# wangxiaohit/GNNPN-SC

Hardware: AMD Instinct MI355X
Metric: service-composition problems/sec (ML+2PN inference) (higher is better)
Workload: dtype f32-split3xf16 (f32 operands and results; recurrent W_hh.h products: fp32 operands split exactly into 3 x f16, six f16-matrix-core products per term, f32 accumulate; everything else f32 arithmetic)

## Files before the change

### gnnpn-sc_amd/_lib.py

```python
import ctypes
import os
from ctypes import c_char_p, c_double, c_float, c_int, c_int32, c_int64, c_uint32, c_void_p

import torch

_HERE = os.path.dirname(os.path.abspath(__file__))
LIB_PATH = os.environ.get("GNNPN_LIB") or os.path.join(_HERE, "libgnnpn_hip.so")
ABI_VERSION = 9

ACT_NONE, ACT_RELU, ACT_SIGMOID = 0, 1, 2
E_UNSUP = -2
WOA_OK, WOA_ROWS_MISMATCH, WOA_INDEX_ERROR, WOA_NO_SLOTS = 0, 1, 2, 3

_P = c_void_p
_SIGNATURES = {
    "gnnpn_abi_version": (c_int, []),
    "gnnpn_last_error": (c_char_p, []),
    "gnnpn_linear_f32": (c_int, [_P, c_int64, _P, c_int64, _P, _P, _P, c_int, _P, c_int64, c_int64, c_int, c_int, _P]),
    "gnnpn_embed_concat_f32": (c_int, [_P, _P, c_int, c_int, c_int, _P, c_int64, _P]),
    "gnnpn_csr_aggregate_f32": (c_int, [_P, _P, _P, _P, c_int64, _P, _P, _P, _P, c_int, _P, c_int64, c_int32,
                                        c_int32, _P]),
    "gnnpn_csr_aggregate_blocks_f32": (c_int, [_P, _P, _P, _P, c_int64, _P, _P, _P, _P, c_int, _P, c_int64, c_int32,
                                               c_int32, c_int32, _P, _P]),
    "gnnpn_csr_block_row_order": (c_int, [_P, c_int32, c_int32, _P, _P]),
    "gnnpn_csr_tile_plan_geometry": (c_int, [c_int32, c_int32, _P]),
    "gnnpn_csr_tile_plan_rows": (c_int, [_P, _P, _P, c_int32, c_int32, _P, _P, _P, _P, _P, _P]),
    "gnnpn_csr_tile_plan_fill": (c_int, [_P, _P, c_int32, c_int32, _P, _P, _P, _P, c_int64, _P]),
    "gnnpn_csr_aggregate_tiled_f32": (c_int, [_P, _P, _P, _P, _P, c_int64, _P, _P, _P, _P, c_int, _P, c_int64, c_int32, c_int32,
                                              c_int32, _P]),
    "gnnpn_gcn_norm_f32": (c_int, [_P, _P, _P, _P, _P, c_int32, _P]),
    "gnnpn_segment_mean_f32": (c_int, [_P, _P, c_int64, _P, c_int64, c_int32, c_int32, _P]),
    "gnnpn_gin_layer_f32": (c_int, [_P, _P, _P, c_int64, c_int32, _P, _P, _P, _P, _P, c_int32, _P, _P, _P, _P, c_int32, _P, _P, c_int32,
                                    _P, c_int64, c_int64, _P]),
    "gnnpn_split_weights_bytes": (c_int64, [c_int32, c_int32]),
    "gnnpn_lstm_split_weights_bytes": (c_int64, []),
    "gnnpn_lstm_pack_split_weights_f32": (c_int, [_P, _P, _P]),
    "gnnpn_pack_split_weights_f16": (c_int, [_P, c_int64, c_int32, c_int32, _P, _P, _P]),
    "gnnpn_gin_layer_split": (c_int, [_P, _P, _P, c_int64, c_int32, _P, _P, _P, _P, _P, _P, c_int32, _P, _P, _P, _P, _P, c_int32,
                                      _P, _P, _P, c_int32, _P, c_int64, c_int64, _P]),
    "gnnpn_request_branch_f32": (c_int, [_P, c_int32, _P, c_int32, c_int32, _P, _P, _P, c_int32, c_int32, c_int32, _P, c_int32,
                                         _P, _P, _P, _P]),
    "gnnpn_select_candidates": (c_int, [_P, c_int64, _P, _P, _P, _P, _P, _P, _P, c_int32, c_int32, c_int32, _P]),
    "gnnpn_rank_rows": (c_int, [_P, c_int64, _P, c_int32, c_int32, _P]),
    "gnnpn_precision_at_k": (c_int, [_P, c_int64, _P, c_int64, c_int32, c_int32, _P, c_int32, _P, _P]),
    "gnnpn_lstm_encode_f32": (c_int, [c_int, _P, c_int32, c_int32, c_int32, c_int32, c_int32, _P, _P, c_int64, _P]),
    "gnnpn_lstm_encode_workspace_bytes": (c_int64, []),
    "gnnpn_set_option": (c_int, [c_char_p, c_int]),
    "gnnpn_decode_diag": (c_int, [_P, c_int32, c_int32]),
    "gnnpn_coop_reset_staffing": (c_int, []),
    "gnnpn_last_launch_units": (c_int64, []),
    "gnnpn_lds_footprint_kb": (c_int, [c_int]),
    "gnnpn_coop_staffing_count": (c_int, []),
    "gnnpn_bn_train_forward_f32": (c_int, [_P, c_int64, c_int32, _P, _P, c_float, c_float, c_int, _P, _P, _P, _P, _P, _P]),
    "gnnpn_bn_train_backward_f32": (c_int, [_P, _P, _P, _P, _P, c_int64, c_int32, c_int, _P, _P, _P, _P]),
    "gnnpn_bce_sigmoid_f32": (c_int, [_P, _P, c_int64, _P, _P, _P]),
    "gnnpn_dot_f32": (c_int, [_P, _P, c_int64, _P, _P]),
    "gnnpn_embed_grad_f32": (c_int, [_P, c_int64, _P, c_int64, c_int64, c_int32, c_int32, _P, _P]),
    "gnnpn_pointer_decode_f32": (c_int, [c_int, _P, _P, c_float, c_int, c_int32, c_int32, c_int32, c_int32, c_int32,
                                         _P, _P, c_int64, _P]),
    "gnnpn_pointer_decode_workspace_bytes": (c_int64, [c_int32, c_int32, c_int32]),
    "gnnpn_pointer_decode_replicas_f32": (c_int, [_P, _P, c_float, c_int, c_int32, c_int32, c_int32, ctypes.c_uint64, c_int32, c_int32,
                                                  c_int32, _P, _P, c_int64, _P]),
    "gnnpn_replica_seed": (ctypes.c_uint64, [ctypes.c_uint64, c_int32]),
    "gnnpn_best_of_select_f32": (c_int, [c_int32, c_int32, c_int32, _P, _P, _P, _P, _P, _P, _P, _P, _P, _P, _P, _P, _P, _P]),
    "gnnpn_pointer_decode_attn_f32": (c_int, [_P, _P, _P, c_float, c_int, c_int32, c_int32, c_int32, c_int32, _P]),
    "gnnpn_attention_logits_f32": (c_int, [_P, _P, c_int64, _P, c_float, c_int, _P, c_int32, c_int32, c_int32,
                                           c_int32, c_int32, _P]),
    "gnnpn_attention_logits_bahdanau_f32": (c_int, [_P, _P, c_int64, _P, _P, c_float, c_int, _P, c_int32, c_int32, c_int32, c_int32, c_int32, _P]),
    "gnnpn_qos_reward_f32": (c_int, [_P, _P, c_int32, c_int32, c_int, _P]),
    "gnnpn_split3_pieces_f32": (c_int, [_P, c_int64, c_int32, _P, _P, _P, _P]),
    "gnnpn_recurrent_product_f32": (c_int, [_P, _P, c_int32, _P, _P, _P]),
    "gnnpn_gemm_f32": (c_int, [_P, c_int64, c_int, _P, c_int64, c_int, _P, c_int64, c_int64, c_int, c_int, c_int, _P]),
    "gnnpn_colsum_chunks_f32": (c_int, [_P, c_int64, c_int64, c_int32, c_int64, _P, _P]),
    "gnnpn_lstm_train_forward_f32": (c_int, [_P, _P, _P, _P, _P, _P, c_int32, c_int32, c_int32, _P]),
    "gnnpn_decode_train_forward_f32": (c_int, [_P, c_int32, c_int32, c_int32, c_int32, c_float, c_int, _P]),
    "gnnpn_decode_train_backward_f32": (c_int, [_P, _P, _P, _P, _P, _P, _P, c_int32, c_int32, c_int32, c_int32, c_float, c_int, _P]),
    "gnnpn_lstm_train_backward_f32": (c_int, [_P, _P, _P, _P, _P, _P, _P, c_int32, c_int32, c_int32, _P]),
    "gnnpn_decode_attn_train_forward_f32": (c_int, [_P, c_int32, c_int32, c_int32, c_int32, c_float, c_int, _P]),
    "gnnpn_decode_attn_train_backward_f32": (c_int, [_P, _P, _P, _P, _P, _P, _P, c_int32, c_int32, c_int32, c_int32, c_float, c_int, _P]),
    "gnnpn_colsum_f32": (c_int, [_P, c_int64, c_int64, c_int32, _P, _P]),
    "gnnpn_scatter_dx_f32": (c_int, [_P, _P, _P, c_int32, c_int32, c_int32, c_int32, _P]),
    "gnnpn_sumsq_f32": (c_int, [_P, c_int64, _P, _P]),
    "gnnpn_adam_step_f32": (c_int, [_P, _P, _P, _P, c_int64, _P, c_float, c_float, c_float, c_float, c_float, c_int32, _P]),
    "gnnpn_eswoa_f64": (c_int, [c_int32, c_int32, _P, _P, _P, _P, _P, c_int32, c_int32, _P, c_int32, _P, _P, _P, _P, _P]),
    "gnnpn_eswoa_wide_workspace_bytes": (c_int64, [c_int32, c_int32, c_int32]),
    "gnnpn_eswoa_wide_f64": (c_int, [c_int32, c_int32, _P, _P, _P, _P, _P, c_int32, c_int32, _P, _P, c_int64, _P, _P, _P, _P, _P]),
    "gnnpn_eswoa_ragged_workspace_bytes": (c_int64, [c_int32, c_int32, c_int32, c_int32]),
    "gnnpn_eswoa_ragged_f64": (c_int, [c_int32, _P, c_int32, c_int32, c_int32, _P, _P, _P, _P, _P, c_int32, c_int32, _P, c_int32, _P,
                                       c_int64, _P, _P, _P, _P, _P, _P]),
    "gnnpn_woa_candidates_workspace_bytes": (c_int64, [c_int32, c_int32, c_int32]),
    "gnnpn_woa_candidates_count": (c_int, [c_int32, c_int32, _P, c_int32, _P, _P, _P, c_int32, _P, _P, _P, c_int32, c_int32, c_double,
                                           _P, c_int32, c_int32, _P, c_int64, _P, _P, _P, _P, _P, _P]),
    "gnnpn_woa_candidates_fill": (c_int, [c_int32, c_int32, _P, _P, _P, c_int32, _P, c_int64, _P, _P, c_int32, c_int32, _P, _P, _P, _P,
                                          _P]),
    "gnnpn_debug_round5_f64": (c_int, [_P, _P, c_int64, _P]),
    "gnnpn_debug_cell_activations": (c_int, [_P, _P, _P, c_int64, _P]),
    "gnnpn_debug_lds_interferer": (c_int, [c_int32, c_int32, c_int32, _P]),
    "gnnpn_gate_wait": (c_int, [_P, c_uint32, c_int32, _P]),
    "gnnpn_debug_mfma_f16": (c_int, [_P, _P, _P, _P, _P]),
}
EXPORTS = tuple(_SIGNATURES)

class DecodeNet(ctypes.Structure):
    _fields_ = [(n, _P) for n in ("embedded", "enc_out", "h0", "c0", "start", "wih_packed", "whh_packed", "bih",
                                  "bhh", "latent_win", "emb_w", "emb_b", "xw_fold", "xb_fold", "start_fold", "idx", "win_logits", "pick_prob", "actions",
                                  "queries")] + \
               [("latent_from", c_int32), ("sample", c_int32), ("sample_seed", ctypes.c_uint64), ("whh_split", _P)]


class Attention(ctypes.Structure):
    _fields_ = [("attention", c_int32), ("n_glimpses", c_int32)] + \
               [(n, _P) for n in ("pointer_wq", "pointer_bq", "pointer_ref", "pointer_v", "glimpse_wq", "glimpse_bq",
                                  "glimpse_ref", "glimpse_v")]


class LaunchOpts(ctypes.Structure):
    _fields_ = [("impl", c_int32), ("lds_kb", c_int32), ("write_through", c_int32), ("paired_start", c_int32),
                ("sticky_status", _P)]


class TilePlanGeom(ctypes.Structure):
    _fields_ = [(n, c_int32) for n in ("n_blocks", "src_tiles", "src_tile_rows", "dst_tiles", "dst_tile_rows", "units", "wavefronts",
                                       "passes")] + \
               [(n, c_int64) for n in ("header_bytes", "order_bytes", "tstart_bytes", "selfw_bytes", "meta_bytes")]


class GinLayer(ctypes.Structure):
    _fields_ = [(n, _P) for n in ("w0_packed", "b0", "bn1_scale", "bn1_shift", "w3_packed", "b3", "bn2_scale", "bn2_shift",
                                  "eps")]


class DecodeTrain(ctypes.Structure):
    _fields_ = [(n, _P) for n in ("embedded", "enc_out", "h0", "c0", "start", "wih", "whh", "bih", "bhh", "latent_win", "idx",
                                  "x_all", "gates_pre", "c_all", "h_all", "z0", "probs", "logp")]


class DecodeAttnTrain(ctypes.Structure):
    _fields_ = ([("base", DecodeTrain), ("bahdanau", c_int32), ("n_glimpses", c_int32)]
                + [(n, _P) for n in ("p_wq_t", "p_wq", "p_bq", "p_v", "p_ref", "g_wq_t", "g_wq", "g_bq", "g_v", "g_ref", "q_all", "a_all",
                                     "d_p_ref", "d_g_ref", "d_p_qp", "d_g_qp", "d_p_v", "d_g_v")])


class EncodeNet(ctypes.Structure):
    _fields_ = [(n, _P) for n in ("pregates", "inputs", "w_in", "b_in", "whh_packed", "bhh", "enc_out", "h_n", "c_n", "whh_split")]


_lib = None


class GnnpnError(RuntimeError):
    pass


SOURCE_GROUPS = {
    "recurrent": ("lstm_coop.hip", "decode_lean.hip", "decode_coop.hip", "coop_common.h", "common.h", "recurrent.h", "lstm_shared.h",
                  "decode_shared.h", "lstm.hip", "decode.hip"),
    "aggregate": ("graph_tiled.hip", "graph.hip", "graph_lds.h", "common.h"),
}


def source_hash(group=None):
    import hashlib
    root = os.path.dirname(_HERE)
    csrc = os.path.join(_HERE, "csrc")
    if group is None:
        files = sorted(os.path.join(csrc, f) for f in os.listdir(csrc) if f.endswith((".hip", ".h", ".cpp")))
    else:
        files = sorted(os.path.join(csrc, f) for f in SOURCE_GROUPS[group])
    files.append(os.path.join(root, "include", "gnnpn_hip.h"))
    h = hashlib.sha256()
    for f in files:
        h.update(os.path.basename(f).encode())
        with open(f, "rb") as fh:
            h.update(fh.read())
    return h.hexdigest()[:16]


def load():
    global _lib
    if _lib is not None:
        return _lib
    if not os.path.exists(LIB_PATH):
        raise GnnpnError(
            f"{LIB_PATH} is missing: build it with `python gnnpn-sc_amd/build.py` (hipcc, gfx950). "
            "There is no CPU fallback for the ML+2PN hot path.")
    lib = ctypes.CDLL(LIB_PATH)
    for name, (res, args) in _SIGNATURES.items():
        fn = getattr(lib, name)
        fn.restype, fn.argtypes = res, args
    if lib.gnnpn_abi_version() != ABI_VERSION:
        raise GnnpnError(f"ABI mismatch: library {lib.gnnpn_abi_version()} vs binding {ABI_VERSION}")
    _lib = lib
    return lib


def check(rc, what):
    if rc != 0:
        msg = load().gnnpn_last_error().decode("utf-8", "replace")
        raise GnnpnError(f"{what} failed ({rc}): {msg}")


def stream_ptr():
    return ctypes.c_void_p(torch.cuda.current_stream().cuda_stream)


def dev_ptr(t, dtype, name, allow_none=False):
    if t is None:
        if allow_none:
            return None
        raise GnnpnError(f"{name}: tensor required")
    if not isinstance(t, torch.Tensor) or not t.is_cuda:
        raise GnnpnError(f"{name}: expected a CUDA tensor (the hot path has no CPU implementation), got "
# ... 14 lines not shown
```

### gnnpn-sc_amd/csrc/coop_common.h

```cpp
#pragma once
#include "common.h"
#include "lstm_shared.h"

typedef float f32x4 __attribute__((ext_vector_type(4)));
typedef unsigned long long u64;

__device__ __forceinline__ void granule_store(u64* p, unsigned tag, float v) {
    __hip_atomic_store(p, ((u64)tag << 32) | __float_as_uint(v), __ATOMIC_RELAXED,
                       __HIP_MEMORY_SCOPE_AGENT);
}

typedef unsigned u32x4 __attribute__((ext_vector_type(4)));
#define GNNPN_LD2(dst, voff, sbase, off) "global_load_dwordx4 " dst ", " voff ", " sbase " offset:" off " sc1\n\t"
__device__ __forceinline__ const u64* uniform_ptr(const u64* p) {
    const unsigned long long v = (unsigned long long)p;
    const unsigned lo = __builtin_amdgcn_readfirstlane((unsigned)v), hi = __builtin_amdgcn_readfirstlane((unsigned)(v >> 32));
    return reinterpret_cast<const u64*>(((unsigned long long)hi << 32) | lo);
}
__device__ __forceinline__ void granule_reload2_x8_masked(u32x4 (&v)[8], const u64* base, unsigned voff, unsigned long long lanes) {
    const u64* q = base + 512;
    unsigned long long saved;
    asm volatile("s_and_saveexec_b64 %8, %12\n\t"
                 GNNPN_LD2("%0", "%9", "%10", "0") GNNPN_LD2("%1", "%9", "%10", "1024") GNNPN_LD2("%2", "%9", "%10", "2048")
                 GNNPN_LD2("%3", "%9", "%10", "3072") GNNPN_LD2("%4", "%9", "%11", "0") GNNPN_LD2("%5", "%9", "%11", "1024")
                 GNNPN_LD2("%6", "%9", "%11", "2048") GNNPN_LD2("%7", "%9", "%11", "3072")
                 "s_waitcnt vmcnt(0)\n\t"
                 "s_mov_b64 exec, %8"
                 : "+v"(v[0]), "+v"(v[1]), "+v"(v[2]), "+v"(v[3]), "+v"(v[4]), "+v"(v[5]), "+v"(v[6]), "+v"(v[7]), "=&s"(saved)
                 : "v"(voff), "s"(base), "s"(q), "s"(lanes)
                 : "memory", "scc");
}
__device__ __forceinline__ void granule_load2_x8_x4(u32x4 (&v)[8], u32x4 (&w)[4], const u64* base, const u64* pbase, unsigned voff) {
    const u64* q = base + 512;
    asm volatile(GNNPN_LD2("%0", "%12", "%13", "0") GNNPN_LD2("%1", "%12", "%13", "1024") GNNPN_LD2("%2", "%12", "%13", "2048")
                 GNNPN_LD2("%3", "%12", "%13", "3072") GNNPN_LD2("%4", "%12", "%14", "0") GNNPN_LD2("%5", "%12", "%14", "1024")
                 GNNPN_LD2("%6", "%12", "%14", "2048") GNNPN_LD2("%7", "%12", "%14", "3072")
                 GNNPN_LD2("%8", "%12", "%15", "0") GNNPN_LD2("%9", "%12", "%15", "1024") GNNPN_LD2("%10", "%12", "%15", "2048")
                 GNNPN_LD2("%11", "%12", "%15", "3072")
                 "s_waitcnt vmcnt(0)"
                 : "=&v"(v[0]), "=&v"(v[1]), "=&v"(v[2]), "=&v"(v[3]), "=&v"(v[4]), "=&v"(v[5]), "=&v"(v[6]), "=&v"(v[7]),
                   "=&v"(w[0]), "=&v"(w[1]), "=&v"(w[2]), "=&v"(w[3])
                 : "v"(voff), "s"(base), "s"(q), "s"(pbase)
                 : "memory");
}

__device__ __forceinline__ void granule_load2_x8_x4_lat(u32x4 (&v)[8], u32x4 (&w)[4], u64& lat, const u64* base, const u64* pbase,
                                                        const u64* lbase, unsigned voff) {
    const u64* q = base + 512;
    asm volatile(GNNPN_LD2("%0", "%13", "%15", "0") GNNPN_LD2("%1", "%13", "%15", "1024") GNNPN_LD2("%2", "%13", "%15", "2048")
                 GNNPN_LD2("%3", "%13", "%15", "3072") GNNPN_LD2("%4", "%13", "%16", "0") GNNPN_LD2("%5", "%13", "%16", "1024")
                 GNNPN_LD2("%6", "%13", "%16", "2048") GNNPN_LD2("%7", "%13", "%16", "3072")
                 GNNPN_LD2("%8", "%13", "%17", "0") GNNPN_LD2("%9", "%13", "%17", "1024") GNNPN_LD2("%10", "%13", "%17", "2048")
                 GNNPN_LD2("%11", "%13", "%17", "3072")
                 "global_load_dwordx2 %12, %14, %18 sc1\n\t"
                 "s_waitcnt vmcnt(0)"
                 : "=&v"(v[0]), "=&v"(v[1]), "=&v"(v[2]), "=&v"(v[3]), "=&v"(v[4]), "=&v"(v[5]), "=&v"(v[6]), "=&v"(v[7]),
                   "=&v"(w[0]), "=&v"(w[1]), "=&v"(w[2]), "=&v"(w[3]), "=&v"(lat)
                 : "v"(voff), "v"(voff >> 1), "s"(base), "s"(q), "s"(pbase), "s"(lbase)
                 : "memory");
}

constexpr int COOP_STAFFING_WORD = 8 * 256 + 8;
__device__ __forceinline__ void coop_raise(unsigned* err, unsigned* sticky, unsigned code, unsigned* seats = nullptr) {
    atomicOr(err, code);
    if (sticky) atomicOr(sticky, code);
    if (seats && atomicCAS(err + 4, 1u, 2u) == 1u) atomicSub(seats + COOP_STAFFING_WORD, 1u);
}

constexpr int COOP_STATUS_BYTES = 16384;
constexpr unsigned COOP_LDS_UNITS = 640;
constexpr int COOP_XCD_STRIDE = 32;
constexpr int COOP_XCDCNT_OFFSET = 12288;
constexpr int COOP_ARRIVE_OFFSET = 13312;
constexpr int COOP_PLACED_OFFSET = 14336;
constexpr int COOP_CLAIM_OFFSET = 2048;
constexpr int COOP_TAKEN_OFFSET = 10240;
constexpr int COOP_OVERREAD_BYTES = 4096;
constexpr int COOP_OVERSUB = 3;
constexpr unsigned COOP_SURPLUS_WAIT_TICKS = 1600;
constexpr unsigned COOP_RESERVE_WAIT_TICKS = 200000;

__device__ __forceinline__ unsigned xcc_id() {
    return __builtin_amdgcn_s_getreg(20 | (0 << 6) | (3 << 11)) & 0xfu;
}

__device__ __forceinline__ void granule_store_l2_bits(u64* p, u64 g) {
    asm volatile("global_store_dwordx2 %0, %1, off" ::"v"(p), "v"(g) : "memory");
}
__device__ __forceinline__ void granule_store_l2(u64* p, unsigned tag, float v) {
    granule_store_l2_bits(p, ((u64)tag << 32) | __float_as_uint(v));
}
__device__ __forceinline__ void granule_publish(u64* p, unsigned tag, float v, bool same_xcd) {
    if (same_xcd) granule_store_l2(p, tag, v);
    else granule_store(p, tag, v);
}

namespace {
__global__ __launch_bounds__(256) void coop_zero_kernel(unsigned long long* __restrict__ p, size_t n8, unsigned* __restrict__ sticky,
                                                        int word, unsigned expected, int skip_zeroing) {
    if (sticky && blockIdx.x == 0 && threadIdx.x == 0) atomicAdd(sticky + word, expected);
    if (skip_zeroing) return;
    for (size_t i = blockIdx.x * (size_t)blockDim.x + threadIdx.x; i < n8; i += (size_t)gridDim.x * blockDim.x)
        __hip_atomic_store(p + i, 0ull, __ATOMIC_RELAXED, __HIP_MEMORY_SCOPE_AGENT);
}
}
inline hipError_t coop_zero_workspace(void* workspace, size_t bytes, hipStream_t s, unsigned* sticky, int word, unsigned expected,
                                      bool skip_zeroing = false) {
    const size_t n8 = bytes / 8;
    unsigned blocks = skip_zeroing ? 1u : (unsigned)((n8 + 255) / 256);
    if (blocks > 2048) blocks = 2048;
    hipLaunchKernelGGL(coop_zero_kernel, dim3(blocks), dim3(256), 0, s, static_cast<unsigned long long*>(workspace), n8, sticky, word,
                       expected, skip_zeroing ? 1 : 0);
    return hipGetLastError();
}

constexpr int COOP_G = 8, COOP_ROWS = 16, COOP_H = 256;

struct CoopLaunch {
    int n_tiles, gpx, groups, groups_per_net;
    unsigned* status;
    char* buffers;
    unsigned* seats;
};

template <typename Need>
inline int coop_begin(const char* who, int n_nets, int32_t rows, Need need, int expected_word, const CoopOpts& opts,
                      void* workspace, int64_t workspace_bytes, hipStream_t s, CoopLaunch& L) {
    int dev = 0, n_cu = 0;
    if (hipGetDevice(&dev) != hipSuccess ||
        hipDeviceGetAttribute(&n_cu, hipDeviceAttributeMultiprocessorCount, dev) != hipSuccess)
        GNNPN_FAIL(GNNPN_E_LAUNCH, "%s: cannot query the device", who);
    L.n_tiles = (rows + COOP_ROWS - 1) / COOP_ROWS;
    L.gpx = n_cu / (8 * COOP_G);
    if (L.gpx > 8) L.gpx = 8;
    while (L.gpx > 1 && (L.gpx - 1) * 8 >= n_nets * L.n_tiles) --L.gpx;
    if (L.gpx < 1 || n_cu < 256)
        GNNPN_FAIL(GNNPN_E_UNSUP, "%s: device has %d CUs, the cooperative form is built for 8 XCDs x 32 CUs", who, n_cu);
    L.groups = L.gpx * 8;
    if (L.groups < n_nets) GNNPN_FAIL(GNNPN_E_UNSUP, "%s: %d groups for %d nets", who, L.groups, n_nets);
    L.groups_per_net = L.groups / n_nets;
    const int64_t bytes = need(L.groups);
    if (!workspace || workspace_bytes < bytes || !gnnpn_aligned(workspace, 256))
        GNNPN_FAIL(GNNPN_E_ARG, "%s: workspace of %lld B (256-B aligned) required", who, (long long)bytes);
    L.seats = gnnpn_cu_seat_table();
    if (!L.seats) GNNPN_FAIL(GNNPN_E_LAUNCH, "%s: cannot allocate the seat table", who);
    const unsigned units = (unsigned)(COOP_G * n_nets * L.n_tiles);
    if (coop_zero_workspace(workspace, (size_t)bytes, s, opts.sticky, expected_word, units, (gnnpn_option_lstm_ablate() & 0x2000) != 0) !=
        hipSuccess)
        GNNPN_FAIL(GNNPN_E_LAUNCH, "%s: workspace memset failed", who);
    g_gnnpn_last_units = opts.sticky ? (int64_t)units : 0;
    L.status = static_cast<unsigned*>(workspace);
    L.buffers = static_cast<char*>(workspace) + COOP_STATUS_BYTES;
    return GNNPN_OK;
}

struct DecodeWorkspace {
    int64_t h_bytes, p_bytes, l_bytes;
    int64_t total() const { return COOP_STATUS_BYTES + h_bytes + p_bytes + l_bytes + COOP_OVERREAD_BYTES; }
};
inline DecodeWorkspace decode_workspace(int64_t groups, int64_t rows, int32_t T, int32_t K, int64_t xp_granules) {
    const int64_t tiles = (rows + COOP_ROWS - 1) / COOP_ROWS;
    return {groups * 2 * COOP_ROWS * COOP_H * 8, groups * 2 * xp_granules * 8, tiles * T * COOP_ROWS * (int64_t)K * 8};
}
__device__ __forceinline__ void coop_note_finished(unsigned* sticky, int word, unsigned tiles_done) {
    if (sticky && tiles_done) atomicAdd(sticky + word, tiles_done);
}

__device__ __forceinline__ void coop_note_staffed(unsigned* status, unsigned* count_xcc, unsigned target, unsigned* seats) {
    if (atomicAdd(count_xcc, 1u) + 1u == target && atomicAdd(status + 5, 1u) + 1u == 8u && atomicExch(status + 4, 2u) == 1u)
        atomicSub(seats + COOP_STAFFING_WORD, 1u);
}
template <int G>
__device__ __forceinline__ bool coop_place(unsigned* status, int gpx, int* slot, int& group, int& member, unsigned* seats,
                                           bool paired_start = false, unsigned* sticky = nullptr) {
    if (threadIdx.x < 64) {
        const int lane = threadIdx.x;
        const unsigned xcc = xcc_id();
        unsigned* count = status + COOP_XCDCNT_OFFSET / 4;
        unsigned* arrive = status + COOP_ARRIVE_OFFSET / 4;
        unsigned* taken = status + COOP_TAKEN_OFFSET / 4 + xcc * 64;
        const unsigned target = (unsigned)(gpx * G);
        auto staffed = [&]() {
            unsigned v = 0;
            if (lane == 0) v = __hip_atomic_load(status + 5, __ATOMIC_RELAXED, __HIP_MEMORY_SCOPE_AGENT);
            return __shfl(v, 0, 64) >= 8u;
        };
        int g = -1, m = 0;
#ifndef GNNPN_COOP_NO_ENTRY_ACQUIRE
        __builtin_amdgcn_fence(__ATOMIC_ACQUIRE, "agent");
#endif
        const unsigned hw = __builtin_amdgcn_s_getreg(4 | (0 << 6) | (31 << 11));
        const unsigned key = (xcc << 8) | ((hw >> 8) & 0xffu);
        unsigned* staffing = seats + COOP_STAFFING_WORD;
        const unsigned* word = lane < 8 ? count + COOP_XCD_STRIDE * lane : lane == 9 ? status + 4 : seats + key;
        unsigned got = 0;
        if (lane < 12 && lane != 8 && lane != 10) got = __hip_atomic_load(word, __ATOMIC_RELAXED, __HIP_MEMORY_SCOPE_AGENT);
        if (lane == 8) got = atomicAdd(arrive + COOP_XCD_STRIDE * xcc, 1u);
        const bool staffed_at_entry = __all(lane >= 8 || got >= target);
        unsigned arrival = __shfl(got, 8, 64);
        const bool marked = __shfl(got, 9, 64) != 0u;
        const unsigned seat_seen = __shfl(got, 11, 64);
        if (lane == 0) {
            if (arrival == 0u && !marked && atomicCAS(status + 4, 0u, 1u) == 0u) atomicAdd(staffing, 1u);
            if (arrival >= gridDim.x / 8 || (staffed_at_entry && arrival < target)) coop_raise(status, sticky, 8u);
        }
        if (!staffed_at_entry) {
            if (lane == 0) {
                atomicAdd(status + COOP_CLAIM_OFFSET / 4 + key, 1u);
                const unsigned la = __builtin_amdgcn_s_getreg(6 | (0 << 6) | (31 << 11));
                const unsigned lds_base = la & 0xfffu, lds_size = (la >> 12) & 0xfffu;
                const bool badly_placed = lds_base != 0u && lds_base < lds_size && lds_base + 2u * lds_size > COOP_LDS_UNITS;
                bool another_staffing = false;
                if (badly_placed && !paired_start) {
                    if (atomicCAS(status + 4, 0u, 1u) == 0u) atomicAdd(staffing, 1u);
                    another_staffing = __hip_atomic_load(staffing, __ATOMIC_RELAXED, __HIP_MEMORY_SCOPE_AGENT) > 1u;
                }
                const bool fragments = (paired_start || another_staffing) && badly_placed;
                const bool reserve_arrival = arrival + target >= gridDim.x / 8;
                if (fragments && !reserve_arrival) {
                    atomicAdd(status + 3, 1u);
                    if (sticky) atomicAdd(sticky + GNNPN_STATUS_DECLINED_SEATS, 1u);
                    g = -2;
                } else if (!fragments) {
                    unsigned s = seat_seen;
                    if (s == 0u) {
                        if (atomicCAS(seats + key, 0u, 0xffffffffu) == 0u) {
                            s = atomicAdd(seats + 8 * 256 + xcc, 1u) + 1u;
                            __hip_atomic_store(seats + key, s, __ATOMIC_RELAXED, __HIP_MEMORY_SCOPE_AGENT);
                        } else {
                            s = 0xffffffffu;
                        }
                    }
                    for (unsigned spin = 0; s == 0xffffffffu && spin < 100000u; ++spin)
                        s = __hip_atomic_load(seats + key, __ATOMIC_RELAXED, __HIP_MEMORY_SCOPE_AGENT);
                    const unsigned seat = s - 1u;
                    if (seat < target && atomicCAS(taken + seat, 0u, 1u) == 0u) {
                        g = (int)xcc * gpx + (int)(seat / G);
                        m = (int)(seat % G);
                        coop_note_staffed(status, count + COOP_XCD_STRIDE * xcc, target, seats);
                    }
                }
            }
            g = __shfl(g, 0, 64);
            m = __shfl(m, 0, 64);
            arrival = __shfl(arrival, 0, 64);
            if (g == -2) {
                g = -1;
            } else if (g < 0) {
                const unsigned per_xcd = gridDim.x / 8;
                const bool reserve = arrival + target >= per_xcd;
                const unsigned long long patience = reserve ? COOP_RESERVE_WAIT_TICKS : COOP_SURPLUS_WAIT_TICKS;
                const unsigned long long t0 = __builtin_amdgcn_s_memrealtime();
                bool done = staffed();
                while (!done && __builtin_amdgcn_s_memrealtime() - t0 < patience) {
                    __builtin_amdgcn_s_sleep(8);
                    done = staffed();
                }
                if (!done && reserve) {
                    if (lane == 0) {
                        for (unsigned seat = 0; seat < target && g < 0; ++seat) {
                            if (atomicCAS(taken + seat, 0u, 1u) == 0u) {
                                g = (int)xcc * gpx + (int)(seat / G);
                                m = (int)(seat % G);
                                coop_note_staffed(status, count + COOP_XCD_STRIDE * xcc, target, seats);
                                atomicAdd(status + 2, 1u);
                                if (sticky) atomicAdd(sticky + GNNPN_STATUS_OFF_CANONICAL_SEATS, 1u);
                            }
                        }
                    }
                    g = __shfl(g, 0, 64);
                    m = __shfl(m, 0, 64);
                }
            }
        }
        if (lane == 0) {
            slot[0] = g;
            slot[1] = m;
        }
    }
    __syncthreads();
    group = slot[0];
    member = slot[1];
    return group >= 0;
}

__device__ __forceinline__ float swap8(float v) {
    return __int_as_float(__builtin_amdgcn_update_dpp(0, __float_as_int(v), 0x128 , 0xF, 0xF, false));
}

__device__ __forceinline__ u64 phase_stamp() {
    u64 t;
    __builtin_amdgcn_sched_barrier(0);
    asm volatile("s_memtime %0\n\ts_waitcnt lgkmcnt(0)" : "=s"(t)::"memory");
    __builtin_amdgcn_sched_barrier(0);
    return t;
}

constexpr int LDT = 260;
__device__ __forceinline__ int ht_index(int row, int unit) { return row * LDT + (unit & 3) * 64 + (unit >> 2); }

struct NoHook {
// ... 220 lines not shown
```

### gnnpn-sc_amd/csrc/decode.hip

```cpp
#include <atomic>

#include "common.h"
#include <string.h>
#include "recurrent.h"
#include "decode_shared.h"
#include "lstm_shared.h"

template <int H, int BT, bool REP = false>
__global__ __launch_bounds__((H < 64 ? 64 : H)) void pointer_decode_kernel(
    const float* __restrict__ embedded, const float* __restrict__ enc_out, const float* __restrict__ h0,
    const float* __restrict__ c0, const float* __restrict__ start, const float* __restrict__ wih,
    const float* __restrict__ whh, const float* __restrict__ bih, const float* __restrict__ bhh,
    const float* __restrict__ latent_win, const float* __restrict__ inputs, float tanh_c, int use_tanh,
    int32_t* __restrict__ idx_out, float* __restrict__ win_logits, float* __restrict__ pick_prob,
    float* __restrict__ actions, float* __restrict__ queries, int32_t B, int32_t T, int32_t n_per, int sample,
    unsigned long long sample_seed, int rep_R, int rep_first) {
    constexpr int NT = H < 64 ? 64 : H;
    constexpr int NW = NT / 64;
    __shared__ __attribute__((aligned(16))) float xs[BT][H];
    __shared__ __attribute__((aligned(16))) float hs[2][BT][H];
    __shared__ float lg[BT][64];
    __shared__ int sel[BT];

    const int j = threadIdx.x;
    const bool owner = j < H;
    const int lane = j & 63, wave = j >> 6;
    const int b0 = blockIdx.x * BT;
    const int L = T * n_per;
    const float4* __restrict__ Wi = reinterpret_cast<const float4*>(wih);
    const float4* __restrict__ Wh = reinterpret_cast<const float4*>(whh);
    auto prob_of = [rep_R](int b) { return REP ? b / rep_R : b; };

    float bi[4], bh[4], c[BT], h[BT];
#pragma unroll
    for (int g = 0; g < 4; ++g) {
        bi[g] = owner ? bih[g * H + j] : 0.0f;
        bh[g] = owner ? bhh[g * H + j] : 0.0f;
    }
#pragma unroll
    for (int p = 0; p < BT; ++p) {
        const bool ok = owner && (b0 + p < B);
        c[p] = ok ? c0[(int64_t)prob_of(b0 + p) * H + j] : 0.0f;
        h[p] = ok ? h0[(int64_t)prob_of(b0 + p) * H + j] : 0.0f;
        if (owner) {
            hs[0][p][j] = h[p];
            xs[p][j] = start[j];
        }
    }
    __syncthreads();

    int cur = 0;
    for (int k = 0; k < T; ++k) {
        if (owner) {
            float ai[BT][4], ah[BT][4];
#pragma unroll
            for (int p = 0; p < BT; ++p)
#pragma unroll
                for (int g = 0; g < 4; ++g) ai[p][g] = ah[p][g] = 0.0f;
            gemv_chain<H, BT>(Wi, xs, j, ai);
            gemv_chain<H, BT>(Wh, hs[cur], j, ah);
#pragma unroll
            for (int p = 0; p < BT; ++p) {
                float gate[4];
#pragma unroll
                for (int g = 0; g < 4; ++g)
                    gate[g] = __fadd_rn(__fadd_rn(ah[p][g], bh[g]), __fadd_rn(ai[p][g], bi[g]));
                lstm_cell_update(gate[0], gate[1], gate[2], gate[3], c[p], h[p]);
                hs[cur ^ 1][p][j] = h[p];
                if (queries && b0 + p < B) queries[((int64_t)(b0 + p) * T + k) * H + j] = h[p];
            }
        }
        __syncthreads();
        cur ^= 1;

        for (int q = wave; q < BT * n_per; q += NW) {
            const int p = q / n_per, r = q - p * n_per;
            float part = 0.0f;
            if (b0 + p < B) part = lane_dot4<H>(enc_out + ((int64_t)prob_of(b0 + p) * L + (int64_t)k * n_per + r) * H, hs[cur][p]);
            const float dot = wave_sum(part);
            if (lane == 0) lg[p][r] = dot;
        }
        __syncthreads();

        if (j < BT && b0 + j < B) {
            const int p = j;
            const int64_t wbase = ((int64_t)(b0 + p) * T + k) * n_per;
            const int64_t lbase = ((int64_t)prob_of(b0 + p) * T + k) * n_per;
            const unsigned long long seed =
                REP ? replica_seed(sample_seed, (unsigned long long)(rep_first + (b0 + p) % rep_R)) : sample_seed;
            float prob;
            const int best_r = window_pick(lg[p], n_per, tanh_c, use_tanh, win_logits, wbase, latent_win, lbase,
                                           sample, seed, (unsigned long long)prob_of(b0 + p) * T + k, prob);
            pick_prob[(int64_t)(b0 + p) * T + k] = prob;
            idx_out[(int64_t)(b0 + p) * T + k] = k * n_per + best_r;
            sel[p] = k * n_per + best_r;
        }
        __syncthreads();

#pragma unroll
        for (int p = 0; p < BT; ++p) {
            if (b0 + p < B) {
                const int64_t row = (int64_t)prob_of(b0 + p) * L + sel[p];
                if (owner) xs[p][j] = embedded[row * H + j];
                if (j < 8) actions[((int64_t)(b0 + p) * T + k) * 8 + j] = inputs[row * 8 + j];
            }
        }
        __syncthreads();
    }
}

template <int H, bool REP = false>
static void launch_decode(const DecodeArgs& args, const DecodeNet& d, const float* latent, hipStream_t s,
                          ReplicaMap rep = ReplicaMap{0, 0}) {
    constexpr int NT = H < 64 ? 64 : H;
    const int32_t B = args.B;
    int bt = 1;
    while (bt < 4 && B / (bt * 2) >= 256) bt *= 2;
    dim3 grid((B + bt - 1) / bt), block(NT);
#define GNNPN_LAUNCH_DEC(BT_)                                                                                                    \
    hipLaunchKernelGGL((pointer_decode_kernel<H, BT_, REP>), grid, block, 0, s, d.embedded, d.enc_out, d.h0, d.c0, d.start, d.wih, \
                       d.whh, d.bih, d.bhh, latent, args.inputs, args.tanh_c, args.use_tanh, d.idx, d.win_logits, d.pick_prob,   \
                       d.actions, d.queries, B, args.T, args.K, d.sample, (unsigned long long)d.sample_seed, rep.R, rep.first)
    switch (bt) {
        case 1: GNNPN_LAUNCH_DEC(1); break;
        case 2: GNNPN_LAUNCH_DEC(2); break;
        default: GNNPN_LAUNCH_DEC(4); break;
    }
#undef GNNPN_LAUNCH_DEC
}

extern "C" int gnnpn_pointer_decode_f32(int n_nets, const gnnpn_decode_net_t* nets, const float* inputs,
                                        float tanh_c, int use_tanh, int32_t B, int32_t T, int32_t n_per, int32_t H,
                                        int32_t precision, const gnnpn_launch_opts_t* opts_in, void* workspace,
                                        int64_t workspace_bytes, void* stream) {
    g_gnnpn_last_units = 0;
    GNNPN_REQUIRE(B >= 0 && T > 0, "pointer_decode: bad shape");
    if (B == 0) return GNNPN_OK;
    GNNPN_REQUIRE(nets && inputs, "pointer_decode: null input");
    const CoopOpts opts = coop_opts(opts_in);
    GNNPN_REQUIRE(opts.impl >= 0 && opts.impl <= 4 && opts.impl != 3, "pointer_decode: opts.impl must be 0 (auto), 1 (streaming), 2 (cooperative, 8-CU groups) or 4 (8-CU groups, 256-register build) — the 16-CU-group form (3) was removed in ABI version 7");
    GNNPN_REQUIRE(opts.lds_kb >= 0 && opts.lds_kb <= 160, "pointer_decode: opts.lds_kb must be 0..160");
    GNNPN_REQUIRE(precision == GNNPN_PREC_F32 || precision == GNNPN_PREC_SPLIT, "pointer_decode: precision must be GNNPN_PREC_F32 or GNNPN_PREC_SPLIT, got %d", precision);
    GNNPN_REQUIRE(n_nets >= 1 && n_nets <= GNNPN_MAX_DECODE_NETS, "pointer_decode: n_nets must be 1..%d",
                  GNNPN_MAX_DECODE_NETS);
    GNNPN_REQUIRE(n_per >= 1 && n_per <= 64, "pointer_decode: n_per must be in [1,64], got %d", n_per);
    if (H != 256 && H != 32) GNNPN_FAIL(GNNPN_E_UNSUP, "pointer_decode: hidden size %d not built (256, 32)", H);
    DecodeArgs args{};
    for (int n = 0; n < n_nets; ++n) {
        const gnnpn_decode_net_t& d = nets[n];
        if (const int rc = decode_net_check(d, "pointer_decode", n)) return rc;
        GNNPN_REQUIRE(d.embedded || (d.emb_w && d.emb_b) || d.xw_fold,
                      "pointer_decode: net %d needs embedded, (emb_w, emb_b) or the folded input side", n);
        GNNPN_REQUIRE(d.latent_from < n && d.latent_from >= -1, "pointer_decode: latent_from of net %d must name an "
                      "earlier net of the call", n);
        GNNPN_REQUIRE(!(d.latent_win && d.latent_from >= 0), "pointer_decode: net %d has two latent sources", n);
        GNNPN_REQUIRE(!d.whh_split || gnnpn_aligned(d.whh_split, 16), "pointer_decode: whh_split must be 16-byte aligned");
        static_assert(sizeof(DecodeNet) == sizeof(gnnpn_decode_net_t), "layout");
        memcpy(&args.net[n], &d, sizeof(DecodeNet));
    }
    args.inputs = inputs;
    args.tanh_c = tanh_c;
    args.use_tanh = use_tanh;
    args.B = B;
    args.T = T;
    args.K = n_per;
    hipStream_t s = (hipStream_t)stream;
    bool any_sample = false;
    for (int n = 0; n < n_nets; ++n) any_sample |= nets[n].sample != 0;
    if (any_sample && (precision != GNNPN_PREC_F32 || opts.impl > 2))
        GNNPN_FAIL(GNNPN_E_UNSUP, "pointer_decode: sampling is built in the streaming and the 8-CU-group fp32 forms (impl 0-2, "
                   "GNNPN_PREC_F32)");
    const int impl = opts.impl;
    if (impl != 1 && gnnpn_decode_coop_supported(H, n_per) && (workspace != nullptr || impl >= 2)) {
        const int rc = gnnpn_launch_decode_coop(args, n_nets, precision, impl == 4, opts, workspace, workspace_bytes, s);
        const bool fall_through = rc == GNNPN_E_UNSUP && impl == 0 && precision == GNNPN_PREC_F32;
        if (rc != GNNPN_OK && !fall_through) return rc;
        if (fall_through) {
            static std::atomic<bool> said{false};
            if (!said.exchange(true))
                fprintf(stderr, "[gnnpn] pointer_decode: %s — taking the per-workgroup streaming form (about 10 x slower per step)\n", gnnpn_last_error());
        }
        if (rc == GNNPN_OK) {
            GNNPN_CHECK_LAUNCH("pointer_decode_f32(coop)");
            return GNNPN_OK;
        }
    }
    if (precision == GNNPN_PREC_SPLIT)
        GNNPN_FAIL(GNNPN_E_UNSUP, "pointer_decode: the split-operand precision needs the cooperative form (H = 256)");
    for (int n = 0; n < n_nets; ++n) {
        const DecodeNet& d = args.net[n];
        if (!d.embedded) GNNPN_FAIL(GNNPN_E_UNSUP, "pointer_decode: the streaming form needs the embedded tensor");
        const float* latent = d.latent_from >= 0 ? args.net[d.latent_from].win_logits : d.latent_win;
        GNNPN_FOR_H(H, launch_decode<HH>(args, d, latent, s));
    }
    GNNPN_CHECK_LAUNCH("pointer_decode_f32");
    return GNNPN_OK;
}

extern "C" uint64_t gnnpn_replica_seed(uint64_t seed, int32_t replica) {
    return replica_seed(seed, (unsigned long long)(long long)replica);
}

extern "C" int gnnpn_pointer_decode_replicas_f32(const gnnpn_decode_net_t* net, const float* inputs, float tanh_c, int use_tanh,
                                                 int32_t B, int32_t R, int32_t first, uint64_t seed, int32_t T, int32_t n_per,
                                                 int32_t H, const gnnpn_launch_opts_t* opts_in, void* workspace,
                                                 int64_t workspace_bytes, void* stream) {
    g_gnnpn_last_units = 0;
    GNNPN_REQUIRE(R >= 1, "pointer_decode_replicas: R must be >= 1, got %d", R);
    GNNPN_REQUIRE(first >= 0, "pointer_decode_replicas: first replica must be >= 0, got %d", first);
    GNNPN_REQUIRE(B >= 0 && T > 0 && n_per >= 1 && n_per <= 64, "pointer_decode_replicas: bad shape (B %d, T %d, n_per %d)", B, T, n_per);
    const int64_t rows = (int64_t)B * R;
    GNNPN_REQUIRE(rows <= (1 << 30), "pointer_decode_replicas: B*R = %lld rows exceed 2^30", (long long)rows);
    if (H != 256 && H != 32) GNNPN_FAIL(GNNPN_E_UNSUP, "pointer_decode_replicas: hidden size %d not built (256, 32)", H);
    if (B == 0) return GNNPN_OK;
    GNNPN_REQUIRE(net && inputs, "pointer_decode_replicas: null input");
    const CoopOpts opts = coop_opts(opts_in);
    GNNPN_REQUIRE(opts.impl >= 0 && opts.impl <= 2, "pointer_decode_replicas: opts.impl must be 0 (auto), 1 (streaming) or 2 (cooperative)");
    GNNPN_REQUIRE(opts.lds_kb >= 0 && opts.lds_kb <= 160, "pointer_decode_replicas: opts.lds_kb must be 0..160");
    const gnnpn_decode_net_t& d = *net;
    if (const int rc = decode_net_check(d, "pointer_decode_replicas", 0)) return rc;
    GNNPN_REQUIRE(d.embedded || d.xw_fold, "pointer_decode_replicas: the net needs embedded or the folded input side");
    GNNPN_REQUIRE(!d.queries, "pointer_decode_replicas: queries are not written (must be NULL)");
    GNNPN_REQUIRE(d.latent_from == -1, "pointer_decode_replicas: latent_from must be -1 (Low's window logits come from latent_win)");
    DecodeArgs args{};
    memcpy(&args.net[0], &d, sizeof(DecodeNet));
    args.net[0].sample = 1;
    args.net[0].sample_seed = seed;
    args.net[0].whh_split = nullptr;
    args.inputs = inputs;
    args.tanh_c = tanh_c;
    args.use_tanh = use_tanh;
    args.B = (int32_t)rows;
    args.T = T;
    args.K = n_per;
    hipStream_t s = (hipStream_t)stream;
    const bool coop = opts.impl != 1 && gnnpn_decode_coop_supported(H, n_per) && d.xw_fold && (workspace != nullptr || opts.impl == 2);
    if (coop) {
        const int64_t need = gnnpn_decode_coop_workspace_need(rows, T, n_per);
        GNNPN_REQUIRE(workspace && workspace_bytes >= need && gnnpn_aligned(workspace, 256),
                      "pointer_decode_replicas: B*R = %lld rows need a workspace of %lld B (256-B aligned), got %lld B",
                      (long long)rows, (long long)need, (long long)workspace_bytes);
        const int rc = gnnpn_launch_decode_coop(args, 1, GNNPN_PREC_F32, false, opts, workspace, workspace_bytes, s,
                                                ReplicaMap{R, first});
        if (rc != GNNPN_OK) return rc;
        GNNPN_CHECK_LAUNCH("pointer_decode_replicas_f32(coop)");
        return GNNPN_OK;
    }
    if (opts.impl == 2) GNNPN_FAIL(GNNPN_E_UNSUP, "pointer_decode_replicas: the cooperative form needs H = 256, n_per <= 16 and the folded input side");
    if (!d.embedded) GNNPN_FAIL(GNNPN_E_UNSUP, "pointer_decode_replicas: the streaming form needs the embedded tensor");
    GNNPN_FOR_H(H, (launch_decode<HH, true>(args, args.net[0], args.net[0].latent_win, s, ReplicaMap{R, first})));
    GNNPN_CHECK_LAUNCH("pointer_decode_replicas_f32");
    return GNNPN_OK;
}

__global__ __launch_bounds__(256) void attention_logits_kernel(const float* __restrict__ enc_out,
                                                               const float* __restrict__ queries, int64_t ld_q,
                                                               float tanh_c, int use_tanh, float* __restrict__ logits,
                                                               int64_t n_rows, int32_t L, int32_t H) {
    const int lane = threadIdx.x & 63;
    const int64_t row = (int64_t)blockIdx.x * 4 + (threadIdx.x >> 6);
    if (row >= n_rows) return;
    const int64_t b = row / L;
    const float* e = enc_out + row * H;
    const float* q = queries + b * ld_q;
    float part = 0.0f;
    for (int i = lane * 4; i < H; i += 256) {
        const float4 ev = *reinterpret_cast<const float4*>(e + i);
        const float4 qv = *reinterpret_cast<const float4*>(q + i);
        part = fmaf(ev.x, qv.x, part);
        part = fmaf(ev.y, qv.y, part);
        part = fmaf(ev.z, qv.z, part);
        part = fmaf(ev.w, qv.w, part);
    }
    float v = wave_sum(part);
    if (use_tanh) v = __fmul_rn(tanh_c, tanhf(v));
    if (lane == 0) logits[row] = v;
}

__global__ __launch_bounds__(256) void attention_logits_bahdanau_kernel(const float* __restrict__ ref, const float* __restrict__ qp,
                                                                        int64_t ld_q, const float* __restrict__ v, float tanh_c,
                                                                        int use_tanh, float* __restrict__ logits, int64_t n_rows,
                                                                        int32_t L, int32_t H) {
    const int lane = threadIdx.x & 63;
    const int64_t row = (int64_t)blockIdx.x * 4 + (threadIdx.x >> 6);
    if (row >= n_rows) return;
    const float* r = ref + row * H;
    const float* q = qp + (row / L) * ld_q;
    float part = 0.0f;
    for (int i = lane; i < H; i += 64) part = fmaf(v[i], tanhf(q[i] + r[i]), part);
    float u = wave_sum(part);
    if (use_tanh) u = __fmul_rn(tanh_c, tanhf(u));
    if (lane == 0) logits[row] = u;
}

__global__ void mask_logits_kernel(const int32_t* __restrict__ masked_idx, float* __restrict__ logits, int32_t B,
                                   int32_t L, int32_t n_masked, int32_t ld_idx) {
    const int i = blockIdx.x * blockDim.x + threadIdx.x;
    if (i >= B * n_masked) return;
    const int b = i / n_masked, m = i - b * n_masked;
    const int pos = masked_idx[(int64_t)b * ld_idx + m];
    if (pos >= 0 && pos < L) logits[(int64_t)b * L + pos] = -INFINITY;
}

extern "C" int gnnpn_attention_logits_f32(const float* enc_out, const float* queries, int64_t ld_q,
                                          const int32_t* masked_idx, float tanh_c, int use_tanh, float* logits,
                                          int32_t B, int32_t L, int32_t H, int32_t n_masked, int32_t ld_idx,
                                          void* stream) {
    GNNPN_REQUIRE(B >= 0 && L > 0 && H > 0 && H % 4 == 0 && ld_q >= H && ld_q % 4 == 0, "attention_logits: bad shape");
    if (B == 0) return GNNPN_OK;
    GNNPN_REQUIRE(enc_out && queries && logits, "attention_logits: null operand");
    GNNPN_REQUIRE(n_masked == 0 || (masked_idx && ld_idx >= n_masked), "attention_logits: bad mask list");
    GNNPN_REQUIRE(gnnpn_aligned(enc_out, 16) && gnnpn_aligned(queries, 16), "attention_logits: 16-byte alignment");
    if (B == 0) return GNNPN_OK;
    hipStream_t s = (hipStream_t)stream;
    const int64_t n_rows = (int64_t)B * L;
    hipLaunchKernelGGL(attention_logits_kernel, dim3((unsigned)((n_rows + 3) / 4)), dim3(256), 0, s, enc_out, queries,
                       ld_q, tanh_c, use_tanh, logits, n_rows, L, H);
    if (n_masked > 0)
        hipLaunchKernelGGL(mask_logits_kernel, dim3((B * n_masked + 255) / 256), dim3(256), 0, s, masked_idx, logits,
                           B, L, n_masked, ld_idx);
    GNNPN_CHECK_LAUNCH("attention_logits_f32");
    return GNNPN_OK;
}

extern "C" int gnnpn_attention_logits_bahdanau_f32(const float* ref, const float* qp, int64_t ld_q, const float* v,
                                                   const int32_t* masked_idx, float tanh_c, int use_tanh, float* logits, int32_t B,
                                                   int32_t L, int32_t H, int32_t n_masked, int32_t ld_idx, void* stream) {
    GNNPN_REQUIRE(ref && qp && v && logits && B >= 0 && L > 0 && H > 0 && ld_q >= H, "attention_logits_bahdanau: bad argument");
    GNNPN_REQUIRE(n_masked == 0 || (masked_idx && ld_idx >= n_masked), "attention_logits_bahdanau: bad mask");
    if (B == 0) return GNNPN_OK;
    hipStream_t s = (hipStream_t)stream;
    const int64_t n_rows = (int64_t)B * L;
    hipLaunchKernelGGL(attention_logits_bahdanau_kernel, dim3((unsigned)((n_rows + 3) / 4)), dim3(256), 0, s, ref, qp, ld_q, v,
                       tanh_c, use_tanh, logits, n_rows, L, H);
    if (n_masked > 0)
        hipLaunchKernelGGL(mask_logits_kernel, dim3((B * n_masked + 255) / 256), dim3(256), 0, s, masked_idx, logits, B, L,
                           n_masked, ld_idx);
    GNNPN_CHECK_LAUNCH("attention_logits_bahdanau_f32");
    return GNNPN_OK;
}

__global__ __launch_bounds__(256) void qos_reward_kernel(const float* __restrict__ actions, float* __restrict__ R, int32_t B,
                                                        int32_t T, int level) {
    const int lane = threadIdx.x & 63;
    const int b = blockIdx.x * 4 + (threadIdx.x >> 6);
    if (b >= B) return;
    const float* a = actions + (int64_t)b * T * 8;
    const float lo0 = a[4], hi0 = a[5], lo1 = a[6], hi1 = a[7];
    float prod2 = 1.0f, prod3 = 1.0f, mn = INFINITY;
    double sum0 = 0.0;
    int n_real = 0;
    auto fetch = [&](int t) { return *reinterpret_cast<const float4*>(a + (int64_t)min(t, T - 1) * 8); };
    auto consume = [&](float4 q, int t0) {
        if (t0 + lane >= T) q = make_float4(0.0f, INFINITY, 1.0f, 1.0f);
        n_real += q.x > 0.0f;
        mn = fminf(mn, q.y);
        const double xd = (double)q.x;
        const int lo = __double2loint(xd), hi = __double2hiint(xd);
        const int zi = __float_as_int(q.z), wi = __float_as_int(q.w);
        const int cnt = min(64, T - t0);
#define GNNPN_REWARD_STEP(i)                                                                                      \
    prod2 = __fmul_rn(prod2, __int_as_float(__builtin_amdgcn_readlane(zi, i)));                                   \
    prod3 = __fmul_rn(prod3, __int_as_float(__builtin_amdgcn_readlane(wi, i)));                                   \
    sum0 += __hiloint2double(__builtin_amdgcn_readlane(hi, i), __builtin_amdgcn_readlane(lo, i));
        if (cnt == 64) {
#pragma unroll
            for (int i = 0; i < 64; ++i) { GNNPN_REWARD_STEP(i) }
        } else {
            for (int i = 0; i < cnt; ++i) { GNNPN_REWARD_STEP(i) }
        }
#undef GNNPN_REWARD_STEP
    };
    float4 qa = fetch(lane), qb;
    for (int t0 = 0; t0 < T; t0 += 128) {
        qb = fetch(t0 + 64 + lane);
        consume(qa, t0);
        if (t0 + 64 >= T) break;
        qa = fetch(t0 + 128 + lane);
        consume(qb, t0 + 64);
    }
#pragma unroll
    for (int off = 32; off > 0; off >>= 1) {
        n_real += __shfl_xor(n_real, off, 64);
        mn = fminf(mn, __shfl_xor(mn, off, 64));
    }
    if (lane != 0) return;
    int violate = 0;
    if (prod2 < lo0 || prod2 > hi0) ++violate;
    if (prod3 < lo1 || prod3 > hi1) ++violate;
    if (level == 0) {
        R[b] = (float)violate;
        return;
    }
    float obj = (float)sum0 / (float)n_real;
    obj = __fadd_rn(obj, 1.0f);
    obj = __fsub_rn(obj, mn);
    obj = obj / 2.0f;
    const double v = (double)violate + (double)obj;
    R[b] = (float)(rint(v * 1e5) / 1e5);
}

extern "C" int gnnpn_qos_reward_f32(const float* actions, float* R, int32_t B, int32_t T, int level,
                                    void* stream) {
    GNNPN_REQUIRE(B >= 0 && T > 0 && (level == 0 || level == 1), "qos_reward: bad argument");
    if (B == 0) return GNNPN_OK;
    GNNPN_REQUIRE(actions && R, "qos_reward: null operand");
    hipLaunchKernelGGL(qos_reward_kernel, dim3((B + 3) / 4), dim3(256), 0, (hipStream_t)stream, actions, R, B, T,
                       level);
    GNNPN_CHECK_LAUNCH("qos_reward_f32");
    return GNNPN_OK;
}

__global__ __launch_bounds__(256) void best_of_select_kernel(int32_t B, int32_t N, int32_t T, const float* __restrict__ R0,
                                                             const int32_t* __restrict__ idx0, const float* __restrict__ act0,
                                                             const float* __restrict__ prob0, const float* __restrict__ Rs,
                                                             const int32_t* __restrict__ idxs, const float* __restrict__ acts,
                                                             const float* __restrict__ probs, float* __restrict__ R_out,
                                                             int32_t* __restrict__ idx_out, float* __restrict__ act_out,
                                                             float* __restrict__ prob_out, int32_t* __restrict__ winner) {
    const int lane = threadIdx.x & 63;
    const int b = blockIdx.x * 4 + (threadIdx.x >> 6);
    if (b >= B) return;
    const int S = N - 1;
    unsigned long long best = ~0ull;
    for (int j = lane; j < N; j += 64) {
        float r = j == 0 ? R0[b] : Rs[(int64_t)b * S + (j - 1)];
        if (r == 0.0f) r = 0.0f;
        const unsigned hi = r != r ? 0xFFFFFFFFu : float_order_key(r);
        const unsigned long long key = ((unsigned long long)hi << 32) | (unsigned)j;
        best = key < best ? key : best;
    }
#pragma unroll
    for (int off = 32; off > 0; off >>= 1) {
        const unsigned lo = __shfl_xor((unsigned)(best & 0xffffffffu), off, 64);
        const unsigned hi = __shfl_xor((unsigned)(best >> 32), off, 64);
        const unsigned long long o = ((unsigned long long)hi << 32) | lo;
        best = o < best ? o : best;
    }
    const int w = (int)(best & 0xffffffffu);
    const int64_t src = w == 0 ? (int64_t)b : (int64_t)b * S + (w - 1);
    const int32_t* si = (w == 0 ? idx0 : idxs) + src * T;
    const float* sp = (w == 0 ? prob0 : probs) + src * T;
    const float* sa = (w == 0 ? act0 : acts) + src * T * 8;
    for (int t = lane; t < T; t += 64) {
        idx_out[(int64_t)b * T + t] = si[t];
        prob_out[(int64_t)b * T + t] = sp[t];
    }
    for (int i = lane; i < T * 8; i += 64) act_out[(int64_t)b * T * 8 + i] = sa[i];
    if (lane == 0) {
        winner[b] = w;
        R_out[b] = w == 0 ? R0[b] : Rs[src];
    }
}

extern "C" int gnnpn_best_of_select_f32(int32_t B, int32_t N, int32_t T, const float* R0, const int32_t* idx0, const float* actions0,
                                        const float* probs0, const float* Rs, const int32_t* idxs, const float* actionss,
                                        const float* probss, float* R_out, int32_t* idx_out, float* actions_out, float* probs_out,
                                        int32_t* winner, void* stream) {
    GNNPN_REQUIRE(B >= 0 && N >= 1 && T > 0 && (int64_t)T * 8 < (1ll << 31), "best_of_select: bad argument (B %d, N %d, T %d)", B, N, T);
    if (B == 0) return GNNPN_OK;
    GNNPN_REQUIRE(R0 && idx0 && actions0 && probs0, "best_of_select: null input (replica 0)");
    GNNPN_REQUIRE(N == 1 || (Rs && idxs && actionss && probss), "best_of_select: null input (replicas 1..N-1)");
    GNNPN_REQUIRE(R_out && idx_out && actions_out && probs_out && winner, "best_of_select: null output");
    hipLaunchKernelGGL(best_of_select_kernel, dim3((B + 3) / 4), dim3(256), 0, (hipStream_t)stream, B, N, T, R0, idx0, actions0,
                       probs0, Rs, idxs, actionss, probss, R_out, idx_out, actions_out, probs_out, winner);
    GNNPN_CHECK_LAUNCH("best_of_select_f32");
    return GNNPN_OK;
}
```

### gnnpn-sc_amd/csrc/decode_lean.hip

```cpp
#include "common.h"
#include "recurrent.h"
#include "decode_shared.h"
#include "coop_common.h"
#include "lstm_shared.h"

namespace {
constexpr int H = COOP_H;
constexpr int G = COOP_G;
constexpr int ROWS = COOP_ROWS;
constexpr int UNITS = H / G;
constexpr int KW = 16;
constexpr unsigned SPIN_LIMIT = 400000;
constexpr int XP_GRANULES = ROWS * KW * G;

typedef unsigned u32x2 __attribute__((ext_vector_type(2)));
constexpr int AUX_SC1 = 16;


__device__ __forceinline__ __amdgpu_buffer_rsrc_t make_rsrc(const void* p, unsigned bytes) {
    return __builtin_amdgcn_make_buffer_rsrc(const_cast<void*>(p), 0, (int)bytes, 0x00020000);
}
__device__ __forceinline__ float dpp_ror(float v, int n) {
    switch (n) {
        case 1: return __int_as_float(__builtin_amdgcn_update_dpp(0, __float_as_int(v), 0x121, 0xF, 0xF, true));
// ... 277 lines not shown
                    float dot = 0.0f, lv = 0.0f;
                    if (live) {
                        dot = __fadd_rn(__fadd_rn(__fadd_rn(__uint_as_float(vp[0].x), __uint_as_float(vp[0].z)), __uint_as_float(vp[1].x)), __uint_as_float(vp[1].z));
                        dot = __fadd_rn(__fadd_rn(__fadd_rn(__fadd_rn(dot, __uint_as_float(vp[2].x)), __uint_as_float(vp[2].z)), __uint_as_float(vp[3].x)), __uint_as_float(vp[3].z));
                        if (latent_in_launch) lv = __uint_as_float(vl.x);
                        else if (net.latent_win) lv = __uint_as_float(__builtin_amdgcn_raw_buffer_load_b32(r_lw, vo_wl, so_t, 0));
                    }
                    float v = a.use_tanh ? __fmul_rn(a.tanh_c, tanhf(dot)) : dot;
                    if (live && first) {
                        __builtin_amdgcn_raw_buffer_store_b32(__float_as_uint(v), r_wl, vo_wl, so_t, 0);
                        if (publishes_latent)
                            __builtin_amdgcn_raw_buffer_store_b64(u32x2{__float_as_uint(v), 1u}, r_lat, vo_lat, so_l0, AUX_SC1);
                    }
                    v = (has_lat && live) ? __fadd_rn(v, lv) : v;
                    float m = live ? v : -INFINITY;
                    m = fmaxf(m, dpp_ror(m, 8));
                    m = fmaxf(m, dpp_ror(m, 4));
                    m = fmaxf(m, dpp_ror(m, 2));
                    m = fmaxf(m, dpp_ror(m, 1));
                    const unsigned hit = (unsigned)(__ballot(live && v == m) >> (16 * rq)) & 0xffffu;
                    const int pick_r = hit ? __ffs(hit) - 1 : 0;
                    if (r == 0) {
                        sel[row] = pick_r;
                        if (first) __builtin_amdgcn_raw_buffer_store_b32((unsigned)((k - 1) * K + pick_r), r_idx, vo_idx, (unsigned)(k - 1) * 4u, 0);
                    }
                }
                __syncthreads();
                if (abort_flag) break;
                axf0 = win[c][sel[c]][kq];
                axf1 = win[c][sel[c]][4 + kq];
                if (first && wave == 0) {
                    __builtin_amdgcn_raw_buffer_store_b32(__float_as_uint(axf0), r_act, vo_act, (unsigned)(k - 1) * 32u, 0);
                    __builtin_amdgcn_raw_buffer_store_b32(__float_as_uint(axf1), r_act, vo_act, (unsigned)(k - 1) * 32u + 16u, 0);
                }
                if (k == T) break;
                if constexpr (DIAG) st[5] = phase_stamp();
            }

            if constexpr (!EV_EARLY) request_ev();
            u32x4 wv0, wv1;
            wv0 = __builtin_amdgcn_raw_buffer_load_b128(r_in, vo_win, so_k * 32u, 0);
            wv1 = __builtin_amdgcn_raw_buffer_load_b128(r_in, vo_win, so_k * 32u + 16u, 0);
            float gx[2][4];
            if (k > 0) {
                f32x4 ax0 = {0.f, 0.f, 0.f, 0.f}, ax1 = ax0;
                ax0 = __builtin_amdgcn_mfma_f32_16x16x4f32(axf0, wXf[0][0], ax0, 0, 0, 0);
                ax1 = __builtin_amdgcn_mfma_f32_16x16x4f32(axf0, wXf[1][0], ax1, 0, 0, 0);
                ax0 = __builtin_amdgcn_mfma_f32_16x16x4f32(axf1, wXf[0][1], ax0, 0, 0, 0);
                ax1 = __builtin_amdgcn_mfma_f32_16x16x4f32(axf1, wXf[1][1], ax1, 0, 0, 0);
#pragma unroll
                for (int q = 0; q < 4; ++q) {
                    gx[0][q] = __fadd_rn(ax0[q], bi[0]);
                    gx[1][q] = __fadd_rn(ax1[q], bi[1]);
                }
            } else {
#pragma unroll
                for (int q = 0; q < 4; ++q) {
                    gx[0][q] = sg[0];
                    gx[1][q] = sg[1];
                }
            }
            {
                f32x2 g0[2], g1[2];
#pragma unroll
                for (int q = 0; q < 2; ++q) {
                    g0[q] = (f32x2{ah[0][2 * q], ah[0][2 * q + 1]} + pk_set(bh[0])) + f32x2{gx[0][2 * q], gx[0][2 * q + 1]};
                    g1[q] = (f32x2{ah[1][2 * q], ah[1][2 * q + 1]} + pk_set(bh[1])) + f32x2{gx[1][2 * q], gx[1][2 * q + 1]};
                }
                cell_update_split(g0, g1, c < 8, cst, hl);
            }
            {
                const unsigned so_pub = (step & 1) * (ROWS * H * 8);
                if constexpr (SPLIT) {
                    store_granule(r_h, vo_hpub, so_pub, split_granule(step + 1, hl.x), same_xcd);
                    store_granule(r_h, vo_hpub, so_pub + H * 8, split_granule(step + 1, hl.y), same_xcd);
                } else {
                    store_granule(r_h, vo_hpub, so_pub, ((u64)(step + 1) << 32) | __float_as_uint(hl.x), same_xcd);
                    store_granule(r_h, vo_hpub, so_pub + H * 8, ((u64)(step + 1) << 32) | __float_as_uint(hl.y), same_xcd);
                }
                hsl[own0][wave * 8 + (c & 7)] = hl.x;
                hsl[own0 + 1][wave * 8 + (c & 7)] = hl.y;
                if (net.queries) {
                    __builtin_amdgcn_raw_buffer_store_b32(__float_as_uint(hl.x), r_q, vo_q, (unsigned)k * (H * 4), 0);
                    __builtin_amdgcn_raw_buffer_store_b32(__float_as_uint(hl.y), r_q, vo_q, (unsigned)(k + T) * (H * 4), 0);
                }
            }
            if constexpr (DIAG) {
                asm volatile("" ::"v"(hl.y));
                st[6] = phase_stamp();
            }
            __syncthreads();
            {
                float p = 0.0f;
                if (pdot) {
#pragma unroll
                    for (int j = 0; j < EVN; ++j) {
                        const float4 hv = *reinterpret_cast<const float4*>(&hsl[prow][phalf * (4 * EVN) + 4 * j]);
                        p = fmaf(__uint_as_float(ev[j].x), hv.x, p);
                        p = fmaf(__uint_as_float(ev[j].y), hv.y, p);
                        p = fmaf(__uint_as_float(ev[j].z), hv.z, p);
                        p = fmaf(__uint_as_float(ev[j].w), hv.w, p);
                    }
                }
                if constexpr (EVH == 2)
                    p = __fadd_rn(p, __int_as_float(__builtin_amdgcn_update_dpp(0, __float_as_int(p), 0xB1 , 0xF, 0xF, false)));
                if (pdot && phalf == 0)
                    store_granule(r_p, vo_ppub, (step & 1) * (XP_GRANULES * 8), ((u64)(step + 1) << 32) | __float_as_uint(p), same_xcd);
            }
            if (wr_live) {
                *reinterpret_cast<u32x4*>(&win[wr_row][wr_cand][0]) = wv0;
                *reinterpret_cast<u32x4*>(&win[wr_row][wr_cand][4]) = wv1;
            }
            if constexpr (DIAG) {
                st[7] = phase_stamp();
                if (blockIdx.x == 0 && tid == 0 && k > 0) {
                    u64* prof = reinterpret_cast<u64*>(err) + 4;
                    prof[0] += st[1] - st[0];
                    prof[1] += st[2] - st[1];
                    prof[2] += st[3] - st[2];
                    prof[3] += st[4] - st[3];
                    prof[4] += st[5] - st[4];
                    prof[5] += st[6] - st[5];
                    prof[6] += st[7] - st[6];
                    prof[7] += 1;
                }
            }
            ++step;
        }
        if (abort_flag) break;
        ++tiles_done;
    }
    if (tid == 0) {
        if (abort_flag) coop_raise(err, sticky, 2u, seats);
        coop_note_finished(sticky, GNNPN_STATUS_DEC_FINISHED, tiles_done);
    }
}

struct PickProbArgs {
    const float* win[2];
    const float* lat[2];
    const int32_t* idx[2];
    float* out[2];
};
__global__ __launch_bounds__(256) void pick_prob_kernel(PickProbArgs a, int64_t rows, int T, int K) {
    const int net = blockIdx.y;
    const float* __restrict__ win = a.win[net];
    const float* __restrict__ lat = a.lat[net];
    const int32_t* __restrict__ idx = a.idx[net];
    float* __restrict__ out = a.out[net];
    const int64_t row = blockIdx.x * 256ll + threadIdx.x;
    if (row >= rows) return;
    const unsigned t_base = (unsigned)__builtin_amdgcn_readfirstlane((int)((blockIdx.x * 256ll) % T));
    const int t = (int)((t_base + threadIdx.x) % (unsigned)T);
    float v[16];
#pragma unroll
    for (int j = 0; j < 16; ++j) {
        v[j] = 0.0f;
        if (j < K) {
            v[j] = win[row * K + j];
            if (lat) v[j] = __fadd_rn(v[j], lat[row * K + j]);
        }
    }
    const int pick_r = min(max(idx[row] - t * K, 0), 15);
    float best = v[0];
#pragma unroll
    for (int j = 1; j < 16; ++j) best = j == pick_r ? v[j] : best;
#pragma unroll
    for (int j = 0; j < 16; ++j) v[j] = j < K ? expf(__fsub_rn(v[j], best)) : 0.0f;
#pragma unroll
    for (int n = 8; n >= 1; n >>= 1)
#pragma unroll
        for (int j = 0; j < n; ++j) v[j] = __fadd_rn(v[j], v[j + n]);
    out[row] = 1.0f / v[0];
}

static DecodeWorkspace lean_workspace(int64_t groups, int64_t rows, int32_t T, int32_t K) {
    return decode_workspace(groups, rows, T, K, XP_GRANULES);
}

int64_t gnnpn_decode_lean_workspace_bytes(int32_t B, int32_t T, int32_t n_per) { return lean_workspace(64, B, T, n_per).total(); }

int gnnpn_launch_decode_lean(const DecodeArgs& args, int n_nets, int precision, bool shared_cu, const CoopOpts& opts,
                             void* workspace, int64_t workspace_bytes, hipStream_t s) {
    if (args.K > KW) GNNPN_FAIL(GNNPN_E_UNSUP, "pointer_decode: the cooperative form is built for n_per <= %d", KW);
    if ((int64_t)ROWS * args.T * args.K * H * 4 >= (1ll << 32) || (int64_t)args.T * ROWS * args.K * 8 >= (1ll << 32))
        GNNPN_FAIL(GNNPN_E_UNSUP, "pointer_decode: a tile of 16 problems must stay below 4 GB of encoder output");
    const bool split = precision == GNNPN_PREC_SPLIT;
    const bool wide = args.K > 8;
    const bool stamps = (gnnpn_option_lstm_ablate() & 0x800) != 0;
    if (stamps && wide) GNNPN_FAIL(GNNPN_E_UNSUP, "pointer_decode: the stamped build exists for n_per <= 8");
    CoopLaunch c;
    const auto need = [&](int groups) { return lean_workspace(groups, args.B, args.T, args.K).total(); };
    if (const int rc = coop_begin("pointer_decode", n_nets, args.B, need, GNNPN_STATUS_DEC_EXPECTED, opts, workspace, workspace_bytes, s, c))
        return rc;
    const DecodeWorkspace w = lean_workspace(c.groups, args.B, args.T, args.K);
    u64* p_h = reinterpret_cast<u64*>(c.buffers);
    u64* p_p = reinterpret_cast<u64*>(c.buffers + w.h_bytes);
    u64* p_l = reinterpret_cast<u64*>(c.buffers + w.h_bytes + w.p_bytes);
    static unsigned* p_diag = gnnpn_decode_diag_buffer();
    const int wt = (opts.write_through ? 1 : 0) | (opts.paired_start ? 2 : 0);
#define GNNPN_LEAN(SPLIT_, OCC_, EVH_, ...)                                                                                           \
    hipLaunchKernelGGL((pointer_decode_lean_kernel<SPLIT_, OCC_, EVH_, ##__VA_ARGS__>), dim3(COOP_OVERSUB * c.groups * G), dim3(256),       \
                       gnnpn_lds_padding((const void*)pointer_decode_lean_kernel<SPLIT_, OCC_, EVH_, ##__VA_ARGS__>, opts.lds_kb), s, args, \
                       p_h, p_p, p_l, c.status, opts.sticky, n_nets, c.groups_per_net, c.gpx, wt, c.seats, p_diag)
    if (stamps) {
        if (split) GNNPN_LEAN(true, 1, 2, true);
        else GNNPN_LEAN(false, 1, 2, true);
    } else if (split && shared_cu && wide) GNNPN_LEAN(true, 2, 1);
    else if (split && shared_cu) GNNPN_LEAN(true, 2, 2);
    else if (split && wide) GNNPN_LEAN(true, 1, 1);
    else if (split) GNNPN_LEAN(true, 1, 2);
    else if (shared_cu && wide) GNNPN_LEAN(false, 2, 1);
    else if (shared_cu) GNNPN_LEAN(false, 2, 2);
    else if (wide) GNNPN_LEAN(false, 1, 1);
    else GNNPN_LEAN(false, 1, 2);
#undef GNNPN_LEAN
    if (hipGetLastError() != hipSuccess) GNNPN_FAIL(GNNPN_E_LAUNCH, "pointer_decode: launch of the cooperative kernel failed");
    const int64_t rows = (int64_t)args.B * args.T;
    for (int n0 = 0; n0 < n_nets; n0 += 2) {
        PickProbArgs pa = {};
        const int cnt = n_nets - n0 < 2 ? n_nets - n0 : 2;
        for (int n = 0; n < cnt; ++n) {
            const DecodeNet& d = args.net[n0 + n];
            pa.win[n] = d.win_logits;
            pa.lat[n] = d.latent_from >= 0 ? args.net[d.latent_from].win_logits : d.latent_win;
            pa.idx[n] = d.idx;
            pa.out[n] = d.pick_prob;
        }
        hipLaunchKernelGGL(pick_prob_kernel, dim3((unsigned)((rows + 255) / 256), (unsigned)cnt), dim3(256), 0, s, pa, rows, args.T, args.K);
    }
    return GNNPN_OK;
}
```

### gnnpn-sc_amd/csrc/decode_shared.h

```cpp
#pragma once
#include "common.h"
#include "lstm_shared.h"

struct DecodeNet {
    const float* embedded;
    const float* enc_out;
    const float* h0;
    const float* c0;
    const float* start;
    const float* wih;
    const float* whh;
    const float* bih;
    const float* bhh;
    const float* latent_win;
    const float* emb_w;
    const float* emb_b;
    const float* xw_fold;
    const float* xb_fold;
    const float* start_fold;
    int32_t* idx;
    float* win_logits;
    float* pick_prob;
    float* actions;
    float* queries;
    int32_t latent_from;
    int32_t sample;
    uint64_t sample_seed;
    const void* whh_split;
};
static_assert(sizeof(DecodeNet) == sizeof(gnnpn_decode_net_t), "DecodeNet must mirror gnnpn_decode_net_t");

inline int decode_net_check(const gnnpn_decode_net_t& d, const char* who, int n) {
    GNNPN_REQUIRE(d.enc_out && d.h0 && d.c0 && d.start && d.wih_packed && d.whh_packed && d.bih && d.bhh,
                  "%s: null input of net %d (enc_out, h0, c0, start and the decoder weights are required)", who, n);
    GNNPN_REQUIRE(d.idx && d.win_logits && d.pick_prob && d.actions, "%s: null output of net %d", who, n);
    GNNPN_REQUIRE((d.xw_fold != nullptr) == (d.xb_fold != nullptr) && (d.xw_fold != nullptr) == (d.start_fold != nullptr),
                  "%s: net %d: xw_fold, xb_fold and start_fold go together", who, n);
    GNNPN_REQUIRE(d.sample == 0 || d.sample == 1, "%s: net %d: sample must be 0 (greedy) or 1 (multinomial)", who, n);
    GNNPN_REQUIRE(gnnpn_aligned(d.wih_packed, 16) && gnnpn_aligned(d.whh_packed, 16) && gnnpn_aligned(d.enc_out, 16) &&
                      (!d.embedded || gnnpn_aligned(d.embedded, 16)),
                  "%s: weights / enc_out / embedded must be 16-byte aligned", who);
    return GNNPN_OK;
}

template <int H>
__device__ __forceinline__ float lane_dot4(const float* __restrict__ row, const float* q) {
    float part = 0.0f;
    for (int e = (threadIdx.x & 63) * 4; e < H; e += 256) {
        const float4 rv = *reinterpret_cast<const float4*>(row + e);
        const float4 qv = *reinterpret_cast<const float4*>(q + e);
        part = fmaf(rv.x, qv.x, part);
        part = fmaf(rv.y, qv.y, part);
        part = fmaf(rv.z, qv.z, part);
        part = fmaf(rv.w, qv.w, part);
    }
    return part;
}

__device__ __forceinline__ int window_pick(float* lg, int K, float tanh_c, int use_tanh, float* __restrict__ win_logits, int64_t wbase,
                                           const float* __restrict__ latent_win, int64_t lbase, int sample, unsigned long long seed,
                                           unsigned long long ctr, float& prob) {
    float best = 0.0f;
    int best_r = -1;
    for (int r = 0; r < K; ++r) {
        float v = lg[r];
        if (use_tanh) v = __fmul_rn(tanh_c, tanhf(v));
        win_logits[wbase + r] = v;
        if (latent_win) v = __fadd_rn(v, latent_win[lbase + r]);
        lg[r] = v;
        if (best_r < 0 || v > best) {
            best = v;
            best_r = r;
        }
    }
    float denom = 0.0f;
    for (int r = 0; r < K; ++r) denom = __fadd_rn(denom, expf(__fsub_rn(lg[r], best)));
    prob = 1.0f / denom;
    if (sample) {
        const float u = stream_uniform24(seed, ctr);
        float cdf = 0.0f;
        int pick = -1, last_pos = 0;
        for (int r = 0; r < K; ++r) {
            const float pr = expf(__fsub_rn(lg[r], best)) / denom;
            cdf = __fadd_rn(cdf, pr);
            if (pr > 0.0f) last_pos = r;
            if (pick < 0 && u < cdf) pick = r;
        }
        if (pick < 0) pick = last_pos;
        best_r = pick;
        prob = expf(__fsub_rn(lg[pick], best)) / denom;
    }
    return best_r;
}

#define GNNPN_MAX_DECODE_NETS 2

struct DecodeArgs {
    DecodeNet net[GNNPN_MAX_DECODE_NETS];
    const float* inputs;
    float tanh_c;
    int use_tanh;
    int32_t B, T, K;
};

struct ReplicaMap {
    int32_t R;
    int32_t first;
};

bool gnnpn_decode_coop_supported(int32_t H, int32_t n_per);
int64_t gnnpn_decode_coop_workspace_need(int64_t rows, int32_t T, int32_t n_per);
int gnnpn_launch_decode_coop(const DecodeArgs& args, int n_nets, int precision, bool shared_cu, const CoopOpts& opts,
                             void* workspace, int64_t workspace_bytes, hipStream_t s, ReplicaMap rep = ReplicaMap{0, 0});
int gnnpn_launch_decode_lean(const DecodeArgs& args, int n_nets, int precision, bool shared_cu, const CoopOpts& opts,
                             void* workspace, int64_t workspace_bytes, hipStream_t s);
int64_t gnnpn_decode_lean_workspace_bytes(int32_t B, int32_t T, int32_t n_per);
unsigned* gnnpn_decode_diag_buffer();
```

### gnnpn-sc_amd/csrc/lstm.hip

```cpp
#include "common.h"
#include "recurrent.h"
#include "lstm_shared.h"

template <int H, int BT>
__global__ __launch_bounds__(H) void lstm_encode_kernel(LstmNets nets, int32_t B, int32_t L) {
    __shared__ __attribute__((aligned(16))) float hs[2][BT][H];
    const int net = blockIdx.y;
    const int b0 = blockIdx.x * BT;
    const int j = threadIdx.x;
    const float* __restrict__ pre = nets.pregates[net];
    const float4* __restrict__ Wp = reinterpret_cast<const float4*>(nets.whh[net]);
    float* __restrict__ enc = nets.enc_out[net];

    float bh[4];
#pragma unroll
    for (int g = 0; g < 4; ++g) bh[g] = nets.bhh[net][g * H + j];
    float c[BT], h[BT];
#pragma unroll
    for (int p = 0; p < BT; ++p) {
        c[p] = 0.0f;
        h[p] = 0.0f;
        hs[0][p][j] = 0.0f;
    }
    __syncthreads();

    int cur = 0;
    for (int t = 0; t < L; ++t) {
        float pg[BT][4];
#pragma unroll
        for (int p = 0; p < BT; ++p)
#pragma unroll
            for (int g = 0; g < 4; ++g)
                pg[p][g] = (b0 + p < B) ? pre[((int64_t)(b0 + p) * L + t) * (4 * H) + g * H + j] : 0.0f;
        float acc[BT][4];
#pragma unroll
        for (int p = 0; p < BT; ++p)
#pragma unroll
            for (int g = 0; g < 4; ++g) acc[p][g] = 0.0f;
        gemv_chain<H, BT>(Wp, hs[cur], j, acc);
#pragma unroll
        for (int p = 0; p < BT; ++p) {
            lstm_cell_update(__fadd_rn(__fadd_rn(acc[p][0], bh[0]), pg[p][0]),
                             __fadd_rn(__fadd_rn(acc[p][1], bh[1]), pg[p][1]),
                             __fadd_rn(__fadd_rn(acc[p][2], bh[2]), pg[p][2]),
                             __fadd_rn(__fadd_rn(acc[p][3], bh[3]), pg[p][3]), c[p], h[p]);
            hs[cur ^ 1][p][j] = h[p];
            if (b0 + p < B) enc[((int64_t)(b0 + p) * L + t) * H + j] = h[p];
        }
        __syncthreads();
        cur ^= 1;
    }
#pragma unroll
    for (int p = 0; p < BT; ++p) {
        if (b0 + p < B) {
            nets.h_n[net][(int64_t)(b0 + p) * H + j] = h[p];
            nets.c_n[net][(int64_t)(b0 + p) * H + j] = c[p];
        }
    }
}

template <int H>
static int launch_encode(const LstmNets& nets, int n_nets, int32_t B, int32_t L, hipStream_t s) {
    int bt = 1;
    while (bt < 8 && (int64_t)B * n_nets / (bt * 2) >= 256) bt *= 2;
    dim3 grid((B + bt - 1) / bt, n_nets), block(H);
    switch (bt) {
        case 1: hipLaunchKernelGGL((lstm_encode_kernel<H, 1>), grid, block, 0, s, nets, B, L); break;
        case 2: hipLaunchKernelGGL((lstm_encode_kernel<H, 2>), grid, block, 0, s, nets, B, L); break;
        case 4: hipLaunchKernelGGL((lstm_encode_kernel<H, 4>), grid, block, 0, s, nets, B, L); break;
        default: hipLaunchKernelGGL((lstm_encode_kernel<H, 8>), grid, block, 0, s, nets, B, L); break;
    }
    return 0;
}

extern "C" int gnnpn_lstm_encode_f32(int n_nets, const gnnpn_encode_net_t* in, int32_t B, int32_t L, int32_t H,
                                     int32_t F, int32_t precision, const gnnpn_launch_opts_t* opts_in, void* workspace,
                                     int64_t workspace_bytes, void* stream) {
    GNNPN_REQUIRE(n_nets >= 1 && n_nets <= GNNPN_MAX_NETS, "lstm_encode: n_nets must be 1..%d", GNNPN_MAX_NETS);
    GNNPN_REQUIRE(in, "lstm_encode: null net array");
    GNNPN_REQUIRE(B >= 0 && L > 0, "lstm_encode: bad shape");
    g_gnnpn_last_units = 0;
    if (B == 0) return GNNPN_OK;
    GNNPN_REQUIRE(precision >= GNNPN_PREC_F32 && precision <= GNNPN_PREC_SPLIT, "lstm_encode: unknown precision %d", precision);
    if (H != 256 && H != 32) GNNPN_FAIL(GNNPN_E_UNSUP, "lstm_encode: hidden size %d not built (256, 32)", H);
    LstmNets nets{};
    bool any_fold = false;
    for (int n = 0; n < n_nets; ++n) {
        const gnnpn_encode_net_t& e = in[n];
        GNNPN_REQUIRE(e.whh_packed && e.bhh && e.enc_out && e.h_n && e.c_n, "lstm_encode: null operand for net %d", n);
        GNNPN_REQUIRE(e.pregates || (e.inputs && e.w_in && e.b_in),
                      "lstm_encode: net %d needs pregates or (inputs, w_in, b_in)", n);
        GNNPN_REQUIRE(gnnpn_aligned(e.whh_packed, 16), "lstm_encode: packed weights must be 16-byte aligned");
        any_fold |= (e.pregates == nullptr);
        nets.pregates[n] = e.pregates;
        nets.inputs[n] = e.inputs;
        nets.w_in[n] = e.w_in;
        nets.b_in[n] = e.b_in;
        nets.whh[n] = e.whh_packed;
        GNNPN_REQUIRE(!e.whh_split || gnnpn_aligned(e.whh_split, 16), "lstm_encode: whh_split must be 16-byte aligned");
        nets.whh_split[n] = e.whh_split;
        nets.bhh[n] = e.bhh;
        nets.enc_out[n] = e.enc_out;
        nets.h_n[n] = e.h_n;
        nets.c_n[n] = e.c_n;
    }
    if (any_fold) GNNPN_REQUIRE(F == 8, "lstm_encode: in-kernel input projection is built for F = 8, got %d", F);
    if (B == 0) return GNNPN_OK;
    hipStream_t s = (hipStream_t)stream;
    const CoopOpts opts = coop_opts(opts_in);
    GNNPN_REQUIRE(opts.impl >= 0 && opts.impl <= 2, "lstm_encode: opts.impl must be 0 (auto), 1 (streaming) or 2 (cooperative, 8-member groups) — the 16-member form (3) was removed in ABI version 7");
    GNNPN_REQUIRE(opts.lds_kb >= 0 && opts.lds_kb <= 160, "lstm_encode: opts.lds_kb must be 0..160");
    const int impl = opts.impl;
    const bool coop = H == 256 && impl != 1 && (workspace != nullptr || impl >= 2);
    if (!coop && any_fold)
        GNNPN_FAIL(GNNPN_E_UNSUP, "lstm_encode: the streaming form needs precomputed pregates");
    if (precision != GNNPN_PREC_F32 && !coop)
        GNNPN_FAIL(GNNPN_E_UNSUP, "lstm_encode: fp16-operand precisions need the cooperative form (H = 256, workspace)");
    if (coop) {
        const int rc = gnnpn_launch_encode_coop(nets, n_nets, B, L, precision, opts, workspace, workspace_bytes, s);
        if (rc != GNNPN_OK) return rc;
    } else if (H == 256) {
        launch_encode<256>(nets, n_nets, B, L, s);
    } else {
        launch_encode<32>(nets, n_nets, B, L, s);
    }
    GNNPN_CHECK_LAUNCH("lstm_encode_f32");
    return GNNPN_OK;
}
```

### gnnpn-sc_amd/csrc/lstm_shared.h

```cpp
#pragma once
#include "common.h"

#define GNNPN_MAX_NETS 4

struct LstmNets {
    const float* pregates[GNNPN_MAX_NETS];
    const float* inputs[GNNPN_MAX_NETS];
    const float* w_in[GNNPN_MAX_NETS];
    const float* b_in[GNNPN_MAX_NETS];
    const float* whh[GNNPN_MAX_NETS];
    const void* whh_split[GNNPN_MAX_NETS];
    const float* bhh[GNNPN_MAX_NETS];
    float* enc_out[GNNPN_MAX_NETS];
    float* h_n[GNNPN_MAX_NETS];
    float* c_n[GNNPN_MAX_NETS];
};


struct CoopOpts {
    int impl = 0, lds_kb = 0;
    bool write_through = false, paired_start = false;
    unsigned* sticky = nullptr;
};
inline CoopOpts coop_opts(const gnnpn_launch_opts_t* o) {
    CoopOpts c;
    if (o) {
        c.impl = o->impl;
        c.lds_kb = o->lds_kb;
        c.write_through = o->write_through != 0;
        c.paired_start = o->paired_start != 0;
        c.sticky = o->sticky_status;
    }
    return c;
}

int gnnpn_launch_encode_coop(const LstmNets& nets, int n_nets, int32_t B, int32_t L, int precision, const CoopOpts& opts,
                             void* workspace, int64_t workspace_bytes, hipStream_t s);
constexpr int COOP_SEAT_TABLE_WORDS = 8 * 256 + 8 + 8;
unsigned* gnnpn_cu_seat_table();
extern thread_local int64_t g_gnnpn_last_units;
int gnnpn_option_lstm_ablate();
```

### gnnpn-sc_amd/csrc/torch_ops.cpp

```cpp
#include <ATen/ATen.h>
#include <c10/core/DeviceGuard.h>
#include <c10/hip/HIPStream.h>
#include <torch/library.h>

#include <string>
#include <vector>

#include "gnnpn_hip.h"

namespace {

using at::Tensor;
using OptTensor = std::optional<Tensor>;

#define GNNPN_ON_DEVICE_OF(t)                          \
    TORCH_CHECK((t).is_cuda(), "gnnpn: expected a CUDA tensor (the hot path has no CPU implementation)"); \
    const c10::DeviceGuard device_guard_((t).device()); \
    void* const stream_ = (void*)c10::hip::getCurrentHIPStream((t).device().index()).stream()
#define cur_stream() stream_

void check_rc(int rc, const char* what) { TORCH_CHECK(rc == GNNPN_OK, what, " failed (", rc, "): ", gnnpn_last_error()); }

template <typename T>
const T* cptr(const Tensor& t, at::ScalarType dt, const char* name) {
// ... 69 lines not shown
                                            (int)act, out_f32(y), C, (int32_t)n, (int32_t)C, (int32_t)block_rows, i32(row_order, "row_order"),
                                            cur_stream()), "gnnpn_csr_aggregate_blocks_f32");
    return y;
}
Tensor csr_aggregate_tiled(const Tensor& header, const Tensor& order, const Tensor& selfw, const Tensor& batches, const Tensor& x,
                           const OptTensor& self_coef, const OptTensor& bias, const OptTensor& scale, const OptTensor& shift, int64_t act,
                           int64_t n_rows, int64_t block_rows) {
    GNNPN_ON_DEVICE_OF(x);
    rows2d(x, "csr_aggregate_tiled.x");
    const int64_t C = x.size(1);
    Tensor y = new_f32(x, {n_rows, C});
    check_rc(gnnpn_csr_aggregate_tiled_f32(i32(header, "header"), i32(order, "order"), f32(selfw, "selfw"),
                                           cptr<uint8_t>(batches, at::kByte, "batches"), f32(x, "x"), C, f32(self_coef, "self_coef"),
                                           f32(bias, "bias"), f32(scale, "scale"), f32(shift, "shift"), (int)act, out_f32(y), C,
                                           (int32_t)n_rows, (int32_t)C, (int32_t)block_rows, cur_stream()), "gnnpn_csr_aggregate_tiled_f32");
    return y;
}

Tensor gcn_norm(const Tensor& rowptr, const Tensor& col, const Tensor& w_raw) {
    GNNPN_ON_DEVICE_OF(w_raw);
    const int64_t n = rowptr.numel() - 1;
    Tensor dis = new_f32(w_raw, {n}), norm = at::empty_like(w_raw);
    check_rc(gnnpn_gcn_norm_f32(i32(rowptr, "rowptr"), i32(col, "col"), f32(w_raw, "w_raw"), out_f32(dis), out_f32(norm), (int32_t)n,
                                cur_stream()), "gnnpn_gcn_norm_f32");
    return norm;
}

Tensor segment_mean(const Tensor& segptr, const Tensor& x) {
    GNNPN_ON_DEVICE_OF(x);
    rows2d(x, "segment_mean.x");
    const int64_t n_seg = segptr.numel() - 1, C = x.size(1);
    Tensor out = new_f32(x, {n_seg, C});
    check_rc(gnnpn_segment_mean_f32(i32(segptr, "segptr"), f32(x, "x"), C, out_f32(out), C, (int32_t)n_seg, (int32_t)C, cur_stream()),
             "gnnpn_segment_mean_f32");
    return out;
}

Tensor request_branch(const Tensor& x, const Tensor& table, const Tensor& rowptr, const Tensor& col, const Tensor& seg_ptr, int64_t max_nodes,
                      at::TensorList layer_tensors, const Tensor& lin_w_packed, const Tensor& lin_b, int64_t hidden) {
    GNNPN_ON_DEVICE_OF(x);
    rows2d(x, "request_branch.x");
    TORCH_CHECK(layer_tensors.size() % 9 == 0, "request_branch: nine tensors per layer");
    const size_t n_layers = layer_tensors.size() / 9;
    std::vector<gnnpn_gin_layer_t> layers(n_layers);
    for (size_t i = 0; i < n_layers; ++i) {
        const float* p[9];
        for (int j = 0; j < 9; ++j) p[j] = f32(layer_tensors[i * 9 + j], "request_branch.layer_tensors");
        layers[i] = gnnpn_gin_layer_t{p[0], p[1], p[2], p[3], p[4], p[5], p[6], p[7], p[8]};
    }
    const int64_t B = seg_ptr.numel() - 1;
    Tensor out = new_f32(x, {B, hidden});
    check_rc(gnnpn_request_branch_f32(f32(x, "x"), (int32_t)(x.size(1) - 1), f32(table, "table"), (int32_t)table.size(0),
                                      (int32_t)table.size(1), i32(rowptr, "rowptr"), i32(col, "col"), i32(seg_ptr, "seg_ptr"), (int32_t)B,
                                      (int32_t)max_nodes, (int32_t)n_layers, layers.data(), (int32_t)hidden, f32(lin_w_packed, "lin_w_packed"),
                                      f32(lin_b, "lin_b"), out_f32(out), cur_stream()), "gnnpn_request_branch_f32");
    return out;
}

Tensor gin_layer(const Tensor& rowptr, const Tensor& col, const Tensor& x, const Tensor& eps, const Tensor& w1, const OptTensor& b1,
                 const OptTensor& a1, const OptTensor& s1, const Tensor& w2, const OptTensor& b2, const OptTensor& a2, const OptTensor& s2,
                 const OptTensor& w3, const OptTensor& b3) {
    GNNPN_ON_DEVICE_OF(x);
    rows2d(x, "gin_layer.x");
    const int64_t n = x.size(0), c_in = x.size(1);
    const bool lin3 = w3.has_value() && w3->defined();
    TORCH_CHECK(w1.dim() == 3 && w2.dim() == 3 && (!lin3 || w3->dim() == 3) && w1.size(1) * 2 == (c_in + 31) / 32 * 32,
                "gin_layer: weights must be packed with ops.pack_mfma_b32 (and w1 for this many input channels)");
    const int64_t h1 = w1.size(0) * 32, h2 = w2.size(0) * 32, h3 = lin3 ? w3->size(0) * 32 : 0;
    Tensor out = new_f32(x, {n, lin3 ? h3 : h2});
    check_rc(gnnpn_gin_layer_f32(i32(rowptr, "rowptr"), i32(col, "col"), f32(x, "x"), c_in, (int32_t)c_in, f32(eps, "eps"), f32(w1, "w1"),
                                 f32(b1, "b1"), f32(a1, "a1"), f32(s1, "s1"), (int32_t)h1, f32(w2, "w2"), f32(b2, "b2"), f32(a2, "a2"),
                                 f32(s2, "s2"), (int32_t)h2, f32(w3, "w3"), f32(b3, "b3"), (int32_t)h3, out_f32(out), out.size(1), n,
                                 cur_stream()), "gnnpn_gin_layer_f32");
    return out;
}

Tensor gin_layer_split(const Tensor& rowptr, const Tensor& col, const Tensor& x, const Tensor& eps, const Tensor& w1, const Tensor& i1,
                       const OptTensor& b1, const OptTensor& a1, const OptTensor& s1, const Tensor& w2, const Tensor& i2, const OptTensor& b2,
                       const OptTensor& a2, const OptTensor& s2, const OptTensor& w3, const OptTensor& i3, const OptTensor& b3) {
    GNNPN_ON_DEVICE_OF(x);
    rows2d(x, "gin_layer_split.x");
    const int64_t n = x.size(0), c_in = x.size(1), k1 = (c_in + 31) / 32 * 32;
    const bool lin3 = w3.has_value() && w3->defined();
    const int64_t h1 = i1.numel(), h2 = i2.numel(), h3 = lin3 ? (i3.has_value() ? i3->numel() : 0) : 0;
    TORCH_CHECK(w1.numel() == gnnpn_split_weights_bytes((int32_t)h1, (int32_t)k1) && w2.numel() == gnnpn_split_weights_bytes((int32_t)h2, (int32_t)h1) &&
                    (!lin3 || w3->numel() == gnnpn_split_weights_bytes((int32_t)h3, (int32_t)h2)),
                "gin_layer_split: packed weights do not chain (c_in -> h1 -> h2 [-> h3]); pack with ops.pack_split_weights");
    Tensor out = new_f32(x, {n, lin3 ? h3 : h2});
    check_rc(gnnpn_gin_layer_split(i32(rowptr, "rowptr"), i32(col, "col"), f32(x, "x"), c_in, (int32_t)c_in, f32(eps, "eps"),
                                   cptr<uint8_t>(w1, at::kByte, "w1"), f32(i1, "i1"), f32(b1, "b1"), f32(a1, "a1"), f32(s1, "s1"), (int32_t)h1,
                                   cptr<uint8_t>(w2, at::kByte, "w2"), f32(i2, "i2"), f32(b2, "b2"), f32(a2, "a2"), f32(s2, "s2"), (int32_t)h2,
                                   cptr<uint8_t>(w3, at::kByte, "w3"), f32(i3, "i3"), f32(b3, "b3"), (int32_t)h3, out_f32(out), out.size(1), n,
                                   cur_stream()), "gnnpn_gin_layer_split");
    return out;
}

std::tuple<Tensor, Tensor> segment_topk_feasible(const Tensor& scores, const Tensor& cat_ptr, const Tensor& qos, const Tensor& local_bounds,
                                                 const Tensor& present, const Tensor& global_bounds, int64_t n_per) {
    GNNPN_ON_DEVICE_OF(scores);
    rows2d(scores, "select.scores");
    const int64_t B = scores.size(0), S = scores.size(1), T = cat_ptr.numel() - 1;
    TORCH_CHECK(qos.sizes() == at::IntArrayRef({S, 4}) && local_bounds.sizes() == at::IntArrayRef({B, T, 4}) &&
                    present.sizes() == at::IntArrayRef({B, T}) && global_bounds.sizes() == at::IntArrayRef({B, 4}),
                "select_candidates: inconsistent shapes");
    Tensor rows = new_f32(scores, {B, T * n_per, 8}), ids = new_i32(scores, {B, T * n_per});
    check_rc(gnnpn_select_candidates(f32(scores, "scores"), S, i32(cat_ptr, "cat_ptr"), cptr<double>(qos, at::kDouble, "qos"),
                                     cptr<double>(local_bounds, at::kDouble, "local_bounds"), cptr<uint8_t>(present, at::kByte, "present"),
                                     cptr<double>(global_bounds, at::kDouble, "global_bounds"), out_f32(rows),
                                     static_cast<int32_t*>(ids.data_ptr()), (int32_t)B, (int32_t)T, (int32_t)n_per, cur_stream()),
             "gnnpn_select_candidates");
    return {rows, ids};
}

Tensor rank_rows(const Tensor& scores) {
    GNNPN_ON_DEVICE_OF(scores);
    rows2d(scores, "rank_rows.scores");
    const int64_t B = scores.size(0), S = scores.size(1);
    Tensor ranking = new_i32(scores, {B, S});
    check_rc(gnnpn_rank_rows(f32(scores, "scores"), S, static_cast<int32_t*>(ranking.data_ptr()), (int32_t)B, (int32_t)S, cur_stream()),
             "gnnpn_rank_rows");
    return ranking;
}

Tensor precision_at_k(const Tensor& ranking, const Tensor& labels, at::IntArrayRef ks) {
    GNNPN_ON_DEVICE_OF(labels);
    const int64_t B = labels.size(0), S = labels.size(1);
    std::vector<int32_t> k32(ks.begin(), ks.end());
    Tensor kt = at::tensor(k32, at::TensorOptions().dtype(at::kInt)).to(labels.device());
    Tensor out = new_f32(labels, {B, (int64_t)ks.size()});
    check_rc(gnnpn_precision_at_k(i32(ranking, "ranking"), ranking.size(1), f32(labels, "labels"), S, (int32_t)B, (int32_t)S, i32(kt, "ks"),
                                  (int32_t)ks.size(), out_f32(out), cur_stream()), "gnnpn_precision_at_k");
    return out;
}

Tensor attention_logits(const Tensor& enc_out, const Tensor& queries, int64_t step, const Tensor& idx, double tanh_c, bool use_tanh) {
    GNNPN_ON_DEVICE_OF(enc_out);
    const int64_t B = enc_out.size(0), L = enc_out.size(1), H = enc_out.size(2), T = queries.size(1);
    f32(enc_out, "enc_out"), f32(queries, "queries");
    Tensor out = new_f32(enc_out, {B, L});
    check_rc(gnnpn_attention_logits_f32(f32(enc_out, "enc_out"), static_cast<const float*>(queries.data_ptr()) + step * H, T * H,
                                        i32(idx, "idx"), (float)tanh_c, use_tanh ? 1 : 0, out_f32(out), (int32_t)B, (int32_t)L, (int32_t)H,
                                        (int32_t)step, (int32_t)T, cur_stream()), "gnnpn_attention_logits_f32");
    return out;
}

Tensor qos_reward(const Tensor& actions, int64_t level) {
    GNNPN_ON_DEVICE_OF(actions);
    const int64_t B = actions.size(0), T = actions.size(1);
    Tensor R = new_f32(actions, {B});
    check_rc(gnnpn_qos_reward_f32(f32(actions, "actions"), out_f32(R), (int32_t)B, (int32_t)T, (int)level, cur_stream()), "gnnpn_qos_reward_f32");
    return R;
}

int precision_code(const std::string& p, const char* what) {
    if (p == "f32") return GNNPN_PREC_F32;
    if (p == "f16") return GNNPN_PREC_F16;
    if (p == "split") return GNNPN_PREC_SPLIT;
    TORCH_CHECK(false, what, ": unknown precision '", p, "'");
}
bool coop_supported(int64_t H, int64_t n_per, int64_t impl) { return H == 256 && n_per <= 16 && impl != 1; }
gnnpn_launch_opts_t launch_opts(int64_t impl, int64_t lds_kb, bool write_through, bool paired_start, const OptTensor& status) {
    gnnpn_launch_opts_t o{};
    o.impl = (int32_t)impl, o.lds_kb = (int32_t)lds_kb, o.write_through = write_through ? 1 : 0, o.paired_start = paired_start ? 1 : 0;
    TORCH_CHECK(!(status.has_value() && status->defined()) || status->numel() >= GNNPN_STATUS_WORDS,
                "status: a block of ", GNNPN_STATUS_WORDS, " int32 words (ops.Workspaces.status)");
    o.sticky_status = (status.has_value() && status->defined())
                          ? const_cast<uint32_t*>(reinterpret_cast<const uint32_t*>(cptr<int32_t>(*status, at::kInt, "status")))
                          : nullptr;
    return o;
}

std::vector<Tensor> lstm_encode(const c10::List<OptTensor>& net_tensors, int64_t n_nets, std::string precision, int64_t impl, int64_t lds_kb,
                                bool write_through, const OptTensor& workspace, const OptTensor& status, bool paired_start) {
    constexpr size_t EK = 7;
    TORCH_CHECK(n_nets >= 1 && net_tensors.size() == EK * (size_t)n_nets, "lstm_encode: seven tensors per net (custom_ops.ENCODE_KEYS)");
    std::vector<OptTensor> t(net_tensors.size());
    for (size_t i = 0; i < t.size(); ++i) t[i] = net_tensors.get(i);
    auto has = [&](size_t i) { return t[i].has_value() && t[i]->defined(); };
    TORCH_CHECK(has(5), "lstm_encode: nets[0].bhh required");
    GNNPN_ON_DEVICE_OF(*t[5]);
    const int64_t H = t[5]->numel() / 4;
    const Tensor& first = has(0) ? *t[0] : *t[1];
    TORCH_CHECK(first.dim() == 3, "lstm_encode: pregates / inputs must be [B, L, .]");
    const int64_t B = first.size(0), L = first.size(1);
    const bool coop = coop_supported(H, 1, impl);
    const int prec = precision_code(precision, "lstm_encode");
    TORCH_CHECK(prec == GNNPN_PREC_F32 || coop, "lstm_encode: precision='", precision, "' needs the cooperative form (H = 256)");
    std::vector<gnnpn_encode_net_t> nets(n_nets);
    std::vector<Tensor> enc, hn, cn, keep;
    for (int64_t i = 0; i < n_nets; ++i)
        if (has(EK * i + 6) && has(EK * i + 4)) lstm_split(*t[EK * i + 6], *t[EK * i + 4], "nets.whh_split");
    for (int64_t i = 0; i < n_nets; ++i) {
        const size_t o = EK * i;
        Tensor pre = has(o) ? *t[o] : Tensor();
        if (!pre.defined() && !coop) {
            TORCH_CHECK(has(o + 1) && has(o + 2) && has(o + 3), "lstm_encode: nets[", i, "] needs pregates or inputs + w_in + b_in");
            const Tensor& x = *t[o + 1];
            pre = linear(x.reshape({B * L, x.size(2)}), *t[o + 2], t[o + 3], std::nullopt, std::nullopt, 0).view({B, L, 4 * H});
            keep.push_back(pre);
        }
        enc.push_back(new_f32(first, {B, L, H})), hn.push_back(new_f32(first, {B, H})), cn.push_back(new_f32(first, {B, H}));
        gnnpn_encode_net_t& a = nets[i];
        a = gnnpn_encode_net_t{};
        a.pregates = pre.defined() ? f32(pre, "nets.pregates") : nullptr;
        if (!pre.defined()) {
            TORCH_CHECK(has(o + 1) && has(o + 2) && has(o + 3), "lstm_encode: nets[", i, "] needs pregates or inputs + w_in + b_in");
            a.inputs = f32(*t[o + 1], "nets.inputs"), a.w_in = f32(*t[o + 2], "nets.w_in"), a.b_in = f32(*t[o + 3], "nets.b_in");
        }
        TORCH_CHECK(has(o + 4) && has(o + 5), "lstm_encode: nets[", i, "].whh / bhh required");
        a.whh_packed = f32(*t[o + 4], "nets.whh"), a.bhh = f32(*t[o + 5], "nets.bhh");
        a.whh_split = has(o + 6) ? lstm_split(*t[o + 6], *t[o + 4], "nets.whh_split") : nullptr;
        a.enc_out = out_f32(enc.back()), a.h_n = out_f32(hn.back()), a.c_n = out_f32(cn.back());
    }
    const bool ws = coop && workspace.has_value() && workspace->defined();
    TORCH_CHECK(!coop || ws, "lstm_encode: the cooperative form (H = 256) needs a workspace (ops.Workspaces.encode())");
    const gnnpn_launch_opts_t opts = launch_opts(impl, lds_kb, write_through, paired_start, coop ? status : OptTensor());
    check_rc(gnnpn_lstm_encode_f32((int)n_nets, nets.data(), (int32_t)B, (int32_t)L, (int32_t)H, 8, prec, &opts,
                                   ws ? const_cast<uint8_t*>(cptr<uint8_t>(*workspace, at::kByte, "workspace")) : nullptr,
                                   ws ? workspace->numel() : 0, cur_stream()), "gnnpn_lstm_encode_f32");
    std::vector<Tensor> out;
    out.insert(out.end(), enc.begin(), enc.end()), out.insert(out.end(), hn.begin(), hn.end()), out.insert(out.end(), cn.begin(), cn.end());
    return out;
}

std::vector<Tensor> pointer_decode(const c10::List<OptTensor>& net_tensors, at::IntArrayRef latent_from, const Tensor& inputs, int64_t n_cat,
                                   int64_t n_per, double tanh_c, bool use_tanh, bool want_queries, std::string precision, int64_t impl,
                                   int64_t lds_kb, bool write_through, const OptTensor& workspace, const OptTensor& status,
                                   at::IntArrayRef sample_seeds, bool paired_start) {
    GNNPN_ON_DEVICE_OF(inputs);
    constexpr size_t NK = 16;
    const size_t n_nets = latent_from.size();
    TORCH_CHECK(n_nets >= 1 && n_nets <= 2 && net_tensors.size() == NK * n_nets, "pointer_decode: sixteen tensors per net (custom_ops.DECODE_KEYS), 1 or 2 nets");
    std::vector<OptTensor> t(net_tensors.size());
    for (size_t i = 0; i < t.size(); ++i) t[i] = net_tensors.get(i);
    auto has = [&](size_t i) { return t[i].has_value() && t[i]->defined(); };
    TORCH_CHECK(has(0) && t[0]->dim() == 3, "pointer_decode: nets[0].enc_out [B, L, H] required");
    const int64_t B = t[0]->size(0), L = t[0]->size(1), H = t[0]->size(2);
    const int prec = precision_code(precision, "pointer_decode");
    TORCH_CHECK(L == n_cat * n_per, "pointer_decode: seq_len ", L, " != ", n_cat, "*", n_per);
    const bool coop = coop_supported(H, n_per, impl);
    for (size_t i = 0; i < n_nets; ++i)
        if (has(NK * i + 15) && has(NK * i + 5)) lstm_split(*t[NK * i + 15], *t[NK * i + 5], "whh_split");
    std::vector<gnnpn_decode_net_t> nets(n_nets);
    std::vector<Tensor> out, keep;
    for (size_t i = 0; i < n_nets; ++i) {
        const size_t o = NK * i;
        gnnpn_decode_net_t& a = nets[i];
        a = gnnpn_decode_net_t{};
        for (size_t j = 0; j < 8; ++j) TORCH_CHECK(has(o + j), "pointer_decode: nets[", i, "] operand ", j, " required");
        a.enc_out = f32(*t[o + 0], "enc_out"), a.h0 = f32(*t[o + 1], "h0"), a.c0 = f32(*t[o + 2], "c0"), a.start = f32(*t[o + 3], "start");
        a.wih_packed = f32(*t[o + 4], "wih"), a.whh_packed = f32(*t[o + 5], "whh"), a.bih = f32(*t[o + 6], "bih"), a.bhh = f32(*t[o + 7], "bhh");
        if (has(o + 11) && coop) {
            TORCH_CHECK(has(o + 12) && has(o + 13), "pointer_decode: xw_fold needs xb_fold and start_fold");
            a.xw_fold = f32(*t[o + 11], "xw_fold"), a.xb_fold = f32(*t[o + 12], "xb_fold"), a.start_fold = f32(*t[o + 13], "start_fold");
        }
        Tensor emb = has(o + 8) ? *t[o + 8] : Tensor();
        if (!emb.defined() && !coop) {
            TORCH_CHECK(has(o + 9) && has(o + 10), "pointer_decode: nets[", i, "] needs embedded or emb_w + emb_b");
            emb = linear(inputs.reshape({B * L, inputs.size(2)}), *t[o + 9], t[o + 10], std::nullopt, std::nullopt, 0).view({B, L, H});
            keep.push_back(emb);
        }
        a.embedded = emb.defined() ? f32(emb, "embedded") : nullptr;
        if (!emb.defined()) {
            TORCH_CHECK(has(o + 9) && has(o + 10), "pointer_decode: nets[", i, "] needs embedded or emb_w + emb_b");
            a.emb_w = f32(*t[o + 9], "emb_w"), a.emb_b = f32(*t[o + 10], "emb_b");
        }
        a.latent_win = has(o + 14) ? f32(*t[o + 14], "latent_win") : nullptr;
        a.whh_split = has(o + 15) ? lstm_split(*t[o + 15], *t[o + 5], "whh_split") : nullptr;
        a.latent_from = (int32_t)latent_from[i];
        const int64_t seed = i < sample_seeds.size() ? sample_seeds[i] : -1;
        a.sample = seed >= 0 ? 1 : 0;
        a.sample_seed = seed >= 0 ? (uint64_t)seed : 0;
        Tensor idx = new_i32(inputs, {B, n_cat}), win = new_f32(inputs, {B, n_cat, n_per}), prob = new_f32(inputs, {B, n_cat});
        Tensor actions = new_f32(inputs, {B, n_cat, 8}), q = want_queries ? new_f32(inputs, {B, n_cat, H}) : new_f32(inputs, {0});
        a.idx = static_cast<int32_t*>(idx.data_ptr()), a.win_logits = out_f32(win), a.pick_prob = out_f32(prob), a.actions = out_f32(actions);
        a.queries = want_queries ? out_f32(q) : nullptr;
        out.push_back(idx), out.push_back(win), out.push_back(prob), out.push_back(actions), out.push_back(q);
    }
    const bool ws = coop && workspace.has_value() && workspace->defined();
    TORCH_CHECK(!coop || ws, "pointer_decode: the cooperative form needs a workspace (ops.Workspaces.decode(B, T, n_per))");
    const gnnpn_launch_opts_t opts = launch_opts(impl, lds_kb, write_through, paired_start, coop ? status : OptTensor());
    check_rc(gnnpn_pointer_decode_f32((int)n_nets, nets.data(), f32(inputs, "inputs"), (float)tanh_c, use_tanh ? 1 : 0, (int32_t)B, (int32_t)n_cat,
                                      (int32_t)n_per, (int32_t)H, prec == GNNPN_PREC_SPLIT ? GNNPN_PREC_SPLIT : GNNPN_PREC_F32, &opts,
                                      ws ? const_cast<uint8_t*>(cptr<uint8_t>(*workspace, at::kByte, "workspace")) : nullptr,
                                      ws ? workspace->numel() : 0, cur_stream()), "gnnpn_pointer_decode_f32");
    return out;
}

}

TORCH_LIBRARY(gnnpn, m) {
    m.def("linear(Tensor a, Tensor weight, Tensor? bias=None, Tensor? scale=None, Tensor? shift=None, int act=0) -> Tensor");
    m.def("embed_concat(Tensor x, Tensor table) -> Tensor");
    m.def("csr_aggregate(Tensor rowptr, Tensor col, Tensor? w, Tensor x, Tensor? self_coef=None, Tensor? bias=None, Tensor? scale=None, "
          "Tensor? shift=None, int act=0) -> Tensor");
    m.def("csr_aggregate_blocks(Tensor rowptr, Tensor col, Tensor? w, Tensor x, Tensor? self_coef, Tensor? bias, Tensor? scale, "
          "Tensor? shift, int act, int block_rows, Tensor? row_order=None) -> Tensor");
    m.def("csr_aggregate_tiled(Tensor header, Tensor order, Tensor selfw, Tensor batches, Tensor x, Tensor? self_coef, Tensor? bias, "
          "Tensor? scale, Tensor? shift, int act, int n_rows, int block_rows) -> Tensor");
    m.def("gcn_norm(Tensor rowptr, Tensor col, Tensor w_raw) -> Tensor");
    m.def("segment_mean(Tensor segptr, Tensor x) -> Tensor");
    m.def("request_branch(Tensor x, Tensor table, Tensor rowptr, Tensor col, Tensor seg_ptr, int max_nodes, Tensor[] layer_tensors, "
          "Tensor lin_w_packed, Tensor lin_b, int hidden) -> Tensor");
    m.def("gin_layer(Tensor rowptr, Tensor col, Tensor x, Tensor eps, Tensor w1, Tensor? b1, Tensor? a1, Tensor? s1, Tensor w2, Tensor? b2, "
          "Tensor? a2, Tensor? s2, Tensor? w3=None, Tensor? b3=None) -> Tensor");
    m.def("gin_layer_split(Tensor rowptr, Tensor col, Tensor x, Tensor eps, Tensor w1, Tensor i1, Tensor? b1, Tensor? a1, Tensor? s1, "
          "Tensor w2, Tensor i2, Tensor? b2, Tensor? a2, Tensor? s2, Tensor? w3=None, Tensor? i3=None, Tensor? b3=None) -> Tensor");
    m.def("segment_topk_feasible(Tensor scores, Tensor cat_ptr, Tensor qos, Tensor local_bounds, Tensor present, Tensor global_bounds, "
          "int n_per) -> (Tensor, Tensor)");
    m.def("rank_rows(Tensor scores) -> Tensor");
    m.def("precision_at_k(Tensor ranking, Tensor labels, int[] ks) -> Tensor");
    m.def("attention_logits(Tensor enc_out, Tensor queries, int step, Tensor idx, float tanh_c, bool use_tanh) -> Tensor");
    m.def("qos_reward(Tensor actions, int level) -> Tensor");
    m.def("lstm_encode(Tensor?[] net_tensors, int n_nets, str precision='f32', int impl=0, int lds_kb=0, bool write_through=False, "
          "Tensor? workspace=None, Tensor? status=None, bool paired_start=False) -> Tensor[]");
    m.def("pointer_decode(Tensor?[] net_tensors, int[] latent_from, Tensor inputs, int n_cat, int n_per, float tanh_c=10.0, "
          "bool use_tanh=True, bool want_queries=False, str precision='f32', int impl=0, int lds_kb=0, bool write_through=False, "
          "Tensor? workspace=None, Tensor? status=None, int[] sample_seeds=[], bool paired_start=False) -> Tensor[]");
}

TORCH_LIBRARY_IMPL(gnnpn, CUDA, m) {
    m.impl("linear", linear);
    m.impl("embed_concat", embed_concat);
    m.impl("csr_aggregate", csr_aggregate);
    m.impl("csr_aggregate_blocks", csr_aggregate_blocks);
    m.impl("csr_aggregate_tiled", csr_aggregate_tiled);
    m.impl("gcn_norm", gcn_norm);
    m.impl("segment_mean", segment_mean);
    m.impl("request_branch", request_branch);
    m.impl("gin_layer", gin_layer);
    m.impl("gin_layer_split", gin_layer_split);
    m.impl("segment_topk_feasible", segment_topk_feasible);
    m.impl("rank_rows", rank_rows);
    m.impl("precision_at_k", precision_at_k);
    m.impl("attention_logits", attention_logits);
    m.impl("qos_reward", qos_reward);
    m.impl("lstm_encode", lstm_encode);
    m.impl("pointer_decode", pointer_decode);
}
```

### gnnpn-sc_amd/custom_ops.py

```python
import os

import torch

from . import _lib, ops

DECODE_KEYS = ("enc_out", "h0", "c0", "start", "wih", "whh", "bih", "bhh", "embedded", "emb_w", "emb_b",
               "xw_fold", "xb_fold", "start_fold", "latent_win", "whh_split")
DECODE_OUTS = ("idx", "win_logits", "pick_prob", "actions", "queries")
ENCODE_KEYS = ("pregates", "inputs", "w_in", "b_in", "whh", "bhh", "whh_split")
REQUEST_LAYER_KEYS = ("w0p", "b0", "a1", "s1", "w3p", "b3", "a2", "s2", "eps")

TORCH_LIB_PATH = os.environ.get("GNNPN_TORCH_LIB") or os.path.join(os.path.dirname(os.path.abspath(__file__)), "libgnnpn_torch.so")


def _load():
    _lib.load()
    if not os.path.exists(TORCH_LIB_PATH):
        raise _lib.GnnpnError(f"{TORCH_LIB_PATH} is missing: build it with `python gnnpn-sc_amd/build.py` (the gnnpn:: operators are "
                              "registered from C++; there is no Python or CPU fallback)")
    torch.ops.load_library(TORCH_LIB_PATH)


_load()



def _gnnpn_errors(fn):
    import functools

    @functools.wraps(fn)
    def call(*a, **k):
        try:
            return fn(*a, **k)
        except _lib.GnnpnError:
            raise
        except RuntimeError as e:
            raise _lib.GnnpnError(str(e).split("\nException raised from")[0]) from None
    return call


def _coop_ws(device, H, n_per, impl, ws):
    return ops.workspaces(device, ws) if ops.coop_supported(H, n_per, impl) else None


@_gnnpn_errors
def lstm_encode(nets, precision="f32", impl=0, lds_kb=0, write_through=False, ws=None, paired_start=False):
    flat = [d.get(k) for d in nets for k in ENCODE_KEYS]
    first = nets[0]["pregates"] if nets[0].get("pregates") is not None else nets[0]["inputs"]
    wsp = _coop_ws(first.device, nets[0]["bhh"].numel() // 4, 1, impl, ws)
    out = torch.ops.gnnpn.lstm_encode(flat, len(nets), precision, impl, lds_kb, bool(write_through),
                                      None if wsp is None else wsp.encode(), None if wsp is None else wsp.status, bool(paired_start))
    if wsp is not None:
        wsp.note_launch(0, _lib.load().gnnpn_last_launch_units())
    n = len(nets)
    return out[:n], out[n:2 * n], out[2 * n:]


@_gnnpn_errors
def pointer_decode(nets, inputs, n_cat, n_per, tanh_c=10.0, use_tanh=True, want_queries=False, precision="f32", impl=0,
                   lds_kb=0, write_through=False, ws=None, paired_start=False):
    flat = [d.get(k) for d in nets for k in DECODE_KEYS]
    lf = [int(d.get("latent_from", -1)) for d in nets]
    seeds = [int(d["sample_seed"]) & 0x7FFFFFFFFFFFFFFF if d.get("sample") else -1 for d in nets]
    B, L, H = nets[0]["enc_out"].shape
    wsp = _coop_ws(inputs.device, H, n_per, impl, ws)
    out = torch.ops.gnnpn.pointer_decode(flat, lf, inputs, n_cat, n_per, float(tanh_c), bool(use_tanh), bool(want_queries),
                                         precision, impl, lds_kb, bool(write_through),
                                         None if wsp is None else wsp.decode(B, n_cat, n_per), None if wsp is None else wsp.status,
                                         seeds, bool(paired_start))
    if wsp is not None:
        wsp.note_launch(1, _lib.load().gnnpn_last_launch_units())
    m = len(DECODE_OUTS)
    res = []
    for i in range(len(nets)):
        d = dict(zip(DECODE_OUTS, out[i * m:(i + 1) * m]))
        if d["queries"].numel() == 0 and not want_queries:
            d["queries"] = None
        res.append(d)
    return res


@_gnnpn_errors
def request_branch(x, table, rowptr, col, seg_ptr, max_nodes, layers, lin_w_packed, lin_b, hidden):
    flat = [lp[k] for lp in layers for k in REQUEST_LAYER_KEYS]
    return torch.ops.gnnpn.request_branch(x, table, rowptr, col, seg_ptr, int(max_nodes), flat, lin_w_packed, lin_b, int(hidden))


@_gnnpn_errors
def csr_aggregate(rowptr, col, w, x, self_coef=None, bias=None, scale=None, shift=None, act=0, block_rows=0):
    form, aux = ops.csr_aggregate_form(rowptr, col, w, x, block_rows)
    if form == "tiled":
        return torch.ops.gnnpn.csr_aggregate_tiled(aux.header, aux.order, aux.selfw, aux.batches, x, self_coef, bias, scale, shift, act,
                                                   aux.n_rows, aux.block_rows)
    if form == "blocks":
        return torch.ops.gnnpn.csr_aggregate_blocks(rowptr, col, w, x, self_coef, bias, scale, shift, act, int(block_rows), aux)
    return torch.ops.gnnpn.csr_aggregate(rowptr, col, w, x, self_coef, bias, scale, shift, act)
```

### gnnpn-sc_amd/modelPN.py

```python
import math

import os

import torch
from torch import nn

from . import custom_ops, ops

FOLD_INPUT_PROJECTION = True

qosandcons = 8
qosNum = 4
consNum = 2


class LatentWindows:

    def __init__(self, win, idx, enc_out, queries, tanh_c, use_tanh, bahdanau=None):
        self.win, self.idx = win, idx
        self._enc_out, self._queries = enc_out, queries
        self._tanh_c, self._use_tanh = tanh_c, use_tanh
        self._bahdanau, self._ref = bahdanau, None

    def __len__(self):
        return self.win.shape[1]

    def __getitem__(self, k):
        if isinstance(k, slice):
            return [self[i] for i in range(*k.indices(len(self)))]
        if k < 0:
            k += len(self)
        if self._bahdanau is not None:
            from . import ops
            a = {n: v.detach().float().contiguous() for n, v in self._bahdanau.items()}
            B, L, H = self._enc_out.shape
            if self._ref is None:
                self._ref = ops.linear(self._enc_out.reshape(B * L, H), a["wref"].reshape(H, H).contiguous(), a["bref"]).view(B, L, H)
            qp = ops.linear(self._queries[:, k, :].contiguous(), a["wq"], a["bq"])
            return ops.attention_logits_bahdanau(self._ref, qp, a["v"], k, self.idx, self._tanh_c, self._use_tanh)
        return torch.ops.gnnpn.attention_logits(self._enc_out, self._queries, k, self.idx, self._tanh_c, self._use_tanh)

    def __iter__(self):
        return (self[k] for k in range(len(self)))

    def copy(self):
        return self


def _window_tensor(latent, n_cat, n_per):
    if latent is None:
        return None
    if isinstance(latent, LatentWindows):
        return latent.win
    if len(latent) != n_cat:
        raise ValueError(f"latent has {len(latent)} steps, expected {n_cat}")
    return torch.stack([latent[k][:, k * n_per:(k + 1) * n_per] for k in range(n_cat)], 1).contiguous()


class Attention(nn.Module):

    def __init__(self, hidden_size, use_tanh=False, C=10, name="Bahdanau", use_cuda=True):
        super().__init__()
        if name not in ops.ATTENTION_NAMES:
            raise NotImplementedError(name)
        self.use_tanh, self.C, self.name = use_tanh, C, name
        if name == "Bahdanau":
            self.W_query = nn.Linear(hidden_size, hidden_size)
            self.W_ref = nn.Conv1d(hidden_size, hidden_size, 1, 1)
            self.V = nn.Parameter(torch.FloatTensor(hidden_size))
            self.V.data.uniform_(-(1. / math.sqrt(hidden_size)), 1. / math.sqrt(hidden_size))

    def side(self):
        if self.name != "Bahdanau":
            return None
        return {"wq": self.W_query.weight, "bq": self.W_query.bias, "wref": self.W_ref.weight, "bref": self.W_ref.bias,
                "v": self.V}


class PointerNet(nn.Module):

    def __init__(self, embedding_size, hidden_size, seq_len, n_glimpses, tanh_exploration, use_tanh, attention,
                 sNumber, sCategory, use_cuda=True, level="low", mask=False):
        super().__init__()
        if n_glimpses < 0:
            raise ValueError("n_glimpses >= 0")
        self.embedding_size, self.hidden_size, self.n_glimpses = embedding_size, hidden_size, n_glimpses
        self.attention = attention
        self.general = attention != "Dot" or n_glimpses != 0
        self.seq_len, self.use_cuda, self.level = seq_len, use_cuda, level
        self.serNumber, self.serCategory = sNumber, sCategory
        self.C, self.use_tanh, self.mask = float(tanh_exploration), bool(use_tanh), mask
        if embedding_size != 0:
            self.embedding1 = nn.Embedding(sCategory, embedding_size)
        self.embedding2 = nn.Linear(embedding_size + qosandcons, hidden_size)
        self.encoder = nn.LSTM(hidden_size, hidden_size, batch_first=True)
        self.decoder = nn.LSTM(hidden_size, hidden_size, batch_first=True)
        self.pointer = Attention(hidden_size, use_tanh=use_tanh, C=tanh_exploration, name=attention, use_cuda=use_cuda)
        self.glimpse = Attention(hidden_size, use_tanh=False, name=attention, use_cuda=use_cuda)
        self.decoder_start_input = nn.Parameter(torch.FloatTensor(hidden_size))
        self.decoder_start_input.data.uniform_(-(1. / math.sqrt(hidden_size)), 1. / math.sqrt(hidden_size))
        self._packed = None
        self.fold_on_device = False
        self.sample_seed = int(torch.initial_seed()) & 0x7FFFFFFF
        self.sample_calls = 0

    def next_sample_seed(self):
        self.sample_calls += 1
        return (self.sample_seed * 1000003 + self.sample_calls) & 0x7FFFFFFFFFFFFFFF

    def _load_from_state_dict(self, *a, **k):
        self._packed = None
        return super()._load_from_state_dict(*a, **k)

    def _apply(self, fn, *a, **k):
        self._packed = None
        return super()._apply(fn, *a, **k)

    def packed(self):
        if self._packed is None:
            f = lambda t: t.detach().float().contiguous()
            self._packed = {
                "emb_w": f(self.embedding2.weight), "emb_b": f(self.embedding2.bias),
                "enc_wih": f(self.encoder.weight_ih_l0), "enc_bih": f(self.encoder.bias_ih_l0),
                "enc_whh": ops.pack_lstm_weight(f(self.encoder.weight_hh_l0)), "enc_bhh": f(self.encoder.bias_hh_l0),
                "dec_wih": ops.pack_lstm_weight(f(self.decoder.weight_ih_l0)), "dec_bih": f(self.decoder.bias_ih_l0),
                "dec_whh": ops.pack_lstm_weight(f(self.decoder.weight_hh_l0)), "dec_bhh": f(self.decoder.bias_hh_l0),
                "start": f(self.decoder_start_input),
            }
            if self.hidden_size == 256 and self.embedding2.weight.is_cuda and not torch.cuda.is_current_stream_capturing():
                self._packed["enc_whh_split"] = ops.pack_lstm_split_weights(self._packed["enc_whh"])
                self._packed["dec_whh_split"] = ops.pack_lstm_split_weights(self._packed["dec_whh"])
            if self.embedding_size != 0:
                self._packed["whh_absmax"] = None
                return self._packed
            where = (lambda t: t.detach().double()) if self.fold_on_device else (lambda t: t.detach().double().cpu())
            dev = self.embedding2.weight.device
            back = lambda t: t.float().contiguous().to(dev)
            w_ih, w_e, b_e = where(self.encoder.weight_ih_l0), where(self.embedding2.weight), where(self.embedding2.bias)
            self._packed["enc_wfold"] = back(w_ih @ w_e)
            self._packed["enc_bfold"] = back(w_ih @ b_e + where(self.encoder.bias_ih_l0))
            d_ih, d_b = where(self.decoder.weight_ih_l0), where(self.decoder.bias_ih_l0)
            self._packed["dec_wfold"] = back(d_ih @ w_e)
            self._packed["dec_bfold"] = back(d_ih @ b_e + d_b)
            self._packed["dec_sfold"] = back(d_ih @ where(self.decoder_start_input) + d_b)
            self._packed["whh_absmax"] = None
        return self._packed

    def check_precision(self, precision):
        if precision == "f16":
            w = self.packed()
            if w["whh_absmax"] is None:
                w["whh_absmax"] = float(max(self.encoder.weight_hh_l0.detach().abs().max(),
                                            self.decoder.weight_hh_l0.detach().abs().max()))
            m = w["whh_absmax"]
            if not m < 6.0e4:
                raise ops.GnnpnError(f"precision={precision!r}: max |W_hh| = {m:g} does not fit fp16 operands; use 'f32' or 'split'")

    def encode_args(self, inputs, fold=None):
        B, L, F = inputs.shape
        assert L == self.seq_len
        w = self.packed()
        fold = FOLD_INPUT_PROJECTION if fold is None else fold
# ... 25 lines not shown
        if sample_seed is not None:
            d.update(sample=True, sample_seed=int(sample_seed))
        return d

    @torch.no_grad()
    def run(self, inputs, latent=None, want_queries=False, fold=None, sample_seed=None, encoder_precision="f32"):
        inputs = inputs.contiguous()
        enc_args, embedded = self.encode_args(inputs, fold)
        enc, h_n, c_n = custom_ops.lstm_encode([enc_args], precision=encoder_precision)
        impl = 0
        if self.embedding_size != 0:
            rows9, inputs = inputs, inputs[:, :, 1:].contiguous()
            fold = False
            if sample_seed is not None:
                impl = 1
        if self.general:
            out = ops.pointer_decode_attn(
                self.decode_args(embedded, enc[0], h_n[0], c_n[0], _window_tensor(latent, self.serCategory, self.serNumber),
                                 fold=False, sample_seed=sample_seed),
                inputs, self.serCategory, self.serNumber, self.attention, self.n_glimpses, self.pointer.side(),
                self.glimpse.side(), self.C, self.use_tanh, want_queries)
            out["enc_out"] = enc[0]
            return self._with_category(out, rows9) if self.embedding_size != 0 else out
        out = custom_ops.pointer_decode(
            [self.decode_args(embedded, enc[0], h_n[0], c_n[0],
                              _window_tensor(latent, self.serCategory, self.serNumber), fold=fold, sample_seed=sample_seed)],
            inputs, self.serCategory, self.serNumber, self.C, self.use_tanh, want_queries, impl=impl)[0]
        out["enc_out"] = enc[0]
        return self._with_category(out, rows9) if self.embedding_size != 0 else out

    @staticmethod
    def _with_category(out, rows9):
        cat = torch.gather(rows9[:, :, 0], 1, out["idx"].long()).unsqueeze(-1)
        out["actions"] = torch.cat([cat, out["actions"]], dim=2)
        return out

    def forward(self, inputs, latent, sample="sample"):
        out = self.run(inputs, latent, want_queries=True,
                       sample_seed=None if sample == "greedy" else self.next_sample_seed())
        lat = LatentWindows(out["win_logits"], out["idx"], out["enc_out"], out["queries"], self.C, self.use_tanh, self.pointer.side())
        idxs = [out["idx"][:, k].long() for k in range(self.serCategory)]
        return _ProbList(out, latent, self.serCategory, self.serNumber), idxs, lat


class _ProbList:

    def __init__(self, out, latent, n_cat, n_per):
        win = out["win_logits"]
        lw = _window_tensor(latent, n_cat, n_per)
        self._p = torch.softmax(win if lw is None else win + lw, dim=2)
        self._n_per, self._L = n_per, n_cat * n_per

    def __len__(self):
        return self._p.shape[1]

    def __getitem__(self, k):
        B = self._p.shape[0]
        full = torch.zeros((B, self._L), dtype=self._p.dtype, device=self._p.device)
        full[:, k * self._n_per:(k + 1) * self._n_per] = self._p[:, k]
        return full

    def __iter__(self):
        return (self[k] for k in range(len(self)))


def calc(services, constraints, sCategory):
    rows = torch.stack([torch.as_tensor(s)[:qosNum].float().cpu() for s in services]).unsqueeze(0)
    act = torch.zeros((1, rows.shape[1], 8), dtype=torch.float32)
    act[0, :, :qosNum] = rows[0]
    for i in range(consNum):
        act[0, 0, qosNum + 2 * i], act[0, 0, qosNum + 2 * i + 1] = constraints[i][0][-2], constraints[i][0][-1]
    dev = torch.device("cuda")
    violate = int(torch.ops.gnnpn.qos_reward(act.to(dev), 0).item())
    total = float(torch.ops.gnnpn.qos_reward(act.to(dev), 1).item())
    return violate, total - violate, []


def reward(sample_solution, optSolutions, sCategory, USE_CUDA=False, level="Low", embedding_size=20,
           verbose=False):
    actions = torch.stack(list(sample_solution), dim=1)
    if actions.shape[-1] == 1 + qosandcons:
        actions = actions[..., 1:]
    actions = actions.contiguous()
    R = torch.ops.gnnpn.qos_reward(actions, 0 if level == "Low" else 1)
    if verbose:
        lst = R.tolist()
        print(f"{level}, {sum(1 for v in lst if v >= 1)}, {sum(lst) / max(len(lst), 1)}: ", lst)
    return R


class CombinatorialRL(nn.Module):

    def __init__(self, embedding_size, hidden_size, seq_len, n_glimpses, tanh_exploration, use_tanh, reward,
                 attention, sNumber, sCategory, use_cuda=True, level="Low", mask=False):
        super().__init__()
        self.reward = reward
        self.use_cuda, self.level, self.embedding_size = use_cuda, level, embedding_size
        self.sNumber, self.serCategory = sNumber, sCategory
        self.actor = PointerNet(embedding_size, hidden_size, seq_len, n_glimpses, tanh_exploration, use_tanh,
                                attention, sNumber, sCategory, use_cuda, level=level, mask=mask)

    @torch.no_grad()
    def forward(self, inputs, labs, latent=None, sample="sample", training="RL"):
        out = self.actor.run(inputs, latent, want_queries=True,
                             sample_seed=None if sample == "greedy" else self.actor.next_sample_seed())
        T = self.serCategory
        action_idxs = [out["idx"][:, k].long() for k in range(T)]
        actions = [out["actions"][:, k, :] for k in range(T)]
        action_probs = [out["pick_prob"][:, k] for k in range(T)]
        latent_p = LatentWindows(out["win_logits"], out["idx"], out["enc_out"], out["queries"], self.actor.C,
                                 self.actor.use_tanh, self.actor.pointer.side())
        if training == "RL":
            R = self.reward(actions, labs, self.serCategory, USE_CUDA=self.use_cuda, level=self.level,
                            embedding_size=self.embedding_size)
            return R, action_probs, actions, action_idxs, latent_p
        return (_ProbList(out, latent, T, self.sNumber), action_probs, actions, action_idxs, latent_p)


@torch.no_grad()
def default_precision(low, high, fold=None, sampling=False, decode_impl=0):
    la, ha = low.actor, high.actor
    fits = all(a.hidden_size == 256 and a.serNumber <= 16 and a.embedding_size == 0 and not a.general for a in (la, ha))
    folded = FOLD_INPUT_PROJECTION if fold is None else bool(fold)
    return "split" if fits and folded and not sampling and decode_impl != 1 else "f32"


def two_level_greedy(low, high, inputs, fold=None, precision=None, decode_impl=0, lds_kb=0, write_through=False, ws=None,
                     sample_high_seed=None, paired_start=False):
    inputs = inputs.contiguous()
    la, ha = low.actor, high.actor
    if precision is None:
        precision = default_precision(low, high, fold, sample_high_seed is not None, decode_impl)
    if la.general or ha.general or la.embedding_size != 0 or ha.embedding_size != 0:
        dl = la.run(inputs, None, fold=fold, encoder_precision=precision)
        dh = ha.run(inputs, LatentWindows(dl["win_logits"], dl["idx"], None, None, la.C, la.use_tanh), fold=fold,
                    sample_seed=sample_high_seed, encoder_precision=precision)
        R = torch.ops.gnnpn.qos_reward(dh["actions"][..., -qosandcons:].contiguous(), 0 if high.level == "Low" else 1)
        return {"idx_low": dl["idx"], "idx_high": dh["idx"], "R": R, "actions": dh["actions"],
                "action_probs": dh["pick_prob"], "win_low": dl["win_logits"], "win_high_raw": dh["win_logits"]}
    for name in ("C", "use_tanh", "serNumber", "serCategory", "hidden_size", "seq_len"):
        if getattr(la, name) != getattr(ha, name):
            raise ops.GnnpnError(f"two_level_greedy: Low and High nets differ in {name} ({getattr(la, name)!r} vs "
                                 f"{getattr(ha, name)!r}); decode them with separate CombinatorialRL.forward calls")
    return _two_level_fused(low, high, inputs, fold, precision, decode_impl, lds_kb, write_through, ws, sample_high_seed,
                            paired_start)[0]


def _two_level_fused(low, high, inputs, fold, precision, decode_impl, lds_kb, write_through, ws, sample_high_seed, paired_start):
    la, ha = low.actor, high.actor
    la.check_precision(precision)
    ha.check_precision(precision)
    enc_l, emb_l = la.encode_args(inputs, fold)
    enc_h, emb_h = ha.encode_args(inputs, fold)
    enc, h_n, c_n = custom_ops.lstm_encode([enc_l, enc_h], precision=precision, lds_kb=lds_kb, write_through=write_through, ws=ws,
                                           paired_start=paired_start)
    del enc_l, enc_h
    dl, dh = custom_ops.pointer_decode([la.decode_args(emb_l, enc[0], h_n[0], c_n[0], fold=fold),
                                 ha.decode_args(emb_h, enc[1], h_n[1], c_n[1], latent_from=0, fold=fold,
                                                sample_seed=sample_high_seed)],
                                inputs, la.serCategory, la.serNumber, la.C, la.use_tanh,
                                precision="split" if precision == "split" else "f32", impl=decode_impl, lds_kb=lds_kb,
                                write_through=write_through, ws=ws, paired_start=paired_start)
    R = torch.ops.gnnpn.qos_reward(dh["actions"], 0 if high.level == "Low" else 1)
    return ({"idx_low": dl["idx"], "idx_high": dh["idx"], "R": R, "actions": dh["actions"],
             "action_probs": dh["pick_prob"], "win_low": dl["win_logits"], "win_high_raw": dh["win_logits"]},
            (enc[1], h_n[1], c_n[1], emb_h))


def fresh_seed():
    return int.from_bytes(os.urandom(8), "little") & 0x7FFFFFFFFFFFFFFF


def two_level_best_of(low, high, inputs, samples, seed=None, precision=None, fold=None, decode_impl=0, lds_kb=0, write_through=False,
                      ws=None):
    samples = int(samples)
    if samples < 1:
        raise ops.GnnpnError(f"two_level_best_of: samples must be >= 1, got {samples}")
    seed = fresh_seed() if seed is None else int(seed)
    inputs = inputs.contiguous()
    la, ha = low.actor, high.actor
    B = inputs.shape[0]
    T, K = ha.serCategory, ha.serNumber
    level = 0 if high.level == "Low" else 1
    general = la.general or ha.general or la.embedding_size != 0 or ha.embedding_size != 0
    if general:
        g = two_level_greedy(low, high, inputs, fold=fold, precision=precision, decode_impl=decode_impl, lds_kb=lds_kb,
                             write_through=write_through, ws=ws)
        if precision is None:
            precision = default_precision(low, high, fold, False, decode_impl)
        rep = None
        if samples > 1:
            lat = LatentWindows(g["win_low"], g["idx_low"], None, None, la.C, la.use_tanh)
            outs = [ha.run(inputs, lat, fold=fold, sample_seed=ops.replica_seed(seed, j), encoder_precision=precision)
                    for j in range(1, samples)]
            rep = {"idx": torch.stack([o["idx"] for o in outs], 1).contiguous(),
                   "actions": torch.stack([o["actions"] for o in outs], 1).contiguous(),
                   "pick_prob": torch.stack([o["pick_prob"] for o in outs], 1).contiguous()}
    else:
        if precision is None:
            precision = default_precision(low, high, fold, False, decode_impl)
        g, (enc_h, h_h, c_h, emb_h) = _two_level_fused(low, high, inputs, fold, precision, decode_impl, lds_kb, write_through, ws,
                                                        None, False)
        rep = None
        if samples > 1:
            net = ha.decode_args(emb_h, enc_h, h_h, c_h, latent_win=g["win_low"], fold=fold)
            rep = ops.pointer_decode_replicas(net, inputs, T, K, samples - 1, seed, first=1, tanh_c=ha.C, use_tanh=ha.use_tanh,
                                              impl=decode_impl, lds_kb=lds_kb, write_through=write_through, ws=ws)
    sam = None
    if rep is not None:
        act = rep["actions"]
        R_s = torch.ops.gnnpn.qos_reward(act[..., -qosandcons:].reshape(B * (samples - 1), T, qosandcons).contiguous(), level)
        sam = {"R": R_s.view(B, samples - 1), "idx": rep["idx"], "actions": act, "probs": rep["pick_prob"]}
    sel = _select(g, sam, g["actions"].shape[-1])
    if ops.coop_supported(ha.hidden_size, K, decode_impl):
        ops.workspaces(inputs.device, ws).check()
    out = dict(g)
    out.update(idx_high=sel["idx"], R=sel["R"], actions=sel["actions"], action_probs=sel["probs"], sample_index=sel["winner"])
    if sam is None:
        out["R_all"] = g["R"].unsqueeze(1).clone()
        out["idx_all"] = g["idx_high"].unsqueeze(1).clone()
    else:
        out["R_all"] = torch.cat([g["R"].unsqueeze(1), sam["R"]], 1)
        out["idx_all"] = torch.cat([g["idx_high"].unsqueeze(1), sam["idx"]], 1)
    return out


def _select(g, sam, width):
    greedy = {"R": g["R"], "idx": g["idx_high"], "actions": g["actions"][..., -qosandcons:].contiguous(), "probs": g["action_probs"]}
    s = None if sam is None else dict(sam, actions=sam["actions"][..., -qosandcons:].contiguous())
    sel = ops.best_of_select(greedy, s)
    if width != qosandcons:
        cat0 = g["actions"][..., :1]
        cats = cat0.unsqueeze(1) if sam is None else torch.cat([cat0.unsqueeze(1), sam["actions"][..., :1]], 1)
        w = sel["winner"].long()
        pick = torch.gather(cats, 1, w.view(-1, 1, 1, 1).expand(-1, 1, cats.shape[2], 1)).squeeze(1)
        sel["actions"] = torch.cat([pick, sel["actions"]], 2)
    return sel
```

### include/gnnpn_hip.h

```cpp
#ifndef GNNPN_HIP_H
#define GNNPN_HIP_H

#include <stdint.h>

#ifdef __cplusplus
extern "C" {
#endif

#define GNNPN_ABI_VERSION 9

#define GNNPN_OK 0
#define GNNPN_E_ARG (-1)
#define GNNPN_E_UNSUP (-2)
#define GNNPN_E_LAUNCH (-3)

#define GNNPN_ACT_NONE 0
#define GNNPN_ACT_RELU 1
#define GNNPN_ACT_SIGMOID 2

int gnnpn_abi_version(void);
const char* gnnpn_last_error(void);

int gnnpn_linear_f32(const float* A, int64_t lda, const float* W, int64_t ldw, const float* bias,
                     const float* scale, const float* shift, int act, float* C, int64_t ldc,
                     int64_t M, int N, int K, void* stream);

int gnnpn_embed_concat_f32(const float* x, const float* table, int vocab, int emb, int nfeat,
                           float* out, int64_t n_rows, void* stream);

int gnnpn_csr_aggregate_f32(const int32_t* rowptr, const int32_t* col, const float* w,
                            const float* x, int64_t ldx, const float* self_coef, const float* bias,
                            const float* scale, const float* shift, int act, float* y, int64_t ldy,
                            int32_t n_rows, int32_t C, void* stream);

int gnnpn_csr_aggregate_blocks_f32(const int32_t* rowptr, const int32_t* col, const float* w,
                                   const float* x, int64_t ldx, const float* self_coef, const float* bias,
                                   const float* scale, const float* shift, int act, float* y, int64_t ldy,
                                   int32_t n_rows, int32_t C, int32_t block_rows, const int32_t* row_order, void* stream);

int gnnpn_csr_block_row_order(const int32_t* rowptr, int32_t n_rows, int32_t block_rows, int32_t* row_order, void* stream);

typedef struct gnnpn_tile_plan_geom {
    int32_t n_blocks;
    int32_t src_tiles;
    int32_t src_tile_rows;
    int32_t dst_tiles;
    int32_t dst_tile_rows;
    int32_t units;
    int32_t wavefronts;
    int32_t passes;
    int64_t header_bytes;
    int64_t order_bytes;
    int64_t tstart_bytes;
    int64_t selfw_bytes;
    int64_t meta_bytes;
} gnnpn_tile_plan_geom_t;
int gnnpn_csr_tile_plan_geometry(int32_t n_rows, int32_t block_rows, gnnpn_tile_plan_geom_t* out);
int gnnpn_csr_tile_plan_rows(const int32_t* rowptr, const int32_t* col, const float* w, int32_t n_rows, int32_t block_rows,
                             int32_t* header, int32_t* order, int32_t* tstart, float* selfw, int32_t* meta, void* stream);
int gnnpn_csr_tile_plan_fill(const int32_t* col, const float* w, int32_t n_rows, int32_t block_rows, const int32_t* header,
                             const int32_t* order, const int32_t* tstart, void* batches, int64_t n_quads, void* stream);
int gnnpn_csr_aggregate_tiled_f32(const int32_t* header, const int32_t* order, const float* selfw, const void* batches,
                                  const float* x, int64_t ldx, const float* self_coef, const float* bias,
                                  const float* scale, const float* shift, int act, float* y, int64_t ldy,
                                  int32_t n_rows, int32_t C, int32_t block_rows, void* stream);

int gnnpn_gcn_norm_f32(const int32_t* rowptr, const int32_t* col, const float* w_raw,
                       float* deg_inv_sqrt, float* norm, int32_t n_rows, void* stream);

int gnnpn_segment_mean_f32(const int32_t* segptr, const float* x, int64_t ldx, float* out,
                           int64_t ldo, int32_t n_seg, int32_t C, void* stream);

int gnnpn_gin_layer_f32(const int32_t* rowptr, const int32_t* col, const float* x, int64_t ldx, int32_t c_in, const float* eps,
                        const float* w1, const float* b1, const float* bn1_scale, const float* bn1_shift, int32_t h1,
                        const float* w2, const float* b2, const float* bn2_scale, const float* bn2_shift, int32_t h2,
                        const float* w3, const float* b3, int32_t h3, float* out, int64_t ldo, int64_t n_rows, void* stream);

int64_t gnnpn_split_weights_bytes(int32_t n_out, int32_t k);
int gnnpn_pack_split_weights_f16(const float* w, int64_t ldw, int32_t n_out, int32_t k, void* packed, float* col_inv, void* stream);
int gnnpn_gin_layer_split(const int32_t* rowptr, const int32_t* col, const float* x, int64_t ldx, int32_t c_in, const float* eps,
                          const void* w1, const float* inv1, const float* b1, const float* bn1_scale, const float* bn1_shift, int32_t h1,
                          const void* w2, const float* inv2, const float* b2, const float* bn2_scale, const float* bn2_shift, int32_t h2,
                          const void* w3, const float* inv3, const float* b3, int32_t h3, float* out, int64_t ldo, int64_t n_rows,
                          void* stream);

typedef struct {
    const float* w0_packed;
    const float* b0;
    const float* bn1_scale;
    const float* bn1_shift;
    const float* w3_packed;
    const float* b3;
    const float* bn2_scale;
    const float* bn2_shift;
    const float* eps;
} gnnpn_gin_layer_t;
int gnnpn_request_branch_f32(const float* x, int32_t nfeat, const float* table, int32_t vocab, int32_t emb,
                             const int32_t* rowptr, const int32_t* col, const int32_t* seg_ptr, int32_t n_graphs,
                             int32_t max_nodes, int32_t n_layers, const gnnpn_gin_layer_t* layers, int32_t hidden,
                             const float* lin_w_packed, const float* lin_b, float* out, void* stream);

int gnnpn_select_candidates(const float* scores, int64_t ld_scores, const int32_t* cat_ptr,
                            const double* qos, const double* local_bounds,
                            const uint8_t* present, const double* global_bounds, float* out_rows,
                            int32_t* out_ids, int32_t B, int32_t T, int32_t n_per, void* stream);

int gnnpn_rank_rows(const float* scores, int64_t ld_scores, int32_t* ranking, int32_t B, int32_t S,
                    void* stream);

int gnnpn_precision_at_k(const int32_t* ranking, int64_t ld_rank, const float* labels, int64_t ld_lab,
                         int32_t B, int32_t S, const int32_t* ks, int32_t n_k, float* out, void* stream);

typedef struct {
    const float* pregates;
    const float* inputs;
    const float* w_in;
    const float* b_in;
    const float* whh_packed;
    const float* bhh;
    float* enc_out;
    float* h_n;
    float* c_n;
    const void* whh_split;
} gnnpn_encode_net_t;

#define GNNPN_PREC_F32 0
#define GNNPN_PREC_F16 1
#define GNNPN_PREC_SPLIT 2

#define GNNPN_STATUS_WORDS 8
#define GNNPN_STATUS_CODE 0
#define GNNPN_STATUS_DECLINED_SEATS 1
#define GNNPN_STATUS_OFF_CANONICAL_SEATS 2
#define GNNPN_STATUS_ENC_EXPECTED 4
#define GNNPN_STATUS_ENC_FINISHED 5
#define GNNPN_STATUS_DEC_EXPECTED 6
#define GNNPN_STATUS_DEC_FINISHED 7
#define GNNPN_COOP_ENC_TIMEOUT 1
#define GNNPN_COOP_DEC_TIMEOUT 2
#define GNNPN_COOP_MEMBER_MISSING 4
#define GNNPN_COOP_DIRTY 8
#define GNNPN_COOP_SHORTFALL 16
typedef struct {
    int32_t impl;
    int32_t lds_kb;
    int32_t write_through;
    int32_t paired_start;
    uint32_t* sticky_status;
} gnnpn_launch_opts_t;

int64_t gnnpn_lstm_split_weights_bytes(void);
int gnnpn_lstm_pack_split_weights_f32(const float* whh_packed, void* split, void* stream);

int gnnpn_lstm_encode_f32(int n_nets, const gnnpn_encode_net_t* nets, int32_t B, int32_t L, int32_t H,
                          int32_t F, int32_t precision, const gnnpn_launch_opts_t* opts, void* workspace,
                          int64_t workspace_bytes, void* stream);

int64_t gnnpn_lstm_encode_workspace_bytes(void);

int gnnpn_lds_footprint_kb(int kb);

int64_t gnnpn_last_launch_units(void);

int gnnpn_set_option(const char* name, int value);

int gnnpn_decode_diag(uint32_t* out, int32_t n_words, int32_t clear);
int gnnpn_coop_reset_staffing(void);
int gnnpn_coop_staffing_count(void);

typedef struct {
    const float* embedded;
    const float* enc_out;
    const float* h0;
    const float* c0;
    const float* start;
    const float* wih_packed;
    const float* whh_packed;
    const float* bih;
    const float* bhh;
    const float* latent_win;
    const float* emb_w;
    const float* emb_b;
    const float* xw_fold;
    const float* xb_fold;
    const float* start_fold;
    int32_t* idx;
    float* win_logits;
    float* pick_prob;
    float* actions;
    float* queries;
    int32_t latent_from;
    int32_t sample;
    uint64_t sample_seed;
    const void* whh_split;
} gnnpn_decode_net_t;

int gnnpn_pointer_decode_f32(int n_nets, const gnnpn_decode_net_t* nets, const float* inputs,
                             float tanh_c, int use_tanh, int32_t B, int32_t T, int32_t n_per, int32_t H,
                             int32_t precision, const gnnpn_launch_opts_t* opts, void* workspace,
                             int64_t workspace_bytes, void* stream);

typedef struct {
    int32_t attention;
    int32_t n_glimpses;
    const float* pointer_wq;
    const float* pointer_bq;
    const float* pointer_ref;
    const float* pointer_v;
    const float* glimpse_wq;
    const float* glimpse_bq;
    const float* glimpse_ref;
    const float* glimpse_v;
} gnnpn_attention_t;

int gnnpn_pointer_decode_attn_f32(const gnnpn_decode_net_t* net, const gnnpn_attention_t* attn, const float* inputs,
                                  float tanh_c, int use_tanh, int32_t B, int32_t T, int32_t n_per, int32_t H, void* stream);

int64_t gnnpn_pointer_decode_workspace_bytes(int32_t B, int32_t T, int32_t n_per);

int gnnpn_pointer_decode_replicas_f32(const gnnpn_decode_net_t* net, const float* inputs, float tanh_c, int use_tanh, int32_t B,
                                      int32_t R, int32_t first, uint64_t seed, int32_t T, int32_t n_per, int32_t H,
                                      const gnnpn_launch_opts_t* opts, void* workspace, int64_t workspace_bytes, void* stream);
uint64_t gnnpn_replica_seed(uint64_t seed, int32_t replica);

int gnnpn_best_of_select_f32(int32_t B, int32_t N, int32_t T, const float* R0, const int32_t* idx0, const float* actions0,
                             const float* probs0, const float* Rs, const int32_t* idxs, const float* actionss, const float* probss,
                             float* R_out, int32_t* idx_out, float* actions_out, float* probs_out, int32_t* winner, void* stream);

int gnnpn_attention_logits_f32(const float* enc_out, const float* queries, int64_t ld_q,
                               const int32_t* masked_idx, float tanh_c, int use_tanh, float* logits,
                               int32_t B, int32_t L, int32_t H, int32_t n_masked, int32_t ld_idx,
                               void* stream);
int gnnpn_attention_logits_bahdanau_f32(const float* ref, const float* qp, int64_t ld_q, const float* v,
                                        const int32_t* masked_idx, float tanh_c, int use_tanh, float* logits,
                                        int32_t B, int32_t L, int32_t H, int32_t n_masked, int32_t ld_idx, void* stream);

int gnnpn_qos_reward_f32(const float* actions, float* R, int32_t B, int32_t T, int level,
                         void* stream);

typedef struct {
    const float* embedded;
    const float* enc_out;
    const float* h0;
    const float* c0;
    const float* start;
    const float* wih;
    const float* whh;
    const float* bih;
    const float* bhh;
    const float* latent_win;
    const int32_t* idx;
    float* x_all;
    float* gates_pre;
    float* c_all;
    float* h_all;
    float* z0;
    float* probs;
    float* logp;
} gnnpn_decode_train_t;
int gnnpn_gemm_f32(const float* A, int64_t lda, int a_kmajor, const float* B, int64_t ldb, int b_kmajor, float* C,
                   int64_t ldc, int64_t M, int N, int K, int split_k, void* stream);
int gnnpn_lstm_train_forward_f32(const float* pregates, const float* whh, const float* bhh, float* enc_out,
                                 float* gates_pre, float* c_all, int32_t B, int32_t L, int32_t H, void* stream);
int gnnpn_decode_train_forward_f32(const gnnpn_decode_train_t* t, int32_t B, int32_t T, int32_t n_per, int32_t H,
                                   float tanh_c, int use_tanh, void* stream);
int gnnpn_decode_train_backward_f32(const gnnpn_decode_train_t* t, const float* gscale, float* d_enc_out, float* dgates,
                                    float* dx, float* dh0, float* dc0, int32_t B, int32_t T, int32_t n_per, int32_t H,
                                    float tanh_c, int use_tanh, void* stream);
int gnnpn_lstm_train_backward_f32(const float* whh, const float* gates_pre, const float* c_all, const float* d_enc_out,
                                  const float* dh0, const float* dc0, float* dgates, int32_t B, int32_t L, int32_t H,
                                  void* stream);

typedef struct {
    gnnpn_decode_train_t base;
    int32_t bahdanau;
    int32_t n_glimpses;
    const float* p_wq_t;
    const float* p_wq;
    const float* p_bq;
    const float* p_v;
    const float* p_ref;
    const float* g_wq_t;
    const float* g_wq;
    const float* g_bq;
    const float* g_v;
    const float* g_ref;
    float* q_all;
    float* a_all;
    float* d_p_ref;
    float* d_g_ref;
    float* d_p_qp;
    float* d_g_qp;
    float* d_p_v;
    float* d_g_v;
} gnnpn_decode_attn_train_t;
int gnnpn_decode_attn_train_forward_f32(const gnnpn_decode_attn_train_t* t, int32_t B, int32_t T, int32_t n_per, int32_t H,
                                        float tanh_c, int use_tanh, void* stream);
int gnnpn_decode_attn_train_backward_f32(const gnnpn_decode_attn_train_t* t, const float* gscale, float* d_enc_out, float* dgates,
                                         float* dx, float* dh0, float* dc0, int32_t B, int32_t T, int32_t n_per, int32_t H,
                                         float tanh_c, int use_tanh, void* stream);
int gnnpn_colsum_f32(const float* X, int64_t ld, int64_t rows, int32_t cols, float* out, void* stream);
int gnnpn_colsum_chunks_f32(const float* X, int64_t ld, int64_t rows, int32_t cols, int64_t rows_per_chunk, float* partial,
                            void* stream);
int gnnpn_scatter_dx_f32(const float* dx, const int32_t* idx, float* d_embedded, int32_t B, int32_t T, int32_t L, int32_t H,
                         void* stream);
int gnnpn_sumsq_f32(const float* x, int64_t n, double* accum, void* stream);
int gnnpn_adam_step_f32(float* p, const float* g, float* m, float* v, int64_t n, const double* grad_sumsq,
                        float max_grad_norm, float lr, float beta1, float beta2, float eps, int32_t step, void* stream);

int gnnpn_debug_cell_activations(const float* x, float* sig, float* th, int64_t n, void* stream);

int gnnpn_gate_wait(const void* flag, uint32_t expect, int32_t timeout_us, void* stream);

int gnnpn_debug_lds_interferer(int32_t n_workgroups, int32_t lds_bytes, int32_t hold_us, void* stream);

int gnnpn_debug_mfma_f16(const float* A, const float* B, const float* C, float* D, void* stream);

int gnnpn_eswoa_f64(int32_t P, int32_t T, const int32_t* cand_ptr, const int32_t* len_init, const double* cand,
                    const double* bounds, const int32_t* start_pos, int32_t pop, int32_t max_iter, const uint64_t* seeds,
                    int32_t max_cand, double* best_fitness, int32_t* best_pos, double* history, int64_t* draws,
                    void* stream);

int64_t gnnpn_eswoa_wide_workspace_bytes(int32_t P, int32_t T, int32_t pop);
int gnnpn_eswoa_wide_f64(int32_t P, int32_t T, const int32_t* cand_ptr, const int32_t* len_init, const double* cand,
                         const double* bounds, const int32_t* start_pos, int32_t pop, int32_t max_iter, const uint64_t* seeds,
                         void* workspace, int64_t workspace_bytes, double* best_fitness, int32_t* best_pos, double* history,
                         int64_t* draws, void* stream);

int64_t gnnpn_eswoa_ragged_workspace_bytes(int32_t n_lists, int32_t max_slots, int32_t pop, int32_t wide);
int gnnpn_eswoa_ragged_f64(int32_t B, const int32_t* prob_ptr, int32_t n_lists, int32_t max_slots, int32_t max_cand,
                           const int32_t* cand_ptr, const int32_t* len_init, const double* cand, const double* bounds,
                           const int32_t* start_pos, int32_t pop, int32_t max_iter, const uint64_t* seeds, int32_t wide,
                           void* workspace, int64_t workspace_bytes, double* best_fitness, int32_t* best_pos, double* best_rows,
                           double* history, int64_t* draws, void* stream);

#define GNNPN_WOA_OK 0
#define GNNPN_WOA_ROWS_MISMATCH 1
#define GNNPN_WOA_INDEX_ERROR 2
#define GNNPN_WOA_NO_SLOTS 3
int64_t gnnpn_woa_candidates_workspace_bytes(int32_t B, int32_t n_nodes, int32_t max_cat_size);
int gnnpn_woa_candidates_count(int32_t B, int32_t n_nodes, const float* x, int32_t x_ld, const int32_t* seg_ptr,
                               const double* local_bounds, const double* global_bounds, int32_t n_cat, const int32_t* cat_ptr,
                               const double* qos, const void* actions, int32_t actions_f64, int32_t actions_T, double reduct,
                               const double* patches, int32_t n_patches, int32_t max_cat_size, void* workspace,
                               int64_t workspace_bytes, int32_t* prob_ptr, int32_t* n_slots, double* bounds, int32_t* status,
                               int32_t* totals, void* stream);
int gnnpn_woa_candidates_fill(int32_t B, int32_t n_nodes, const int32_t* seg_ptr, const int32_t* cat_ptr, const double* qos,
                              int32_t max_cat_size, const void* workspace, int64_t workspace_bytes, const int32_t* status,
                              const int32_t* prob_ptr, int32_t n_lists, int32_t n_cand, int32_t* cand_ptr, int32_t* len_init,
                              double* cand, int32_t* start_pos, void* stream);
int gnnpn_debug_round5_f64(const double* x, double* y, int64_t n, void* stream);

int gnnpn_bn_train_forward_f32(const float* x, int64_t rows, int32_t cols, const float* gamma, const float* beta, float eps,
                               float momentum, int relu, float* y, float* xhat, float* invstd, float* running_mean,
                               float* running_var, void* stream);
int gnnpn_bn_train_backward_f32(const float* dy, const float* y, const float* xhat, const float* gamma, const float* invstd,
                                int64_t rows, int32_t cols, int relu, float* dx, float* dgamma, float* dbeta, void* stream);
int gnnpn_bce_sigmoid_f32(const float* p, const float* y, int64_t n, float* dz, float* loss, void* stream);
int gnnpn_dot_f32(const float* a, const float* b, int64_t n, float* out, void* stream);
int gnnpn_embed_grad_f32(const float* dh, int64_t ldh, const float* x, int64_t ldx, int64_t rows, int32_t c, int32_t vocab,
                         float* dtable, void* stream);

int gnnpn_split3_pieces_f32(const float* x, int64_t n, int32_t scale_log2, uint16_t* p0, uint16_t* p1, uint16_t* p2, void* stream);
int gnnpn_recurrent_product_f32(const float* whh_packed, const float* h, int32_t precision, float* gates, float* col_inv,
                                void* stream);

#ifdef __cplusplus
}
#endif
#endif
```

Measured before the change: 478,800.

## Fold decode workspace zeroing into encode launch and fuse pick-prob with reward

The encoder's workspace-zeroing kernel now also zeroes the next decode launch's workspace, so the decoder can skip its own zeroing launch. The decoder's separate pick-probability kernel is also dropped and its per-row work is folded into the QoS reward kernel as one step-tail launch. Both aim to cut kernel launches and small serial kernels per inference step. The cost is coupling between the encode, decode and tail stages, which must agree on workspace layout and flags, and it only applies on the greedy, folded, cooperative path.

```diff
diff --git a/gnnpn-sc_amd/_lib.py b/gnnpn-sc_amd/_lib.py
--- a/gnnpn-sc_amd/_lib.py
+++ b/gnnpn-sc_amd/_lib.py
@@ -44,6 +44,8 @@
     "gnnpn_rank_rows": (c_int, [_P, c_int64, _P, c_int32, c_int32, _P]),
     "gnnpn_precision_at_k": (c_int, [_P, c_int64, _P, c_int64, c_int32, c_int32, _P, c_int32, _P, _P]),
     "gnnpn_lstm_encode_f32": (c_int, [c_int, _P, c_int32, c_int32, c_int32, c_int32, c_int32, _P, _P, c_int64, _P]),
+    "gnnpn_lstm_encode_step_f32": (c_int, [c_int, _P, c_int32, c_int32, c_int32, c_int32, c_int32, _P, _P, c_int64, _P, c_int64, c_int32,
+                                           c_int32, _P]),
     "gnnpn_lstm_encode_workspace_bytes": (c_int64, []),
     "gnnpn_set_option": (c_int, [c_char_p, c_int]),
     "gnnpn_decode_diag": (c_int, [_P, c_int32, c_int32]),
@@ -58,6 +60,9 @@
     "gnnpn_embed_grad_f32": (c_int, [_P, c_int64, _P, c_int64, c_int64, c_int32, c_int32, _P, _P]),
     "gnnpn_pointer_decode_f32": (c_int, [c_int, _P, _P, c_float, c_int, c_int32, c_int32, c_int32, c_int32, c_int32,
                                          _P, _P, c_int64, _P]),
+    "gnnpn_pointer_decode_step_f32": (c_int, [c_int, _P, _P, c_float, c_int, c_int32, c_int32, c_int32, c_int32, c_int32,
+                                              _P, _P, c_int64, c_int32, _P]),
+    "gnnpn_step_tail_f32": (c_int, [_P, _P, _P, _P, _P, _P, c_int32, c_int32, c_int32, c_int, _P]),
     "gnnpn_pointer_decode_workspace_bytes": (c_int64, [c_int32, c_int32, c_int32]),
     "gnnpn_pointer_decode_replicas_f32": (c_int, [_P, _P, c_float, c_int, c_int32, c_int32, c_int32, ctypes.c_uint64, c_int32, c_int32,
                                                   c_int32, _P, _P, c_int64, _P]),
diff --git a/gnnpn-sc_amd/csrc/coop_common.h b/gnnpn-sc_amd/csrc/coop_common.h
--- a/gnnpn-sc_amd/csrc/coop_common.h
+++ b/gnnpn-sc_amd/csrc/coop_common.h
@@ -97,20 +97,26 @@
 
 namespace {
 __global__ __launch_bounds__(256) void coop_zero_kernel(unsigned long long* __restrict__ p, size_t n8, unsigned* __restrict__ sticky,
-                                                        int word, unsigned expected, int skip_zeroing) {
-    if (sticky && blockIdx.x == 0 && threadIdx.x == 0) atomicAdd(sticky + word, expected);
+                                                        int word, unsigned expected, int skip_zeroing,
+                                                        unsigned long long* __restrict__ also, size_t also_n8, int also_word,
+                                                        unsigned also_expected) {
+    if (sticky && blockIdx.x == 0 && threadIdx.x == 0) {
+        atomicAdd(sticky + word, expected);
+        if (also) atomicAdd(sticky + also_word, also_expected);
+    }
     if (skip_zeroing) return;
-    for (size_t i = blockIdx.x * (size_t)blockDim.x + threadIdx.x; i < n8; i += (size_t)gridDim.x * blockDim.x)
-        __hip_atomic_store(p + i, 0ull, __ATOMIC_RELAXED, __HIP_MEMORY_SCOPE_AGENT);
+    for (size_t i = blockIdx.x * (size_t)blockDim.x + threadIdx.x; i < n8 + also_n8; i += (size_t)gridDim.x * blockDim.x)
+        __hip_atomic_store(i < n8 ? p + i : also + (i - n8), 0ull, __ATOMIC_RELAXED, __HIP_MEMORY_SCOPE_AGENT);
 }
 }
 inline hipError_t coop_zero_workspace(void* workspace, size_t bytes, hipStream_t s, unsigned* sticky, int word, unsigned expected,
-                                      bool skip_zeroing = false) {
-    const size_t n8 = bytes / 8;
-    unsigned blocks = skip_zeroing ? 1u : (unsigned)((n8 + 255) / 256);
+                                      bool skip_zeroing = false, void* also = nullptr, size_t also_bytes = 0, int also_word = 0,
+                                      unsigned also_expected = 0) {
+    const size_t n8 = bytes / 8, also_n8 = also ? also_bytes / 8 : 0;
+    unsigned blocks = skip_zeroing ? 1u : (unsigned)((n8 + also_n8 + 255) / 256);
     if (blocks > 2048) blocks = 2048;
     hipLaunchKernelGGL(coop_zero_kernel, dim3(blocks), dim3(256), 0, s, static_cast<unsigned long long*>(workspace), n8, sticky, word,
-                       expected, skip_zeroing ? 1 : 0);
+                       expected, skip_zeroing ? 1 : 0, static_cast<unsigned long long*>(also), also_n8, also_word, also_expected);
     return hipGetLastError();
 }
 
@@ -145,8 +151,10 @@
     L.seats = gnnpn_cu_seat_table();
     if (!L.seats) GNNPN_FAIL(GNNPN_E_LAUNCH, "%s: cannot allocate the seat table", who);
     const unsigned units = (unsigned)(COOP_G * n_nets * L.n_tiles);
-    if (coop_zero_workspace(workspace, (size_t)bytes, s, opts.sticky, expected_word, units, (gnnpn_option_lstm_ablate() & 0x2000) != 0) !=
-        hipSuccess)
+    const bool keep_dirty = (gnnpn_option_lstm_ablate() & 0x2000) != 0;
+    if (!opts.ws_clean &&
+        coop_zero_workspace(workspace, (size_t)bytes, s, opts.sticky, expected_word, units, keep_dirty, opts.also_ws, (size_t)opts.also_bytes,
+                            opts.also_word, opts.also_units) != hipSuccess)
         GNNPN_FAIL(GNNPN_E_LAUNCH, "%s: workspace memset failed", who);
     g_gnnpn_last_units = opts.sticky ? (int64_t)units : 0;
     L.status = static_cast<unsigned*>(workspace);
diff --git a/gnnpn-sc_amd/csrc/decode.hip b/gnnpn-sc_amd/csrc/decode.hip
--- a/gnnpn-sc_amd/csrc/decode.hip
+++ b/gnnpn-sc_amd/csrc/decode.hip
@@ -129,15 +129,16 @@
 #undef GNNPN_LAUNCH_DEC
 }
 
-extern "C" int gnnpn_pointer_decode_f32(int n_nets, const gnnpn_decode_net_t* nets, const float* inputs,
-                                        float tanh_c, int use_tanh, int32_t B, int32_t T, int32_t n_per, int32_t H,
-                                        int32_t precision, const gnnpn_launch_opts_t* opts_in, void* workspace,
-                                        int64_t workspace_bytes, void* stream) {
+static int pointer_decode(int n_nets, const gnnpn_decode_net_t* nets, const float* inputs, float tanh_c, int use_tanh, int32_t B,
+                          int32_t T, int32_t n_per, int32_t H, int32_t precision, const gnnpn_launch_opts_t* opts_in, void* workspace,
+                          int64_t workspace_bytes, int32_t flags, void* stream) {
     g_gnnpn_last_units = 0;
     GNNPN_REQUIRE(B >= 0 && T > 0, "pointer_decode: bad shape");
     if (B == 0) return GNNPN_OK;
     GNNPN_REQUIRE(nets && inputs, "pointer_decode: null input");
-    const CoopOpts opts = coop_opts(opts_in);
+    CoopOpts opts = coop_opts(opts_in);
+    opts.ws_clean = (flags & GNNPN_DECODE_WORKSPACE_CLEAN) != 0;
+    opts.no_pick_prob = (flags & GNNPN_DECODE_NO_PICK_PROB) != 0;
     GNNPN_REQUIRE(opts.impl >= 0 && opts.impl <= 4 && opts.impl != 3, "pointer_decode: opts.impl must be 0 (auto), 1 (streaming), 2 (cooperative, 8-CU groups) or 4 (8-CU groups, 256-register build) — the 16-CU-group form (3) was removed in ABI version 7");
     GNNPN_REQUIRE(opts.lds_kb >= 0 && opts.lds_kb <= 160, "pointer_decode: opts.lds_kb must be 0..160");
     GNNPN_REQUIRE(precision == GNNPN_PREC_F32 || precision == GNNPN_PREC_SPLIT, "pointer_decode: precision must be GNNPN_PREC_F32 or GNNPN_PREC_SPLIT, got %d", precision);
@@ -171,9 +172,15 @@
         GNNPN_FAIL(GNNPN_E_UNSUP, "pointer_decode: sampling is built in the streaming and the 8-CU-group fp32 forms (impl 0-2, "
                    "GNNPN_PREC_F32)");
     const int impl = opts.impl;
+    if (flags) {
+        bool lean = impl != 1 && gnnpn_decode_coop_supported(H, n_per) && workspace != nullptr && n_per <= 16 && !any_sample;
+        for (int n = 0; n < n_nets; ++n) lean = lean && nets[n].xw_fold != nullptr;
+        if (!lean)
+            GNNPN_FAIL(GNNPN_E_UNSUP, "pointer_decode_step: the step flags need the cooperative form with the folded input side and greedy picks");
+    }
     if (impl != 1 && gnnpn_decode_coop_supported(H, n_per) && (workspace != nullptr || impl >= 2)) {
         const int rc = gnnpn_launch_decode_coop(args, n_nets, precision, impl == 4, opts, workspace, workspace_bytes, s);
-        const bool fall_through = rc == GNNPN_E_UNSUP && impl == 0 && precision == GNNPN_PREC_F32;
+        const bool fall_through = rc == GNNPN_E_UNSUP && impl == 0 && precision == GNNPN_PREC_F32 && !flags;
         if (rc != GNNPN_OK && !fall_through) return rc;
         if (fall_through) {
             static std::atomic<bool> said{false};
@@ -195,6 +202,21 @@
     }
     GNNPN_CHECK_LAUNCH("pointer_decode_f32");
     return GNNPN_OK;
+}
+
+extern "C" int gnnpn_pointer_decode_f32(int n_nets, const gnnpn_decode_net_t* nets, const float* inputs,
+                                        float tanh_c, int use_tanh, int32_t B, int32_t T, int32_t n_per, int32_t H,
+                                        int32_t precision, const gnnpn_launch_opts_t* opts_in, void* workspace,
+                                        int64_t workspace_bytes, void* stream) {
+    return pointer_decode(n_nets, nets, inputs, tanh_c, use_tanh, B, T, n_per, H, precision, opts_in, workspace, workspace_bytes, 0, stream);
+}
+
+extern "C" int gnnpn_pointer_decode_step_f32(int n_nets, const gnnpn_decode_net_t* nets, const float* inputs, float tanh_c, int use_tanh,
+                                             int32_t B, int32_t T, int32_t n_per, int32_t H, int32_t precision,
+                                             const gnnpn_launch_opts_t* opts_in, void* workspace, int64_t workspace_bytes, int32_t flags,
+                                             void* stream) {
+    GNNPN_REQUIRE((flags & ~(GNNPN_DECODE_WORKSPACE_CLEAN | GNNPN_DECODE_NO_PICK_PROB)) == 0, "pointer_decode_step: unknown flag in %d", flags);
+    return pointer_decode(n_nets, nets, inputs, tanh_c, use_tanh, B, T, n_per, H, precision, opts_in, workspace, workspace_bytes, flags, stream);
 }
 
 extern "C" uint64_t gnnpn_replica_seed(uint64_t seed, int32_t replica) {
@@ -340,11 +362,8 @@
     return GNNPN_OK;
 }
 
-__global__ __launch_bounds__(256) void qos_reward_kernel(const float* __restrict__ actions, float* __restrict__ R, int32_t B,
-                                                        int32_t T, int level) {
+__device__ __forceinline__ void qos_reward_wave(const float* __restrict__ actions, float* __restrict__ R, int b, int32_t T, int level) {
     const int lane = threadIdx.x & 63;
-    const int b = blockIdx.x * 4 + (threadIdx.x >> 6);
-    if (b >= B) return;
     const float* a = actions + (int64_t)b * T * 8;
     const float lo0 = a[4], hi0 = a[5], lo1 = a[6], hi1 = a[7];
     float prod2 = 1.0f, prod3 = 1.0f, mn = INFINITY;
@@ -400,14 +419,42 @@
     R[b] = (float)(rint(v * 1e5) / 1e5);
 }
 
+__global__ __launch_bounds__(256) void qos_reward_kernel(const float* __restrict__ actions, float* __restrict__ R, int32_t B,
+                                                        int32_t T, int level, const float* __restrict__ win,
+                                                        const float* __restrict__ lat, const int32_t* __restrict__ idx,
+                                                        float* __restrict__ pick_prob, int32_t K) {
+    const int b = blockIdx.x * 4 + (threadIdx.x >> 6);
+    if (b >= B) return;
+    if (win) {
+        for (int t = threadIdx.x & 63; t < T; t += 64) {
+            const int64_t row = (int64_t)b * T + t;
+            pick_prob[row] = pick_prob_row(win, lat, idx, row, t, K);
+        }
+    }
+    qos_reward_wave(actions, R, b, T, level);
+}
+
 extern "C" int gnnpn_qos_reward_f32(const float* actions, float* R, int32_t B, int32_t T, int level,
                                     void* stream) {
     GNNPN_REQUIRE(B >= 0 && T > 0 && (level == 0 || level == 1), "qos_reward: bad argument");
     if (B == 0) return GNNPN_OK;
     GNNPN_REQUIRE(actions && R, "qos_reward: null operand");
     hipLaunchKernelGGL(qos_reward_kernel, dim3((B + 3) / 4), dim3(256), 0, (hipStream_t)stream, actions, R, B, T,
-                       level);
+                       level, (const float*)nullptr, (const float*)nullptr, (const int32_t*)nullptr, (float*)nullptr, 0);
     GNNPN_CHECK_LAUNCH("qos_reward_f32");
+    return GNNPN_OK;
+}
+
+extern "C" int gnnpn_step_tail_f32(const float* win_logits, const float* latent_win, const int32_t* idx, const float* actions,
+                                   float* pick_prob, float* R, int32_t B, int32_t T, int32_t n_per, int level, void* stream) {
+    GNNPN_REQUIRE(B >= 0 && T > 0 && (level == 0 || level == 1), "step_tail: bad argument");
+    GNNPN_REQUIRE(n_per >= 1 && n_per <= 16, "step_tail: n_per must be in [1,16] (the windows of the cooperative decoder), got %d", n_per);
+    if (B == 0) return GNNPN_OK;
+    GNNPN_REQUIRE(win_logits && idx && actions && pick_prob && R, "step_tail: null operand");
+    GNNPN_REQUIRE(gnnpn_aligned(actions, 16), "step_tail: actions must be 16-byte aligned");
+    hipLaunchKernelGGL(qos_reward_kernel, dim3((B + 3) / 4), dim3(256), 0, (hipStream_t)stream, actions, R, B, T, level, win_logits,
+                       latent_win, idx, pick_prob, n_per);
+    GNNPN_CHECK_LAUNCH("step_tail_f32");
     return GNNPN_OK;
 }
 
diff --git a/gnnpn-sc_amd/csrc/decode_lean.hip b/gnnpn-sc_amd/csrc/decode_lean.hip
--- a/gnnpn-sc_amd/csrc/decode_lean.hip
+++ b/gnnpn-sc_amd/csrc/decode_lean.hip
@@ -453,26 +453,7 @@
     if (row >= rows) return;
     const unsigned t_base = (unsigned)__builtin_amdgcn_readfirstlane((int)((blockIdx.x * 256ll) % T));
     const int t = (int)((t_base + threadIdx.x) % (unsigned)T);
-    float v[16];
-#pragma unroll
-    for (int j = 0; j < 16; ++j) {
-        v[j] = 0.0f;
-        if (j < K) {
-            v[j] = win[row * K + j];
-            if (lat) v[j] = __fadd_rn(v[j], lat[row * K + j]);
-        }
-    }
-    const int pick_r = min(max(idx[row] - t * K, 0), 15);
-    float best = v[0];
-#pragma unroll
-    for (int j = 1; j < 16; ++j) best = j == pick_r ? v[j] : best;
-#pragma unroll
-    for (int j = 0; j < 16; ++j) v[j] = j < K ? expf(__fsub_rn(v[j], best)) : 0.0f;
-#pragma unroll
-    for (int n = 8; n >= 1; n >>= 1)
-#pragma unroll
-        for (int j = 0; j < n; ++j) v[j] = __fadd_rn(v[j], v[j + n]);
-    out[row] = 1.0f / v[0];
+    out[row] = pick_prob_row(win, lat, idx, row, t, K);
 }
 
 static DecodeWorkspace lean_workspace(int64_t groups, int64_t rows, int32_t T, int32_t K) {
@@ -517,6 +498,7 @@
     else GNNPN_LEAN(false, 1, 2);
 #undef GNNPN_LEAN
     if (hipGetLastError() != hipSuccess) GNNPN_FAIL(GNNPN_E_LAUNCH, "pointer_decode: launch of the cooperative kernel failed");
+    if (opts.no_pick_prob) return GNNPN_OK;
     const int64_t rows = (int64_t)args.B * args.T;
     for (int n0 = 0; n0 < n_nets; n0 += 2) {
         PickProbArgs pa = {};
diff --git a/gnnpn-sc_amd/csrc/decode_shared.h b/gnnpn-sc_amd/csrc/decode_shared.h
--- a/gnnpn-sc_amd/csrc/decode_shared.h
+++ b/gnnpn-sc_amd/csrc/decode_shared.h
@@ -93,6 +93,30 @@
     return best_r;
 }
 
+__device__ __forceinline__ float pick_prob_row(const float* __restrict__ win, const float* __restrict__ lat,
+                                               const int32_t* __restrict__ idx, int64_t row, int t, int K) {
+    float v[16];
+#pragma unroll
+    for (int j = 0; j < 16; ++j) {
+        v[j] = 0.0f;
+        if (j < K) {
+            v[j] = win[row * K + j];
+            if (lat) v[j] = __fadd_rn(v[j], lat[row * K + j]);
+        }
+    }
+    const int pick_r = min(max(idx[row] - t * K, 0), 15);
+    float best = v[0];
+#pragma unroll
+    for (int j = 1; j < 16; ++j) best = j == pick_r ? v[j] : best;
+#pragma unroll
+    for (int j = 0; j < 16; ++j) v[j] = j < K ? expf(__fsub_rn(v[j], best)) : 0.0f;
+#pragma unroll
+    for (int n = 8; n >= 1; n >>= 1)
+#pragma unroll
+        for (int j = 0; j < n; ++j) v[j] = __fadd_rn(v[j], v[j + n]);
+    return 1.0f / v[0];
+}
+
 #define GNNPN_MAX_DECODE_NETS 2
 
 struct DecodeArgs {
diff --git a/gnnpn-sc_amd/csrc/lstm.hip b/gnnpn-sc_amd/csrc/lstm.hip
--- a/gnnpn-sc_amd/csrc/lstm.hip
+++ b/gnnpn-sc_amd/csrc/lstm.hip
@@ -73,9 +73,9 @@
     return 0;
 }
 
-extern "C" int gnnpn_lstm_encode_f32(int n_nets, const gnnpn_encode_net_t* in, int32_t B, int32_t L, int32_t H,
-                                     int32_t F, int32_t precision, const gnnpn_launch_opts_t* opts_in, void* workspace,
-                                     int64_t workspace_bytes, void* stream) {
+static int lstm_encode(int n_nets, const gnnpn_encode_net_t* in, int32_t B, int32_t L, int32_t H, int32_t F, int32_t precision,
+                       const gnnpn_launch_opts_t* opts_in, void* workspace, int64_t workspace_bytes, void* also, int64_t also_bytes,
+                       int32_t also_nets, int32_t also_rows, void* stream) {
     GNNPN_REQUIRE(n_nets >= 1 && n_nets <= GNNPN_MAX_NETS, "lstm_encode: n_nets must be 1..%d", GNNPN_MAX_NETS);
     GNNPN_REQUIRE(in, "lstm_encode: null net array");
     GNNPN_REQUIRE(B >= 0 && L > 0, "lstm_encode: bad shape");
@@ -107,11 +107,18 @@
     if (any_fold) GNNPN_REQUIRE(F == 8, "lstm_encode: in-kernel input projection is built for F = 8, got %d", F);
     if (B == 0) return GNNPN_OK;
     hipStream_t s = (hipStream_t)stream;
-    const CoopOpts opts = coop_opts(opts_in);
+    CoopOpts opts = coop_opts(opts_in);
+    if (also) {
+        GNNPN_REQUIRE(also_bytes > 0 && also_bytes % 16 == 0 && gnnpn_aligned(also, 256) && also_nets >= 1 && also_nets <= GNNPN_MAX_NETS && also_rows > 0,
+                      "lstm_encode_step: the next launch's workspace must be 256-byte aligned, a multiple of 16 bytes, for 1..%d nets", GNNPN_MAX_NETS);
+        opts.also_ws = also, opts.also_bytes = also_bytes, opts.also_word = GNNPN_STATUS_DEC_EXPECTED;
+        opts.also_units = 8u * (unsigned)also_nets * (unsigned)((also_rows + 15) / 16);
+    }
     GNNPN_REQUIRE(opts.impl >= 0 && opts.impl <= 2, "lstm_encode: opts.impl must be 0 (auto), 1 (streaming) or 2 (cooperative, 8-member groups) — the 16-member form (3) was removed in ABI version 7");
     GNNPN_REQUIRE(opts.lds_kb >= 0 && opts.lds_kb <= 160, "lstm_encode: opts.lds_kb must be 0..160");
     const int impl = opts.impl;
     const bool coop = H == 256 && impl != 1 && (workspace != nullptr || impl >= 2);
+    if (also && !coop) GNNPN_FAIL(GNNPN_E_UNSUP, "lstm_encode_step: zeroing the next launch's workspace needs the cooperative form");
     if (!coop && any_fold)
         GNNPN_FAIL(GNNPN_E_UNSUP, "lstm_encode: the streaming form needs precomputed pregates");
     if (precision != GNNPN_PREC_F32 && !coop)
@@ -127,3 +134,18 @@
     GNNPN_CHECK_LAUNCH("lstm_encode_f32");
     return GNNPN_OK;
 }
+
+extern "C" int gnnpn_lstm_encode_f32(int n_nets, const gnnpn_encode_net_t* in, int32_t B, int32_t L, int32_t H,
+                                     int32_t F, int32_t precision, const gnnpn_launch_opts_t* opts_in, void* workspace,
+                                     int64_t workspace_bytes, void* stream) {
+    return lstm_encode(n_nets, in, B, L, H, F, precision, opts_in, workspace, workspace_bytes, nullptr, 0, 0, 0, stream);
+}
+
+extern "C" int gnnpn_lstm_encode_step_f32(int n_nets, const gnnpn_encode_net_t* in, int32_t B, int32_t L, int32_t H, int32_t F,
+                                          int32_t precision, const gnnpn_launch_opts_t* opts_in, void* workspace, int64_t workspace_bytes,
+                                          void* next_workspace, int64_t next_workspace_bytes, int32_t next_nets, int32_t next_rows,
+                                          void* stream) {
+    GNNPN_REQUIRE(next_workspace, "lstm_encode_step: null next_workspace (gnnpn_lstm_encode_f32 is the call without one)");
+    return lstm_encode(n_nets, in, B, L, H, F, precision, opts_in, workspace, workspace_bytes, next_workspace, next_workspace_bytes,
+                       next_nets, next_rows, stream);
+}
diff --git a/gnnpn-sc_amd/csrc/lstm_shared.h b/gnnpn-sc_amd/csrc/lstm_shared.h
--- a/gnnpn-sc_amd/csrc/lstm_shared.h
+++ b/gnnpn-sc_amd/csrc/lstm_shared.h
@@ -21,6 +21,12 @@
     int impl = 0, lds_kb = 0;
     bool write_through = false, paired_start = false;
     unsigned* sticky = nullptr;
+    void* also_ws = nullptr;
+    int64_t also_bytes = 0;
+    int also_word = 0;
+    unsigned also_units = 0;
+    bool ws_clean = false;
+    bool no_pick_prob = false;
 };
 inline CoopOpts coop_opts(const gnnpn_launch_opts_t* o) {
     CoopOpts c;
diff --git a/gnnpn-sc_amd/csrc/torch_ops.cpp b/gnnpn-sc_amd/csrc/torch_ops.cpp
--- a/gnnpn-sc_amd/csrc/torch_ops.cpp
+++ b/gnnpn-sc_amd/csrc/torch_ops.cpp
@@ -245,6 +245,21 @@
     return R;
 }
 
+std::tuple<Tensor, Tensor> step_tail(const Tensor& win_logits, const OptTensor& latent_win, const Tensor& idx, const Tensor& actions,
+                                     int64_t level) {
+    GNNPN_ON_DEVICE_OF(actions);
+    TORCH_CHECK(win_logits.dim() == 3 && actions.dim() == 3 && actions.size(2) == 8, "step_tail: win_logits [B,T,K], actions [B,T,8]");
+    const int64_t B = win_logits.size(0), T = win_logits.size(1), K = win_logits.size(2);
+    TORCH_CHECK(actions.size(0) == B && actions.size(1) == T && idx.numel() == B * T, "step_tail: idx [B,T] and actions [B,T,8] must match win_logits");
+    const bool lat = latent_win.has_value() && latent_win->defined();
+    TORCH_CHECK(!lat || latent_win->numel() == B * T * K, "step_tail: latent_win must have win_logits' shape");
+    Tensor prob = new_f32(actions, {B, T}), R = new_f32(actions, {B});
+    check_rc(gnnpn_step_tail_f32(f32(win_logits, "win_logits"), lat ? f32(*latent_win, "latent_win") : nullptr, i32(idx, "idx"),
+                                 f32(actions, "actions"), out_f32(prob), out_f32(R), (int32_t)B, (int32_t)T, (int32_t)K, (int)level,
+                                 cur_stream()), "gnnpn_step_tail_f32");
+    return {prob, R};
+}
+
 int precision_code(const std::string& p, const char* what) {
     if (p == "f32") return GNNPN_PREC_F32;
     if (p == "f16") return GNNPN_PREC_F16;
@@ -264,7 +279,8 @@
 }
 
 std::vector<Tensor> lstm_encode(const c10::List<OptTensor>& net_tensors, int64_t n_nets, std::string precision, int64_t impl, int64_t lds_kb,
-                                bool write_through, const OptTensor& workspace, const OptTensor& status, bool paired_start) {
+                                bool write_through, const OptTensor& workspace, const OptTensor& status, bool paired_start,
+                                const OptTensor& next_workspace, int64_t next_nets, int64_t next_rows) {
     constexpr size_t EK = 7;
     TORCH_CHECK(n_nets >= 1 && net_tensors.size() == EK * (size_t)n_nets, "lstm_encode: seven tensors per net (custom_ops.ENCODE_KEYS)");
     std::vector<OptTensor> t(net_tensors.size());
@@ -308,9 +324,18 @@
     const bool ws = coop && workspace.has_value() && workspace->defined();
     TORCH_CHECK(!coop || ws, "lstm_encode: the cooperative form (H = 256) needs a workspace (ops.Workspaces.encode())");
     const gnnpn_launch_opts_t opts = launch_opts(impl, lds_kb, write_through, paired_start, coop ? status : OptTensor());
-    check_rc(gnnpn_lstm_encode_f32((int)n_nets, nets.data(), (int32_t)B, (int32_t)L, (int32_t)H, 8, prec, &opts,
-                                   ws ? const_cast<uint8_t*>(cptr<uint8_t>(*workspace, at::kByte, "workspace")) : nullptr,
-                                   ws ? workspace->numel() : 0, cur_stream()), "gnnpn_lstm_encode_f32");
+    if (next_workspace.has_value() && next_workspace->defined()) {
+        TORCH_CHECK(ws, "lstm_encode: next_workspace needs the cooperative form");
+        check_rc(gnnpn_lstm_encode_step_f32((int)n_nets, nets.data(), (int32_t)B, (int32_t)L, (int32_t)H, 8, prec, &opts,
+                                            const_cast<uint8_t*>(cptr<uint8_t>(*workspace, at::kByte, "workspace")), workspace->numel(),
+                                            const_cast<uint8_t*>(cptr<uint8_t>(*next_workspace, at::kByte, "next_workspace")),
+                                            next_workspace->numel(), (int32_t)next_nets, (int32_t)next_rows, cur_stream()),
+                 "gnnpn_lstm_encode_step_f32");
+    } else {
+        check_rc(gnnpn_lstm_encode_f32((int)n_nets, nets.data(), (int32_t)B, (int32_t)L, (int32_t)H, 8, prec, &opts,
+                                       ws ? const_cast<uint8_t*>(cptr<uint8_t>(*workspace, at::kByte, "workspace")) : nullptr,
+                                       ws ? workspace->numel() : 0, cur_stream()), "gnnpn_lstm_encode_f32");
+    }
     std::vector<Tensor> out;
     out.insert(out.end(), enc.begin(), enc.end()), out.insert(out.end(), hn.begin(), hn.end()), out.insert(out.end(), cn.begin(), cn.end());
     return out;
@@ -319,7 +344,7 @@
 std::vector<Tensor> pointer_decode(const c10::List<OptTensor>& net_tensors, at::IntArrayRef latent_from, const Tensor& inputs, int64_t n_cat,
                                    int64_t n_per, double tanh_c, bool use_tanh, bool want_queries, std::string precision, int64_t impl,
                                    int64_t lds_kb, bool write_through, const OptTensor& workspace, const OptTensor& status,
-                                   at::IntArrayRef sample_seeds, bool paired_start) {
+                                   at::IntArrayRef sample_seeds, bool paired_start, int64_t step_flags) {
     GNNPN_ON_DEVICE_OF(inputs);
     constexpr size_t NK = 16;
     const size_t n_nets = latent_from.size();
@@ -373,10 +398,16 @@
     const bool ws = coop && workspace.has_value() && workspace->defined();
     TORCH_CHECK(!coop || ws, "pointer_decode: the cooperative form needs a workspace (ops.Workspaces.decode(B, T, n_per))");
     const gnnpn_launch_opts_t opts = launch_opts(impl, lds_kb, write_through, paired_start, coop ? status : OptTensor());
-    check_rc(gnnpn_pointer_decode_f32((int)n_nets, nets.data(), f32(inputs, "inputs"), (float)tanh_c, use_tanh ? 1 : 0, (int32_t)B, (int32_t)n_cat,
-                                      (int32_t)n_per, (int32_t)H, prec == GNNPN_PREC_SPLIT ? GNNPN_PREC_SPLIT : GNNPN_PREC_F32, &opts,
-                                      ws ? const_cast<uint8_t*>(cptr<uint8_t>(*workspace, at::kByte, "workspace")) : nullptr,
-                                      ws ? workspace->numel() : 0, cur_stream()), "gnnpn_pointer_decode_f32");
+    uint8_t* wsp = ws ? const_cast<uint8_t*>(cptr<uint8_t>(*workspace, at::kByte, "workspace")) : nullptr;
+    const int32_t dprec = prec == GNNPN_PREC_SPLIT ? GNNPN_PREC_SPLIT : GNNPN_PREC_F32;
+    if (step_flags != 0)
+        check_rc(gnnpn_pointer_decode_step_f32((int)n_nets, nets.data(), f32(inputs, "inputs"), (float)tanh_c, use_tanh ? 1 : 0, (int32_t)B,
+                                               (int32_t)n_cat, (int32_t)n_per, (int32_t)H, dprec, &opts, wsp, ws ? workspace->numel() : 0,
+                                               (int32_t)step_flags, cur_stream()), "gnnpn_pointer_decode_step_f32");
+    else
+        check_rc(gnnpn_pointer_decode_f32((int)n_nets, nets.data(), f32(inputs, "inputs"), (float)tanh_c, use_tanh ? 1 : 0, (int32_t)B, (int32_t)n_cat,
+                                          (int32_t)n_per, (int32_t)H, dprec, &opts, wsp, ws ? workspace->numel() : 0, cur_stream()),
+                 "gnnpn_pointer_decode_f32");
     return out;
 }
 
@@ -406,10 +437,12 @@
     m.def("attention_logits(Tensor enc_out, Tensor queries, int step, Tensor idx, float tanh_c, bool use_tanh) -> Tensor");
     m.def("qos_reward(Tensor actions, int level) -> Tensor");
     m.def("lstm_encode(Tensor?[] net_tensors, int n_nets, str precision='f32', int impl=0, int lds_kb=0, bool write_through=False, "
-          "Tensor? workspace=None, Tensor? status=None, bool paired_start=False) -> Tensor[]");
+          "Tensor? workspace=None, Tensor? status=None, bool paired_start=False, Tensor? next_workspace=None, int next_nets=0, "
+          "int next_rows=0) -> Tensor[]");
     m.def("pointer_decode(Tensor?[] net_tensors, int[] latent_from, Tensor inputs, int n_cat, int n_per, float tanh_c=10.0, "
           "bool use_tanh=True, bool want_queries=False, str precision='f32', int impl=0, int lds_kb=0, bool write_through=False, "
-          "Tensor? workspace=None, Tensor? status=None, int[] sample_seeds=[], bool paired_start=False) -> Tensor[]");
+          "Tensor? workspace=None, Tensor? status=None, int[] sample_seeds=[], bool paired_start=False, int step_flags=0) -> Tensor[]");
+    m.def("step_tail(Tensor win_logits, Tensor? latent_win, Tensor idx, Tensor actions, int level) -> (Tensor, Tensor)");
 }
 
 TORCH_LIBRARY_IMPL(gnnpn, CUDA, m) {
@@ -430,4 +463,5 @@
     m.impl("qos_reward", qos_reward);
     m.impl("lstm_encode", lstm_encode);
     m.impl("pointer_decode", pointer_decode);
-}
+    m.impl("step_tail", step_tail);
+}
diff --git a/gnnpn-sc_amd/custom_ops.py b/gnnpn-sc_amd/custom_ops.py
--- a/gnnpn-sc_amd/custom_ops.py
+++ b/gnnpn-sc_amd/custom_ops.py
@@ -8,6 +8,7 @@
                "xw_fold", "xb_fold", "start_fold", "latent_win", "whh_split")
 DECODE_OUTS = ("idx", "win_logits", "pick_prob", "actions", "queries")
 ENCODE_KEYS = ("pregates", "inputs", "w_in", "b_in", "whh", "bhh", "whh_split")
+STEP_WORKSPACE_CLEAN, STEP_NO_PICK_PROB = 1, 2
 REQUEST_LAYER_KEYS = ("w0p", "b0", "a1", "s1", "w3p", "b3", "a2", "s2", "eps")
 
 TORCH_LIB_PATH = os.environ.get("GNNPN_TORCH_LIB") or os.path.join(os.path.dirname(os.path.abspath(__file__)), "libgnnpn_torch.so")
@@ -44,12 +45,19 @@
 
 
 @_gnnpn_errors
-def lstm_encode(nets, precision="f32", impl=0, lds_kb=0, write_through=False, ws=None, paired_start=False):
+def lstm_encode(nets, precision="f32", impl=0, lds_kb=0, write_through=False, ws=None, paired_start=False, zero_decode=None):
     flat = [d.get(k) for d in nets for k in ENCODE_KEYS]
     first = nets[0]["pregates"] if nets[0].get("pregates") is not None else nets[0]["inputs"]
     wsp = _coop_ws(first.device, nets[0]["bhh"].numel() // 4, 1, impl, ws)
+    nxt, nxt_nets, nxt_rows = None, 0, 0
+    if zero_decode is not None:
+        if wsp is None:
+            raise _lib.GnnpnError("lstm_encode: zero_decode needs the cooperative form")
+        nxt_nets, nxt_rows, n_cat, n_per = (int(v) for v in zero_decode)
+        nxt = wsp.decode(nxt_rows, n_cat, n_per)[:int(_lib.load().gnnpn_pointer_decode_workspace_bytes(nxt_rows, n_cat, n_per))]
     out = torch.ops.gnnpn.lstm_encode(flat, len(nets), precision, impl, lds_kb, bool(write_through),
-                                      None if wsp is None else wsp.encode(), None if wsp is None else wsp.status, bool(paired_start))
+                                      None if wsp is None else wsp.encode(), None if wsp is None else wsp.status, bool(paired_start),
+                                      nxt, nxt_nets, nxt_rows)
     if wsp is not None:
         wsp.note_launch(0, _lib.load().gnnpn_last_launch_units())
     n = len(nets)
@@ -58,7 +66,7 @@
 
 @_gnnpn_errors
 def pointer_decode(nets, inputs, n_cat, n_per, tanh_c=10.0, use_tanh=True, want_queries=False, precision="f32", impl=0,
-                   lds_kb=0, write_through=False, ws=None, paired_start=False):
+                   lds_kb=0, write_through=False, ws=None, paired_start=False, step_flags=0):
     flat = [d.get(k) for d in nets for k in DECODE_KEYS]
     lf = [int(d.get("latent_from", -1)) for d in nets]
     seeds = [int(d["sample_seed"]) & 0x7FFFFFFFFFFFFFFF if d.get("sample") else -1 for d in nets]
@@ -67,7 +75,7 @@
     out = torch.ops.gnnpn.pointer_decode(flat, lf, inputs, n_cat, n_per, float(tanh_c), bool(use_tanh), bool(want_queries),
                                          precision, impl, lds_kb, bool(write_through),
                                          None if wsp is None else wsp.decode(B, n_cat, n_per), None if wsp is None else wsp.status,
-                                         seeds, bool(paired_start))
+                                         seeds, bool(paired_start), int(step_flags))
     if wsp is not None:
         wsp.note_launch(1, _lib.load().gnnpn_last_launch_units())
     m = len(DECODE_OUTS)
diff --git a/gnnpn-sc_amd/modelPN.py b/gnnpn-sc_amd/modelPN.py
--- a/gnnpn-sc_amd/modelPN.py
+++ b/gnnpn-sc_amd/modelPN.py
@@ -8,6 +8,8 @@
 from . import custom_ops, ops
 
 FOLD_INPUT_PROJECTION = True
+
+STEP_FUSE = int(os.environ.get("GNNPN_STEP_FUSE", "3"))
 
 qosandcons = 8
 qosNum = 4
@@ -339,16 +341,24 @@
     ha.check_precision(precision)
     enc_l, emb_l = la.encode_args(inputs, fold)
     enc_h, emb_h = ha.encode_args(inputs, fold)
+    B, n_cat, n_per = inputs.shape[0], la.serCategory, la.serNumber
+    lean = (sample_high_seed is None and ops.coop_supported(la.hidden_size, n_per, decode_impl) and B > 0 and
+            (FOLD_INPUT_PROJECTION if fold is None else bool(fold)))
+    one_tail, one_zero = lean and bool(STEP_FUSE & 1), lean and bool(STEP_FUSE & 2)
     enc, h_n, c_n = custom_ops.lstm_encode([enc_l, enc_h], precision=precision, lds_kb=lds_kb, write_through=write_through, ws=ws,
-                                           paired_start=paired_start)
+                                           paired_start=paired_start, zero_decode=(2, B, n_cat, n_per) if one_zero else None)
     del enc_l, enc_h
     dl, dh = custom_ops.pointer_decode([la.decode_args(emb_l, enc[0], h_n[0], c_n[0], fold=fold),
                                  ha.decode_args(emb_h, enc[1], h_n[1], c_n[1], latent_from=0, fold=fold,
                                                 sample_seed=sample_high_seed)],
-                                inputs, la.serCategory, la.serNumber, la.C, la.use_tanh,
+                                inputs, n_cat, n_per, la.C, la.use_tanh,
                                 precision="split" if precision == "split" else "f32", impl=decode_impl, lds_kb=lds_kb,
-                                write_through=write_through, ws=ws, paired_start=paired_start)
-    R = torch.ops.gnnpn.qos_reward(dh["actions"], 0 if high.level == "Low" else 1)
+                                write_through=write_through, ws=ws, paired_start=paired_start,
+                                step_flags=(custom_ops.STEP_NO_PICK_PROB if one_tail else 0) | (custom_ops.STEP_WORKSPACE_CLEAN if one_zero else 0))
+    if one_tail:
+        dh["pick_prob"], R = torch.ops.gnnpn.step_tail(dh["win_logits"], dl["win_logits"], dh["idx"], dh["actions"], 0 if high.level == "Low" else 1)
+    else:
+        R = torch.ops.gnnpn.qos_reward(dh["actions"], 0 if high.level == "Low" else 1)
     return ({"idx_low": dl["idx"], "idx_high": dh["idx"], "R": R, "actions": dh["actions"],
              "action_probs": dh["pick_prob"], "win_low": dl["win_logits"], "win_high_raw": dh["win_logits"]},
             (enc[1], h_n[1], c_n[1], emb_h))
diff --git a/include/gnnpn_hip.h b/include/gnnpn_hip.h
--- a/include/gnnpn_hip.h
+++ b/include/gnnpn_hip.h
@@ -155,6 +155,11 @@
 int gnnpn_lstm_encode_f32(int n_nets, const gnnpn_encode_net_t* nets, int32_t B, int32_t L, int32_t H,
                           int32_t F, int32_t precision, const gnnpn_launch_opts_t* opts, void* workspace,
                           int64_t workspace_bytes, void* stream);
+
+int gnnpn_lstm_encode_step_f32(int n_nets, const gnnpn_encode_net_t* nets, int32_t B, int32_t L, int32_t H, int32_t F,
+                               int32_t precision, const gnnpn_launch_opts_t* opts, void* workspace, int64_t workspace_bytes,
+                               void* next_workspace, int64_t next_workspace_bytes, int32_t next_nets, int32_t next_rows,
+                               void* stream);
 
 int64_t gnnpn_lstm_encode_workspace_bytes(void);
 
@@ -200,6 +205,13 @@
                              int32_t precision, const gnnpn_launch_opts_t* opts, void* workspace,
                              int64_t workspace_bytes, void* stream);
 
+#define GNNPN_DECODE_WORKSPACE_CLEAN 1
+#define GNNPN_DECODE_NO_PICK_PROB 2
+int gnnpn_pointer_decode_step_f32(int n_nets, const gnnpn_decode_net_t* nets, const float* inputs, float tanh_c, int use_tanh,
+                                  int32_t B, int32_t T, int32_t n_per, int32_t H, int32_t precision,
+                                  const gnnpn_launch_opts_t* opts, void* workspace, int64_t workspace_bytes, int32_t flags,
+                                  void* stream);
+
 typedef struct {
     int32_t attention;
     int32_t n_glimpses;
@@ -237,6 +249,9 @@
 
 int gnnpn_qos_reward_f32(const float* actions, float* R, int32_t B, int32_t T, int level,
                          void* stream);
+
+int gnnpn_step_tail_f32(const float* win_logits, const float* latent_win, const int32_t* idx, const float* actions,
+                        float* pick_prob, float* R, int32_t B, int32_t T, int32_t n_per, int level, void* stream);
 
 typedef struct {
     const float* embedded;
```

Result: no change. 478,600 (-0.0%).
